# mathijs727/OpenCL-Path-Tracer

Hardware: AMD Instinct MI355X
Metric: Mrays/s at 1080p, 1M-tri SBVH scene; 1/2/4/8-GPU scaling + %HBM roofline (higher is better)
Workload: dtype f32

## Files before the change

### include/ptamd.h

```cpp
#ifndef PTAMD_H
#define PTAMD_H

#include <stddef.h>
#include <stdint.h>

#ifdef __cplusplus
extern "C" {
#endif

typedef enum {
    PT_OK = 0,
    PT_ERR_INVALID = -1,
    PT_ERR_HIP = -2,
    PT_ERR_STATE = -3,
    PT_ERR_UNSUPPORTED = -4
} pt_status;


typedef struct {
    float vertex[4];
    float normal[4];
    float texCoord[2];
    float _pad[2];
} pt_vertex;
// ... 121 lines not shown
void pt_destroy(pt_ctx* ctx);
const char* pt_last_error(const pt_ctx* ctx);
int pt_set_stream(pt_ctx* ctx, void* hip_stream);

int pt_upload_static(pt_ctx* ctx, const pt_vertex* verts, uint32_t n_verts, const pt_triangle* tris, uint32_t n_tris,
    const pt_material* mats, uint32_t n_mats, const pt_sub_bvh_node* nodes, uint32_t n_nodes);
int pt_upload_dynamic(pt_ctx* ctx, const pt_emissive_triangle* lights, uint32_t n_lights,
    const pt_top_bvh_node* top_nodes, uint32_t n_top, uint32_t top_root);
int pt_upload_static_async(pt_ctx* ctx, const pt_vertex* verts, uint32_t n_verts, const pt_triangle* tris, uint32_t n_tris,
    const pt_material* mats, uint32_t n_mats, const pt_sub_bvh_node* nodes, uint32_t n_nodes);
int pt_upload_dynamic_async(pt_ctx* ctx, const pt_emissive_triangle* lights, uint32_t n_lights,
    const pt_top_bvh_node* top_nodes, uint32_t n_top, uint32_t top_root);
int pt_frame_tick(pt_ctx* ctx);
int pt_update_geometry(pt_ctx* ctx, const pt_vertex* verts, uint32_t n_verts, const pt_sub_bvh_node* nodes, uint32_t n_nodes);
int pt_refit_vertices(pt_ctx* ctx, uint32_t first_vertex, const pt_vertex* verts, uint32_t n_verts);
typedef enum { PT_TEX_RGBA32F = 0, PT_TEX_BGRA8_UNORM = 1 } pt_texture_format;
int pt_upload_texture_array(pt_ctx* ctx, int kind, uint32_t width, uint32_t height, uint32_t layers, int format, const void* data);

int pt_set_camera(pt_ctx* ctx, const pt_camera* cam);
int pt_set_tiles(pt_ctx* ctx, const pt_rect* rects, uint32_t n);
int pt_set_accum_buffer(pt_ctx* ctx, void* device_float4);
int pt_clear(pt_ctx* ctx);

int pt_render(pt_ctx* ctx, uint32_t spp);
int pt_synchronize(pt_ctx* ctx);
int pt_resolve(pt_ctx* ctx, float* rgba_out);
int pt_resolve_device(pt_ctx* ctx, void* device_rgba);
void* pt_resolve_device_ptr(pt_ctx* ctx);
int pt_read_accum(pt_ctx* ctx, float* out_float4);
int pt_write_accum(pt_ctx* ctx, const float* in_float4, uint32_t spp);
void* pt_accum_device_ptr(pt_ctx* ctx);
uint32_t pt_samples_per_pixel(const pt_ctx* ctx);
int pt_stats_get(pt_ctx* ctx, pt_stats* out);
int pt_stats_reset(pt_ctx* ctx);
int pt_profile_kernels(pt_ctx* ctx, int enable);
int pt_reduce_accum(pt_ctx* ctx, void* nccl_comm, int root);

#define PT_GUIDE_SKY_DEPTH 1e6f
int pt_render_guides(pt_ctx* ctx, uint32_t spp);
uint32_t pt_guide_samples(const pt_ctx* ctx);
int pt_read_guides(pt_ctx* ctx, float* albedo_hits, float* normal_depth);
int pt_write_guides(pt_ctx* ctx, const float* albedo_hits, const float* normal_depth, uint32_t spp);
void* pt_guides_device_ptr(pt_ctx* ctx, int which);

#define PT_DENOISE_DEFAULT_K_NORMAL 64.0f
#define PT_DENOISE_DEFAULT_SIGMA_DEPTH 0.05f
#define PT_DENOISE_DEFAULT_SIGMA_LUM 0.7f
enum { PT_DENOISE_TONEMAPPED = 0, PT_DENOISE_HDR = 1 };
enum { PT_DENOISE_INPUT_ACCUM = 0, PT_DENOISE_INPUT_TEMPORAL = 1, PT_DENOISE_INPUT_TEMPORAL_VARIANCE = 2 };
typedef struct {
    uint32_t iterations;
    uint32_t output;
    float k_normal, sigma_depth, sigma_lum;
    uint32_t input;
    uint32_t _reserved[2];
} pt_denoise_params;
int pt_denoise(pt_ctx* ctx, const pt_denoise_params* params, float* rgba_out, float* ms_out);
int pt_denoise_device(pt_ctx* ctx, const pt_denoise_params* params, void* device_rgba);

int pt_set_sample_base(pt_ctx* ctx, uint32_t base);
uint32_t pt_sample_base(const pt_ctx* ctx);

typedef struct {
    uint32_t max_history;
    float k_normal, sigma_depth;
    uint32_t _reserved[5];
} pt_temporal_params;
int pt_temporal_accumulate(pt_ctx* ctx, const pt_temporal_params* params);
int pt_temporal_reset(pt_ctx* ctx);
uint32_t pt_temporal_frames(const pt_ctx* ctx);
int pt_read_temporal(pt_ctx* ctx, float* colour_count, float* normal_depth);
int pt_write_temporal(pt_ctx* ctx, const float* colour_count, const float* normal_depth, const pt_camera* made_under);
void* pt_temporal_device_ptr(pt_ctx* ctx, int which);

int pt_set_instance_motion(pt_ctx* ctx, const float* prev_inv_transforms, uint32_t n_top);
int pt_instance_motion(const pt_ctx* ctx, uint32_t* moving_out);
int pt_read_motion_guides(pt_ctx* ctx, float* motion, float* prev_normal);
int pt_write_motion_guides(pt_ctx* ctx, const float* motion, const float* prev_normal);
void* pt_motion_guides_device_ptr(pt_ctx* ctx, int which);
int pt_debug_motion_records(const float* prev_inv, const float* cur_inv, uint32_t n, float* out24);

int pt_set_vertex_motion(pt_ctx* ctx, int enable);
int pt_vertex_motion(const pt_ctx* ctx, uint32_t* deformed_out);
int pt_debug_vertex_motion_rows(const float* inv_transforms, uint32_t n, float* out12);

#define PT_VARIANCE_DEFAULT_SIGMA_VARIANCE 2.0f
#define PT_VARIANCE_DEFAULT_RELATIVE_FLOOR 0.1f
#define PT_VARIANCE_DEFAULT_FULL_HISTORY 16.0f
typedef struct {
    float sigma_variance;
    float relative_floor;
    float full_history;
    uint32_t _reserved[5];
} pt_variance_params;
int pt_set_temporal_variance(pt_ctx* ctx, const pt_variance_params* params);
int pt_temporal_variance(const pt_ctx* ctx);
int pt_read_temporal_variance(pt_ctx* ctx, float* out);
int pt_write_temporal_variance(pt_ctx* ctx, const float* in);
void* pt_temporal_variance_device_ptr(pt_ctx* ctx);

#define PT_RESPONSE_RADIUS 3
#define PT_RESPONSE_DEFAULT_FAST_HISTORY 4u
#define PT_RESPONSE_DEFAULT_SIGMA_RESPONSE 2.0f
#define PT_RESPONSE_DEFAULT_RELATIVE_FLOOR 0.02f
typedef struct {
    uint32_t fast_history;
    float sigma_response;
    float relative_floor;
    uint32_t _reserved[5];
} pt_response_params;
int pt_set_temporal_response(pt_ctx* ctx, const pt_response_params* params);
int pt_temporal_response(const pt_ctx* ctx);
int pt_read_temporal_fast(pt_ctx* ctx, float* colour_count);
int pt_write_temporal_fast(pt_ctx* ctx, const float* colour_count);
int pt_read_temporal_response(pt_ctx* ctx, float* s_out);
void* pt_temporal_fast_device_ptr(pt_ctx* ctx);

typedef struct {
    const float *ox, *oy, *oz, *dx, *dy, *dz;
    const float* tmax;
} pt_rays_soa;
typedef struct {
    float *t, *u, *v;
    int32_t* prim;
    int32_t* inst;
} pt_hits_soa;
int pt_intersect(pt_ctx* ctx, const pt_rays_soa* rays, uint32_t n, int any_hit, pt_hits_soa* hits, uint32_t repeat, float* ms_out);
int pt_gen_rays(pt_ctx* ctx, uint32_t sample, uint32_t n, float* ox, float* oy, float* oz, float* dx, float* dy, float* dz, uint32_t* pixel);
int pt_primary_pass(pt_ctx* ctx, uint32_t sample, uint32_t batch, uint32_t n, float* ox, float* oy, float* oz, float* dx, float* dy, float* dz,
    uint32_t* pixel, pt_hits_soa* hits);

typedef struct {
    uint32_t n;
    const float *ox, *oy, *oz, *dx, *dy, *dz;
    const float *thr_r, *thr_g, *thr_b;
    const uint32_t* pixel;
    const uint32_t* flags;
    const uint32_t* bounce;
    const float *t, *u, *v;
    const int32_t *prim, *inst;
    uint32_t sample;
    float *radiance;
    uint32_t* out_alive;
    float *nox, *noy, *noz, *ndx, *ndy, *ndz, *nthr_r, *nthr_g, *nthr_b;
    uint32_t* nflags;
    uint32_t* shadow_alive;
    float *sox, *soy, *soz, *sdx, *sdy, *sdz, *slen, *sc_r, *sc_g, *sc_b;
} pt_shade_batch_io;
int pt_shade_batch(pt_ctx* ctx, pt_shade_batch_io* io);

int pt_debug_copy_bandwidth(pt_ctx* ctx, size_t bytes, uint32_t repeat, float* gbps_out);
int pt_debug_math_probe(pt_ctx* ctx, const float* a, const float* b, uint32_t n, float* out);
int pt_debug_rng_probe(pt_ctx* ctx, const uint32_t* in, uint32_t n, uint32_t* out);
int pt_debug_live_resources(uint32_t out[4]);
int pt_debug_quantise_node(const float* lo12, const float* hi12, const uint32_t* refs4, const uint8_t* empty4, uint32_t empty_ref, void* out64);
int pt_debug_convert(const pt_config* cfg, const pt_vertex* verts, uint32_t n_verts, const pt_triangle* tris, uint32_t n_tris, const pt_material* mats,
                     uint32_t n_mats, const pt_sub_bvh_node* nodes, uint32_t n_nodes, const pt_emissive_triangle* lights, uint32_t n_lights,
                     const pt_top_bvh_node* top_nodes, uint32_t n_top, uint32_t top_root, char* line, size_t line_bytes);
const char* pt_version(void);

#ifdef __cplusplus
}
#endif
#endif
```

### opencl-path-tracer_amd/csrc/pt_context.h

```cpp
#pragma once

namespace {

thread_local std::string g_createError;

std::atomic<uint32_t> g_live[4];

template <typename T>
struct DevBuf {
    T* p = nullptr;
    size_t n = 0;
    DevBuf() = default;
    DevBuf(DevBuf&& o) noexcept : p(std::exchange(o.p, nullptr)), n(std::exchange(o.n, 0)) {}
    ~DevBuf() { release(); }
    hipError_t alloc(size_t count)
    {
        release();
        n = count;
        if (count == 0)
            return hipSuccess;
        const hipError_t e = hipMalloc((void**)&p, count * sizeof(T));
        if (e == hipSuccess)
            g_live[0]++;
        return e;
// ... 126 lines not shown
    DevBuf<float4> plane[2];
    float4* operator[](int k) const { return plane[k].p; }
    int ensure(pt_ctx* c);
    int zero(pt_ctx* c);
    int read(pt_ctx* c, float* out0, float* out1);
    int write(pt_ctx* c, const float* in0, const float* in1);
};

inline hipError_t allocPlanes(DevBuf<float4>& a, DevBuf<float4>& b, DevBuf<float4>& c, size_t count)
{
    hipError_t e = a.alloc(count);
    if (e == hipSuccess && (e = b.alloc(count)) == hipSuccess)
        e = c.alloc(count);
    return e;
}
struct RayQueueBuf {
    DevBuf<float4> o, d, thr;
    RayQueue view() const { return { o.p, d.p, thr.p }; }
    hipError_t alloc(size_t count) { return allocPlanes(o, d, thr, count); }
    void release() { o.release(), d.release(), thr.release(); }
};
struct ShadowQueueBuf {
    DevBuf<float4> o, d, c;
    ShadowQueue view() const { return { o.p, d.p, c.p }; }
    hipError_t alloc(size_t count) { return allocPlanes(o, d, c, count); }
    void release() { o.release(), d.release(), c.release(); }
};

}

struct StaticScene {
    ptconv::StaticHost host;
    DevBuf<WideNode> dWide;
    DevBuf<WideBoxes> dBoxes;
    DevBuf<uint32_t> dLeafOfs, dRefTri;
    DevBuf<TriIsect> dTris;
    DevBuf<TriFat> dFat;
    uint64_t onDeviceTopology = 0;
    DevBuf<pt_vertex> dVerts;
    DevBuf<pt_sub_bvh_node> dNodes;
    DevBuf<uint32_t> dKidBoxNode;
    DevBuf<float> dExtra;
    DevBuf<uint32_t> dParent, dNeed, dArrived;
    uint64_t refitTablesFor = 0;
    bool refitTablesOk = false;
    bool latestInStage = false;
    Staging stage;
    DevBuf<TriShade> triShade;
    DevBuf<Material> materials;
    bool have = false;
};

struct pt_ctx {
    pt_config cfg {};
    std::string error;
    int device = 0;
    int numCUs = 0;
    Stream stream;
    Stream copyStream;
    Stream sideStream;
    Stream sideStream2;
    Event evStart, evStop;
    std::vector<Event> profEvents;
    bool profile = false;

    ~pt_ctx()
    {
        (void)hipSetDevice(device);
        for (hipStream_t s : { stream.s, copyStream.s, sideStream.s, sideStream2.s })
            if (s)
                (void)hipStreamSynchronize(s);
    }

    struct DynamicSet {
        DevBuf<WideNode> wide;
        DevBuf<TriIsect> tris;
        DevBuf<TriFat> fat;
        DevBuf<Instance> instances;
        DevBuf<Light> lights;
        DevBuf<BakeJob> jobs;
        uint64_t staticVersion = 0;
        int staticIndex = 0;
        uint32_t numTris = 0, firstWorldNode = 0;
        Staging stage;
        uint32_t numLights = 0, rootRef = 0;
        uint32_t foldedInstances = 0, instRootBase = 0, numInstRoots = 0;
        DevBuf<float4> instFold;
        DevBuf<uint32_t> instRootSrc;
        uint32_t instFoldCount = 0;
        uint32_t rootRefFolded = 0;
        bool packetOk = false;
        uint32_t stackNeed = 0;
        bool hasInstances = false;
        bool generalRoute = false;
        uint32_t enteredInstances = 0;
        std::vector<uint32_t> instanceTopNode;
        std::vector<Instance> hostInstances;
        uint32_t numTopNodes = 0;
        Event uploaded;
        Event lastUse;
        bool used = false;
    } dyn[2];
    StaticScene stat[2];
    StaticScene* st = &stat[0];
    int statCur = 0;
    int statPending = -1;
    uint64_t staticVersions = 0;
    int active = 0;
    int pending = -1;
    Event evShaded[kMaxPasses], evShadowed[kMaxPasses];
    DevBuf<float4> accumShadow;
    ShadowQueueBuf shadowQ[kMaxPasses];
    bool mergePending = false;
    DevBuf<uint8_t> texMaterial, texSky;
    SceneDev scene {};
    bool haveStatic = false, haveDynamic = false, haveCamera = false;

    CameraDev camera {};
    DevBuf<uint32_t> pixelList;
    std::vector<uint32_t> hostPixelList;
    DevBuf<uint32_t> pixelOrdinal;
    DevBuf<float4> resolveTmp;
    uint32_t numOwned = 0;
    uint32_t capacity = 0;
    uint32_t capExt = 0, capShadow = 0;
    bool q0Small = false;
    bool ratiosKnown = false;
    double ratioExt = 0, ratioShadow = 0;
    double ratioShadowFirst = 0;
    Pinned<uint32_t> overflowPinned;
    uint32_t batchSamples = 0, probeBatches = 0;
    uint32_t epoch = 0, passCountsEpoch = 0;
    bool identityPixels = true;
    DevBuf<float4> accumOwn, accumPlanes;
    uint32_t packetBlocks[2] = { 0, 0 };
    uint32_t multiBlocks[4] = { 0, 0, 0, 0 };
    Pinned<uint32_t> passCountsPinned;
    Event passCountsCopied;
    uint32_t passCountsHint[2 * (kMaxPasses + 1)] = {};
    uint32_t passCountsEntries = 0;
    uint32_t passCountsPending = 0;
    uint32_t shadeHeadShift = 0;
    uint32_t packetUse = 0;
    uint64_t packetLaunches = 0, genLaunches = 0, bundleLaunches = 0;
    float4* accum = nullptr;
    uint32_t planes = 1;
    uint32_t spp = 0;

    RayQueueBuf rays[2], stagedRays;
    ShadowQueueBuf shadow, stagedShadow;
    DevBuf<float4> hitH;
    DevBuf<int32_t> hitInst;
    DevBuf<uint32_t> activeFlag;
    DevBuf<uint4> streams;
    DevBuf<Control> control;
    DevBuf<Totals> totals;
    DevBuf<uint32_t> spill;
    size_t spillHalf = 0;
    uint32_t traceBlocks[3] = { 0, 0, 0 };
    uint32_t teamBlocks = 0;
    float teamRounds = 1.5f;
    uint32_t teamUse = 7;
    uint32_t batchEntries = 0;
    uint64_t teamLaunches = 0;
    uint32_t foldPlanes = 0;
    bool queuesReady = false;

    PlanePair guides;
    uint32_t guideSpp = 0;
    DevBuf<float4> guideRayO, guideRayD, guideHit;
    DevBuf<int32_t> guideHitInst;
    DevBuf<Control> guideCtl;
    DevBuf<float4> denoiseColour[2], denoiseGuide;
    Event evDenoise[2];

    PlanePair temporal[2];
    int temporalNewest = 0;
    uint32_t temporalFrames = 0;
    CameraDev temporalCamera {};
    uint32_t sampleBase = 0;

    DevBuf<float> temporalVariance[2];
    bool varianceSet = false;
    float sigmaVariance = 0, relativeFloor = 0, fullHistory = 0;

    DevBuf<float4> temporalFast[2];
    DevBuf<float2> responseLuminance;
    DevBuf<float> responseMix;
    bool responseSet = false;
    float fastHistory = 0, sigmaResponse = 0, responseFloor = 0;

    DevBuf<MotionRecord> motionRecords;
    std::vector<MotionRecord> motionHost;
    bool motionSet = false;
    uint32_t motionMoving = 0;
    PlanePair motionGuides;

    DevBuf<TriFat> fatThen;
    DevBuf<float4> vertexRows;
    std::vector<float4> vertexRowsHost;
    bool vertexMotionSet = false;
    bool vertexDeformed = false;

    double msLastRender = 0, msIntersect = 0, msShade = 0, msShadow = 0, msGen = 0, msPacket = 0;
};

namespace {

int fail(pt_ctx* ctx, int code, const char* fmt, ...)
{
    char buf[512];
    va_list ap;
    va_start(ap, fmt);
    vsnprintf(buf, sizeof(buf), fmt, ap);
    va_end(ap);
    if (ctx)
        ctx->error = buf;
    else
        g_createError = buf;
    return code;
}

#define HIPCHK(ctx, call)                                                                              \
    do {                                                                                               \
        hipError_t _e = (call);                                                                        \
        if (_e != hipSuccess)                                                                          \
            return fail(ctx, PT_ERR_HIP, "%s failed: %s (%s:%d)", #call, hipGetErrorString(_e), __FILE__, __LINE__); \
    } while (0)

template <typename F>
int guarded(pt_ctx* c, const char* what, F&& body)
{
    try {
        return body();
    } catch (const std::bad_alloc&) {
        return fail(c, PT_ERR_UNSUPPORTED, "%s: out of host memory", what);
    } catch (const std::exception& e) {
        return fail(c, PT_ERR_INVALID, "%s: %s", what, e.what());
    } catch (...) {
        return fail(c, PT_ERR_INVALID, "%s: unknown exception", what);
    }
}

inline AccumView accumView(const pt_ctx* c) { return { c->accum, c->accumPlanes.p, c->pixelOrdinal.p, c->planes - 1u }; }
inline uint32_t maxBounces(const pt_ctx* c) { return c->cfg.max_bounces ? c->cfg.max_bounces : 4u; }
inline bool parityMode(const pt_ctx* c) { return c->cfg.rng_mode == PT_RNG_LFSR113_PARITY; }
inline bool generalShading(const pt_ctx* c) { return (c->cfg.flags & (PT_FLAG_INTEGRATOR_MIS | PT_FLAG_COMPARE_SHADING | PT_FLAG_SOLID_ANGLE_LIGHTS)) != 0u; }

void refreshSceneView(pt_ctx* c)
{
    SceneDev& s = c->scene;
    const pt_ctx::DynamicSet& d = c->dyn[c->active];
    s.wide = d.wide.p;
    s.tris = d.tris.p;
    s.triFat = d.fat.p;
    s.materials = c->st->materials.p;
    s.instances = d.instances.p;
    s.lights = d.lights.p;
    s.numLights = d.numLights;
    s.rootRef = d.rootRef;
    s.firstWorldNode = d.firstWorldNode;
    s.instRootBase = d.numInstRoots ? d.instRootBase : 0x7FFFFFFFu;
    s.numInstRoots = d.numInstRoots;
    s.materialTex.texels = c->texMaterial.p;
    s.sky.texels = c->texSky.p;
    s.numTriangles = c->haveDynamic ? d.numTris : c->st->host.numTris;
}

template <typename T>
int uploadVec(pt_ctx* c, DevBuf<T>& buf, const std::vector<T>& host)
{
    if (!buf.p || buf.n < std::max<size_t>(host.size(), 1))
        HIPCHK(c, buf.alloc(std::max<size_t>(host.size() + host.size() / 8, 1)));
    if (!host.empty())
        HIPCHK(c, hipMemcpy(buf.p, host.data(), host.size() * sizeof(T), hipMemcpyHostToDevice));
    return PT_OK;
}

int PlanePair::zero(pt_ctx* c)
{
    for (DevBuf<float4>& b : plane)
        HIPCHK(c, hipMemsetAsync(b.p, 0, b.n * sizeof(float4), c->stream));
    return PT_OK;
}

int PlanePair::ensure(pt_ctx* c)
{
    if (plane[0].p)
        return PT_OK;
    for (DevBuf<float4>& b : plane)
        HIPCHK(c, b.alloc((size_t)c->cfg.width * c->cfg.height));
    return zero(c);
}

int PlanePair::read(pt_ctx* c, float* out0, float* out1)
{
    if (const int rc = ensure(c))
        return rc;
    float* const out[2] = { out0, out1 };
    for (int k = 0; k < 2; k++)
        if (out[k])
            HIPCHK(c, hipMemcpyAsync(out[k], plane[k].p, plane[k].n * sizeof(float4), hipMemcpyDeviceToHost, c->stream));
    HIPCHK(c, hipStreamSynchronize(c->stream));
    return PT_OK;
}

// ... 13 lines not shown
```

### opencl-path-tracer_amd/csrc/pt_device.h

```cpp
#pragma once
#include <hip/hip_runtime.h>
#include <stdint.h>

namespace ptd {

struct PairNode {
    float4 bx;
    float4 by;
    float4 bz;
    uint32_t left, right;
    uint32_t _pad0, _pad1;
};

struct WideNode {
    float ox, oy, oz;
    float scaleX;
    uint32_t qlox, qhix, qloy, qhiy;
    uint32_t qloz, qhiz;
    float scaleY, scaleZ;
    uint32_t child[4];
};

constexpr uint32_t kRefIndexBits = 27;
constexpr uint32_t kRefIndexMask = (1u << kRefIndexBits) - 1u;
constexpr uint32_t kMaxLeafTris = 30;
constexpr uint32_t kRefSpecial = 31;
constexpr uint32_t kSpecialFinish = kRefIndexMask;
constexpr uint32_t kSpecialLeaveInstance = kRefIndexMask - 1u;
constexpr uint32_t kRefFinish = 0xFFFFFFFFu;
constexpr uint32_t kRefLeaveInstance = (kRefSpecial << kRefIndexBits) | kSpecialLeaveInstance;
constexpr uint32_t kRefNone = kRefFinish;
constexpr uint32_t kSpecialIdle = kRefIndexMask - 2u;
constexpr uint32_t kRefIdle = (kRefSpecial << kRefIndexBits) | kSpecialIdle;
constexpr uint32_t kRefFirstSpecial = kRefSpecial << kRefIndexBits;
__host__ __device__ inline uint32_t makeRef(uint32_t index, uint32_t count) { return (count << kRefIndexBits) | index; }
__host__ __device__ inline uint32_t refIndex(uint32_t r) { return r & kRefIndexMask; }
__host__ __device__ inline uint32_t refCount(uint32_t r) { return r >> kRefIndexBits; }

struct TriIsect {
    float4 a;
    float4 b;
    float4 c;
};

struct TriShade {
    uint32_t i0, i1, i2, material;
};
struct VertexShade {
    float4 n_u;
    float4 v_pad;
};
struct TriFat {
    float4 n0u, n1u, n2u;
    float4 vvvm;
    float4 e1e;
    float4 e2v;
    float4 v0c;
    float4 mat;
};

struct Instance {
    float4 r0, r1, r2;
    uint32_t rootRef;
    uint32_t topNode;
    uint32_t folded;
    uint32_t simple;
};

struct MotionRecord {
    float4 a0, a1, a2;
    float4 p0, p1, p2;
};

struct Material {
    float4 colour;
    float4 params;
    float4 typeAndPad;
};
enum : int { MAT_DIFFUSE = 0, MAT_PBR = 1, MAT_REFRACTIVE = 2, MAT_BASIC_REFRACTIVE = 3, MAT_EMISSIVE = 4 };

struct Light {
    float4 v0, v1, v2;
    float4 normal;
    float4 colour;
};

struct BakeJob {
    double m[12];
    uint32_t srcNode, numNodes;
    uint32_t dstNode;
    uint32_t srcRef, numRefs;
    uint32_t dstTri;
    uint32_t instance;
    uint32_t _pad;
};

struct WideBoxes {
    float lo[4][3], hi[4][3];
};

struct Texture {
    const void* texels;
    int32_t width, height, layers;
    int32_t format;
};
__device__ inline float4 fetchTexel(const Texture& tex, size_t index)
{
    if (tex.format == 0)
        return ((const float4*)tex.texels)[index];
    const uint32_t p = ((const uint32_t*)tex.texels)[index];
    return make_float4((float)((p >> 16) & 0xFFu) / 255.0f, (float)((p >> 8) & 0xFFu) / 255.0f, (float)(p & 0xFFu) / 255.0f, (float)(p >> 24) / 255.0f);
}

struct SceneDev {
    const PairNode* nodes;
    const WideNode* wide;
    const TriIsect* tris;
    const TriFat* triFat;
    const Material* materials;
    const Instance* instances;
    const Light* lights;
    Texture materialTex;
    Texture sky;
    uint32_t numLights;
    uint32_t rootRef;
    uint32_t numTriangles;
    uint32_t firstWorldNode;
    uint32_t instRootBase;
    uint32_t numInstRoots;
};

struct RayQueue {
    float4* o;
    float4* d;
    float4* thr;
};
struct HitQueue {
    float4* h;
    int32_t* inst;
};
struct ShadowQueue {
    float4* o;
    float4* d;
    float4* c;
};

enum : uint32_t { FLAG_FINISHED = 1, FLAG_LASTSPECULAR = 2 };
__host__ __device__ inline uint32_t packState(uint32_t flags, uint32_t bounce, uint32_t plane) { return (flags & 0xFFu) | ((bounce & 0xFFu) << 8) | (plane << 16); }
struct AccumView {
    float4* plane0;
    float4* extra;
    const uint32_t* ordinal;
    uint32_t perPixel;
    __device__ inline float4* at(uint32_t plane, uint32_t pixel) const
    {
        if (plane == 0u)
            return plane0 + pixel;
        const uint32_t slot = ordinal ? ordinal[pixel] : pixel;
        return extra + (size_t)slot * perPixel + (plane - 1u);
    }
    __device__ inline float4* atOrdinal(uint32_t plane, uint32_t slot) const { return extra + (size_t)slot * perPixel + (plane - 1u); }
};

struct CameraDev {
    float4 eye, screen, u, v, uN, vN;
    float focalDistance, apertureRadius, relativeAperture, shutterTime, ISO;
    uint32_t thinLens;
};

constexpr int kMaxPasses = 16;
#ifndef PT_GEN_INTERLEAVE
#define PT_GEN_INTERLEAVE 256
#endif
constexpr uint32_t kGenInterleave = PT_GEN_INTERLEAVE;
constexpr uint32_t kDepositSlots = 64;
struct Control {
    uint32_t extCount[kMaxPasses + 1];
    uint32_t shadowCount[kMaxPasses + 1];
    uint32_t extCursor[kMaxPasses + 1];
    uint32_t shadowCursor[kMaxPasses + 1];
    uint32_t shadeHits[kMaxPasses + 1];
    uint32_t depositsShade;
    uint32_t depositsShadow;
    uint32_t generated;
    uint32_t _pad;
    uint32_t depositSlots[kDepositSlots][16];
};
struct Totals {
    unsigned long long raysExtension, raysShadow, raysGenerated, shadeHits, deposits, depositsShadow;
};

}
```

### opencl-path-tracer_amd/csrc/pt_packet_multi.h

```cpp
#pragma once
#include "pt_packet.h"

#ifndef PT_MULTI_RAYS
#define PT_MULTI_RAYS 4
#endif
#ifndef PT_MULTI_MIN_WAVES
#define PT_MULTI_MIN_WAVES (PT_MULTI_RAYS >= 8 ? 3 : PT_MULTI_RAYS >= 4 ? 5 : 6)
#endif

namespace ptd {


template <int R>
__device__ inline bool bundleOctant(const V3 (&d)[R], V3& mLo, V3& mHi, bool& nx, bool& ny, bool& nz)
{
    mLo = mk(INFINITY), mHi = mk(0.f);
    unsigned long long sx = 0ull, sy = 0ull, sz = 0ull, ax = ~0ull, ay = ~0ull, az = ~0ull;
#pragma unroll
    for (int r = 0; r < R; r++) {
        const V3 id = mk(rcpSlab(d[r].x), rcpSlab(d[r].y), rcpSlab(d[r].z));
        mLo = mk(fminf(mLo.x, fabsf(id.x)), fminf(mLo.y, fabsf(id.y)), fminf(mLo.z, fabsf(id.z)));
        mHi = mk(fmaxf(mHi.x, fabsf(id.x)), fmaxf(mHi.y, fabsf(id.y)), fmaxf(mHi.z, fabsf(id.z)));
        const unsigned long long bx = __builtin_amdgcn_ballot_w64(id.x < 0.f), by = __builtin_amdgcn_ballot_w64(id.y < 0.f), bz = __builtin_amdgcn_ballot_w64(id.z < 0.f);
        sx |= bx, sy |= by, sz |= bz, ax &= bx, ay &= by, az &= bz;
    }
    nx = sx != 0ull, ny = sy != 0ull, nz = sz != 0ull;
    return (sx == 0ull || ax == ~0ull) && (sy == 0ull || ay == ~0ull) && (sz == 0ull || az == ~0ull);
}
__device__ inline void bundleBeam(const V3 co, V3 mLo, V3 mHi, bool nx, bool ny, bool nz, uint32_t axis, uint32_t isFar, float& S, float& negSO, float& mulPos,
    float& mulNeg, uint32_t& ofsQ)
{
    waveMin3Max3(mLo.x, mLo.y, mLo.z, mHi.x, mHi.y, mHi.z);
    const bool neg = axis == 0u ? nx : (axis == 1u ? ny : nz);
    const float oA = axis == 0u ? co.x : (axis == 1u ? co.y : co.z);
    const float mLoA = (axis == 0u ? mLo.x : (axis == 1u ? mLo.y : mLo.z)) * (1.f - 1.f / 262144.f);
    const float mHiA = (axis == 0u ? mHi.x : (axis == 1u ? mHi.y : mHi.z)) * (1.f + 1.f / 262144.f);
    S = neg ? -1.f : 1.f;
    negSO = -(S * oA);
    mulPos = isFar ? -mHiA : mLoA, mulNeg = isFar ? -mLoA : mHiA;
    ofsQ = 16u + 4u * (2u * axis + ((neg ? 1u : 0u) ^ isFar));
}

template <int R>
__device__ inline void bundleWaist(const V3 (&o)[R], const V3 (&d)[R], V3& pLo, V3& pHi)
{
    pLo = mk(INFINITY), pHi = mk(-INFINITY);
#pragma unroll
    for (int r = 0; r < R; r++) {
        const V3 p = mk(o[r].x + d[r].x, o[r].y + d[r].y, o[r].z + d[r].z);
        const V3 e = mk((fabsf(o[r].x) + fabsf(d[r].x)) * 0x1p-22f, (fabsf(o[r].y) + fabsf(d[r].y)) * 0x1p-22f, (fabsf(o[r].z) + fabsf(d[r].z)) * 0x1p-22f);
        pLo = mk(fminf(pLo.x, p.x - e.x), fminf(pLo.y, p.y - e.y), fminf(pLo.z, p.z - e.z));
        pHi = mk(fmaxf(pHi.x, p.x + e.x), fmaxf(pHi.y, p.y + e.y), fmaxf(pHi.z, p.z + e.z));
    }
}
__device__ inline void bundleBeamLens(V3 pLo, V3 pHi, V3 mLo, V3 mHi, bool nx, bool ny, bool nz, uint32_t axis, uint32_t isFar, float& S, float& negSO, float& mulPos,
    float& mulNeg, uint32_t& ofsQ, float& corner)
{
    waveMin3Max3(pLo.x, pLo.y, pLo.z, pHi.x, pHi.y, pHi.z);
    waveMin3Max3(mLo.x, mLo.y, mLo.z, mHi.x, mHi.y, mHi.z);
    const bool neg = axis == 0u ? nx : (axis == 1u ? ny : nz);
    const float pLoA = axis == 0u ? pLo.x : (axis == 1u ? pLo.y : pLo.z), pHiA = axis == 0u ? pHi.x : (axis == 1u ? pHi.y : pHi.z);
    const float mLoA = (axis == 0u ? mLo.x : (axis == 1u ? mLo.y : mLo.z)) * (1.f - 1.f / 262144.f);
    const float mHiA = (axis == 0u ? mHi.x : (axis == 1u ? mHi.y : mHi.z)) * (1.f + 1.f / 262144.f);
    S = neg ? -1.f : 1.f;
    corner = (neg != (isFar != 0u)) ? pLoA : pHiA;
    negSO = -(S * corner);
    mulPos = isFar ? -mHiA : mLoA, mulNeg = isFar ? -mLoA : mHiA;
    ofsQ = 16u + 4u * (2u * axis + ((neg ? 1u : 0u) ^ isFar));
}

template <int R, bool TWO_LEVEL, bool LENS = false>
#ifndef PT_MULTI_MIN_WAVES_TL
#define PT_MULTI_MIN_WAVES_TL PT_MULTI_MIN_WAVES
#endif
#ifndef PT_MULTI_MIN_WAVES_LENS
#define PT_MULTI_MIN_WAVES_LENS PT_MULTI_MIN_WAVES
#endif
#ifndef PT_MULTI_MIN_WAVES_LENS_TL
#define PT_MULTI_MIN_WAVES_LENS_TL 4
#endif
__global__ void __launch_bounds__(kPacketBlock, LENS ? (TWO_LEVEL ? PT_MULTI_MIN_WAVES_LENS_TL : PT_MULTI_MIN_WAVES_LENS) : (TWO_LEVEL ? PT_MULTI_MIN_WAVES_TL : PT_MULTI_MIN_WAVES))
    k_trace_multi(TraceArgs a)
{
    constexpr int RO = LENS ? R : 1;
    constexpr float tShift = LENS ? 1.0f : 0.0f;
    constexpr int kSaveRay = 0, kSaveBeam = 3 * RO + 3 * R, kSaveInst = kSaveBeam + 5, kSave = kSaveInst + R;
    __shared__ uint32_t ldsSave[TWO_LEVEL ? kPacketBlock / 64 : 1][TWO_LEVEL ? kSave : 1][64];
    const uint32_t pwave = threadIdx.x >> 6;
    typedef uint32_t u4v __attribute__((ext_vector_type(4)));
    typedef const u4v __attribute__((address_space(4)))* ScalarU4;
    const uint32_t lane = threadIdx.x & 63u;
    const uint32_t gwave = (blockIdx.x * kPacketBlock + threadIdx.x) >> 6;
    const uint32_t totalWaves = (gridDim.x * kPacketBlock) >> 6;
    const uint32_t count = a.ctl->extCount[a.pass];
    const SceneDev& sc = a.sc;
    constexpr uint32_t kPer = 64u * R;
    const uint32_t supers = (count + kPer - 1u) / kPer;
    const uint32_t rootRef = uni(sc.rootRef);
    const ScalarU4 wideS = (ScalarU4)(unsigned long long)sc.wide;
    const ScalarU4 trisS = (ScalarU4)(unsigned long long)sc.tris;

#ifndef PT_MULTI_SPAN
#define PT_MULTI_SPAN 8
#endif
    constexpr uint32_t kSpan = PT_MULTI_SPAN;
    uint32_t spanBase = uni(gwave) * kSpan, spanLeft = kSpan;
    for (;;) {
        if (spanLeft == 0u) {
            const uint32_t left = supers > spanBase ? supers - spanBase : 0u;
            const uint32_t claim = min(kSpan, max(1u, left / totalWaves));
            uint32_t b = 0;
            if (lane == 0)
                b = atomicAdd(&a.ctl->extCursor[a.pass], claim);
            spanBase = totalWaves * kSpan + uni(b);
            spanLeft = claim;
        }
        if (spanBase >= supers)
            break;
        const uint32_t base = spanBase * kPer;
        spanBase++;
        spanLeft--;

        V3 co[RO], cd[R];
        float tClosest[R], hu[R], hv[R];
        int hprim[R];
        bool whole = true;
#pragma unroll
        for (int r = 0; r < R; r++) {
            const uint32_t idx = base + 64u * (uint32_t)r + lane;
            const bool active = idx < count;
            V3 o = mk(0.f), d = mk(0.f, 0.f, 1.f);
            if (active) {
                uint32_t px, pl;
                primaryEntry(a.fp, a.pixelList, idx, &px, &pl);
                primaryRay(a.fp, px, pl, &o, &d);
                if (a.noOrigins) {
                    ((float4*)a.rayD)[idx] = make_float4(d.x, d.y, d.z, asF(px));
                } else {
                    ((float4*)a.rayO)[idx] = make_float4(o.x, o.y, o.z, asF(px));
                    ((float4*)a.rayD)[idx] = make_float4(d.x, d.y, d.z, asF(packState(FLAG_LASTSPECULAR, 0u, pl)));
                }
            }
            nudgeZero(o, d);
            if (LENS || r == 0)
                co[LENS ? r : 0] = o;
            cd[r] = d;
            tClosest[r] = INFINITY, hu[r] = hv[r] = 0.f, hprim[r] = -1;
            if constexpr (TWO_LEVEL)
                ldsSave[pwave][kSaveInst + r][lane] = 0xFFFFFFFFu;
            whole = whole && __builtin_amdgcn_ballot_w64(active) == ~0ull;
            if constexpr (!LENS)
                whole = whole && __builtin_amdgcn_ballot_w64(o.x != asF(uni(asU(co[0].x))) || o.y != asF(uni(asU(co[0].y))) || o.z != asF(uni(asU(co[0].z)))) == 0ull;
        }
        V3 mLo, mHi;
        bool nx, ny, nz;
        whole = bundleOctant<R>(cd, mLo, mHi, nx, ny, nz) && whole;

        if (whole) {
            const uint32_t role = lane & 7u, child = (lane >> 3) & 3u, axis = min(role >> 1, 2u), isFar = role & 1u;
            const uint32_t ofsO = 4u * axis, ofsE = axis == 0u ? 12u : 36u + 4u * axis, shift = 8u * child;
            float S, negSO, mulPos, mulNeg, corner = 0.f;
            uint32_t ofsQ;
            if constexpr (LENS) {
                V3 pLo, pHi;
                bundleWaist<R>(co, cd, pLo, pHi);
                bundleBeamLens(pLo, pHi, mLo, mHi, nx, ny, nz, axis, isFar, S, negSO, mulPos, mulNeg, ofsQ, corner);
            } else {
                bundleBeam(co[0], mLo, mHi, nx, ny, nz, axis, isFar, S, negSO, mulPos, mulNeg, ofsQ);
            }
            int curInst = -1;
            if constexpr (TWO_LEVEL) {
#pragma unroll
                for (int r = 0; r < RO; r++)
                    ldsSave[pwave][kSaveRay + 3 * r][lane] = asU(co[r].x), ldsSave[pwave][kSaveRay + 3 * r + 1][lane] = asU(co[r].y), ldsSave[pwave][kSaveRay + 3 * r + 2][lane] = asU(co[r].z);
#pragma unroll
                for (int r = 0; r < R; r++)
                    ldsSave[pwave][kSaveRay + 3 * RO + 3 * r][lane] = asU(cd[r].x), ldsSave[pwave][kSaveRay + 3 * RO + 1 + 3 * r][lane] = asU(cd[r].y),
                                  ldsSave[pwave][kSaveRay + 3 * RO + 2 + 3 * r][lane] = asU(cd[r].z);
                ldsSave[pwave][kSaveBeam + 0][lane] = asU(S), ldsSave[pwave][kSaveBeam + 1][lane] = asU(negSO), ldsSave[pwave][kSaveBeam + 2][lane] = asU(mulPos);
                ldsSave[pwave][kSaveBeam + 3][lane] = asU(mulNeg), ldsSave[pwave][kSaveBeam + 4][lane] = ofsQ;
            }
            float tcMax = INFINITY;
            uint32_t stRef = 0u;
            uint32_t sp = 0u;
            uint32_t cur = rootRef;
#ifdef PT_TRACE_STATS
            uint32_t stNodes = 0u, stLeaves = 0u, stTris = 0u;
#endif
            while (true) {
#ifdef PT_TRACE_STATS
                if (refCount(cur) == 0u)
                    stNodes++;
                else if (refCount(cur) != kRefSpecial)
                    stLeaves++, stTris += refCount(cur);
#endif
                if (TWO_LEVEL && refCount(cur) == kRefSpecial) {
                    if (cur != kRefLeaveInstance) {
                        typedef const u4v_t __attribute__((address_space(4)))* ScalarU4i;
                        const ScalarU4i mrow = (ScalarU4i)(unsigned long long)&sc.instances[refIndex(cur)];
                        const u4v_t m0 = mrow[0], m1 = mrow[1], m2 = mrow[2];
                        const float4 r0 = asF4(m0), r1 = asF4(m1), r2 = asF4(m2);
                        if (uni(mrow[3].w) != 0u) {
#pragma unroll
                            for (int r = 0; r < RO; r++)
                                co[r] = mk(fmaf(r0.x, co[r].x, r0.w), fmaf(r1.y, co[r].y, r1.w), fmaf(r2.z, co[r].z, r2.w));
#pragma unroll
                            for (int r = 0; r < R; r++)
                                cd[r] = mk(r0.x * cd[r].x, r1.y * cd[r].y, r2.z * cd[r].z);
                            const float scl = fastRcp(r0.x);
                            if constexpr (LENS) {
                                const float wA = axis == 0u ? r0.w : (axis == 1u ? r1.w : r2.w);
                                const float c = fmaf(r0.x, corner, wA);
                                const float e = (fabsf(r0.x * corner) + fabsf(wA)) * 0x1p-22f;
                                negSO = isFar ? -(S * c) + e : -(S * c) - e;
                            } else {
                                negSO = -(S * (axis == 0u ? co[0].x : (axis == 1u ? co[0].y : co[0].z)));
                            }
                            mulPos *= scl, mulNeg *= scl;
                        } else {
                            V3 to[RO], td[R];
#pragma unroll
                            for (int r = 0; r < R; r++)
                                rayIntoInstance(r0, r1, r2, co[LENS ? r : 0], cd[r], &to[LENS ? r : 0], &td[r]);
                            V3 tLo, tHi;
                            bool tnx, tny, tnz;
                            if (!bundleOctant<R>(td, tLo, tHi, tnx, tny, tnz)) {
                                whole = false;
                                break;
                            }
#pragma unroll
                            for (int r = 0; r < RO; r++)
                                co[r] = to[r];
#pragma unroll
                            for (int r = 0; r < R; r++)
                                cd[r] = td[r];
                            if constexpr (LENS) {
                                V3 pLo, pHi;
                                float cornerInst;
                                bundleWaist<R>(co, cd, pLo, pHi);
                                bundleBeamLens(pLo, pHi, tLo, tHi, tnx, tny, tnz, axis, isFar, S, negSO, mulPos, mulNeg, ofsQ, cornerInst);
                            } else {
                                bundleBeam(co[0], tLo, tHi, tnx, tny, tnz, axis, isFar, S, negSO, mulPos, mulNeg, ofsQ);
                            }
                        }
                        curInst = (int)refIndex(cur);
                        stRef = laneWrite(stRef, kRefLeaveInstance, uni(sp));
                        sp++;
                        cur = uni(mrow[3].x);
                        continue;
                    }
#pragma unroll
                    for (int r = 0; r < RO; r++)
                        co[r] = mk(asF(ldsSave[pwave][kSaveRay + 3 * r][lane]), asF(ldsSave[pwave][kSaveRay + 3 * r + 1][lane]), asF(ldsSave[pwave][kSaveRay + 3 * r + 2][lane]));
#pragma unroll
                    for (int r = 0; r < R; r++)
                        cd[r] = mk(asF(ldsSave[pwave][kSaveRay + 3 * RO + 3 * r][lane]), asF(ldsSave[pwave][kSaveRay + 3 * RO + 1 + 3 * r][lane]),
                            asF(ldsSave[pwave][kSaveRay + 3 * RO + 2 + 3 * r][lane]));
                    S = asF(ldsSave[pwave][kSaveBeam + 0][lane]), negSO = asF(ldsSave[pwave][kSaveBeam + 1][lane]), mulPos = asF(ldsSave[pwave][kSaveBeam + 2][lane]);
                    mulNeg = asF(ldsSave[pwave][kSaveBeam + 3][lane]), ofsQ = ldsSave[pwave][kSaveBeam + 4][lane];
                    curInst = -1;
                } else if (refCount(cur) == 0u) {
                    const uint32_t ni = refIndex(cur);
                    const u4v D = wideS[ni * 4u + 3u];
                    const char* nb = (const char*)&sc.wide[ni];
                    const float originA = *(const float*)(nb + ofsO);
                    const float scaleA = *(const float*)(nb + ofsE);
                    const uint32_t qd = *(const uint32_t*)(nb + ofsQ);
                    const float q = (float)((qd >> shift) & 0xFFu);
                    const float g = fmaf(q, S * scaleA, fmaf(S, originA, negSO));
                    float v = g * (g >= 0.f ? mulPos : mulNeg);
                    v = maxRowShr2(v);
                    v = maxRowShr2(v);
                    const float tn = rowShr1(v);
                    const unsigned long long m = __builtin_amdgcn_ballot_w64(tn + v <= 0.f) & __builtin_amdgcn_ballot_w64(v <= tShift) & __builtin_amdgcn_ballot_w64(tn < tcMax);
                    const uint32_t tloBits = (uint32_t)max((int32_t)asU(tn + tShift), 0);
                    uint32_t key[4];
#pragma unroll
                    for (int k = 0; k < 4; k++)
                        key[k] = ((m >> (8 * k + 5)) & 1ull) ? ((__builtin_amdgcn_readlane(tloBits, 8 * k + 5) & ~3u) | (uint32_t)k) : (kKeyNone | (uint32_t)k);
                    const bool s01 = key[0] < key[1], s23 = key[2] < key[3];
                    const uint32_t k01 = s01 ? key[0] : key[1], k23 = s23 ? key[2] : key[3];
                    const uint32_t r01 = s01 ? D.x : D.y, r23 = s23 ? D.z : D.w;
                    const bool sl = k01 < k23;
                    const uint32_t best = sl ? k01 : k23;
                    if (best < kKeyNone) {
                        const uint32_t refs[4] = { D.x, D.y, D.z, D.w };
                        const uint32_t limit = kKeyNone - best - 1u;
#pragma unroll
                        for (int k = 0; k < 4; k++)
                            if (key[k] - best - 1u < limit) {
                                stRef = laneWrite(stRef, uni(refs[k]), uni(sp));
                                sp++;
                            }
                        cur = sl ? r01 : r23;
                        continue;
// ... 14 lines not shown
                        for (int r = 0; r < R; r++) {
                            float det, u, v, t;
                            if constexpr (LENS)
                                triOriginHalf(co[r], v0, e1, e2, &T, &Q, &e2Q);
                            triRayHalf(cd[r], e1, e2, T, Q, e2Q, &det, &u, &v, &t);
                            const bool hit = PT_TRI_HIT(det, u, v, t, tClosest[r]);
                            if (hit) {
                                tClosest[r] = t;
                                hu[r] = u;
                                hv[r] = v;
                                hprim[r] = (int)(first + k);
                                if constexpr (TWO_LEVEL)
                                    ldsSave[pwave][kSaveInst + r][lane] = (uint32_t)curInst;
                                any = true;
                            }
                        }
                    }
                    if (__builtin_amdgcn_ballot_w64(any) != 0ull) {
                        float far = tClosest[0];
#pragma unroll
                        for (int r = 1; r < R; r++)
                            far = fmaxf(far, tClosest[r]);
                        if (__builtin_amdgcn_ballot_w64(far == INFINITY) == 0ull)
                            tcMax = LENS ? asF(uni(asU(waveMax(far)))) * (1.0f + 0x1p-20f) - tShift : asF(uni(asU(waveMax(far))));
                    }
                }
                if (sp == 0u)
                    break;
                sp--;
                cur = __builtin_amdgcn_readlane(stRef, sp);
            }
#ifdef PT_TRACE_STATS
            if (lane == 0) {
                atomicAdd(&g_traceStats[56], 1ull), atomicAdd(&g_traceStats[57], (unsigned long long)stNodes), atomicAdd(&g_traceStats[58], (unsigned long long)stLeaves);
                atomicAdd(&g_traceStats[59], (unsigned long long)stTris);
                if (!whole)
                    atomicAdd(&g_traceStats[60], 1ull);
            }
#endif
        }
        if (!whole) {
#pragma unroll 1
            for (int r = 0; r < R; r++) {
                const uint32_t idx = base + 64u * (uint32_t)r + lane;
                const bool active = idx < count;
                V3 o = mk(0.f), d = mk(0.f, 0.f, 1.f);
                if (active) {
                    uint32_t px, pl;
                    primaryEntry(a.fp, a.pixelList, idx, &px, &pl);
                    primaryRay(a.fp, px, pl, &o, &d);
                }
                nudgeZero(o, d);
                V3 cid = mk(rcpSlab(d.x), rcpSlab(d.y), rcpSlab(d.z));
                bool nx = cid.x < 0.f, ny = cid.y < 0.f, nz = cid.z < 0.f;
                const V3 wo = o, wd = d;
                int curInst = -1;
                if constexpr (TWO_LEVEL)
                    ldsSave[pwave][kSaveInst + r][lane] = 0xFFFFFFFFu;
                float tC = INFINITY, u_ = 0.f, v_ = 0.f;
                int hp = -1;
                uint32_t stRef = 0u, stLo = 0u, stHi = 0u;
                uint32_t sp = 0u;
                uint32_t cur = rootRef;
                unsigned long long curMask = __builtin_amdgcn_ballot_w64(active);
                if (curMask != 0ull)
                    while (true) {
                        const bool here = __builtin_amdgcn_inverse_ballot_w64(curMask);
                        if (TWO_LEVEL && refCount(cur) == kRefSpecial) {
                            if (cur != kRefLeaveInstance) {
                                V3 to, td;
                                uint32_t root;
                                packetIntoInstance(sc.instances, refIndex(cur), o, d, &to, &td, &root);
                                o = to, d = td, cid = mk(rcpSlab(td.x), rcpSlab(td.y), rcpSlab(td.z));
                                nx = cid.x < 0.f, ny = cid.y < 0.f, nz = cid.z < 0.f;
                                curInst = (int)refIndex(cur);
                                lanePush(stRef, stLo, stHi, kRefLeaveInstance, 0u, 0u, uni(sp));
                                sp++;
                                cur = uni(root);
                                continue;
                            }
                            o = wo, d = wd, cid = mk(rcpSlab(d.x), rcpSlab(d.y), rcpSlab(d.z));
                            nx = cid.x < 0.f, ny = cid.y < 0.f, nz = cid.z < 0.f;
                            curInst = -1;
                        } else if (refCount(cur) == 0u) {
                            const uint32_t ni = refIndex(cur);
                            const u4v A = wideS[ni * 4u + 0u], Cs = wideS[ni * 4u + 2u], D = wideS[ni * 4u + 3u];
                            const uint4* wp = (const uint4*)&sc.wide[ni];
                            const uint4 B = wp[1];
                            const uint2 C = *(const uint2*)&wp[2];
                            const SlabSetup slab = slabSetup(make_uint4(A.x, A.y, A.z, A.w), B, make_uint4(C.x, C.y, Cs.z, Cs.w), o, cid, nx, ny, nz);
                            const float tLimit = here ? tC : -INFINITY;
                            unsigned long long m[4];
                            uint32_t key[4];
#pragma unroll
                            for (int k = 0; k < 4; k++) {
                                const f2 tt = childSlab(slab, k);
                                const float tmin = tt.x, tmax = tt.y;
                                const float tlo = fmaxf(tmin, 0.f);
                                const bool vis = tmax >= tlo && tmin < tLimit;
                                m[k] = __builtin_amdgcn_ballot_w64(vis);
                                const uint32_t pick = (uint32_t)(__builtin_ffsll((long long)m[k]) - 1) & 63u;
                                key[k] = (__builtin_amdgcn_readlane(asU(vis ? tlo : INFINITY), pick) & ~3u) | (uint32_t)k;
                            }
                            const bool s01 = key[0] < key[1], s23 = key[2] < key[3];
                            const uint32_t k01 = s01 ? key[0] : key[1], k23 = s23 ? key[2] : key[3];
                            const uint32_t r01 = s01 ? D.x : D.y, r23 = s23 ? D.z : D.w;
                            const unsigned long long m01 = s01 ? m[0] : m[1], m23 = s23 ? m[2] : m[3];
                            const bool sl = k01 < k23;
                            const uint32_t best = sl ? k01 : k23;
                            if (best < kKeyNone) {
                                const uint32_t refs[4] = { D.x, D.y, D.z, D.w };
                                const uint32_t limit = kKeyNone - best - 1u;
#pragma unroll
                                for (int k = 0; k < 4; k++)
                                    if (key[k] - best - 1u < limit) {
                                        lanePush(stRef, stLo, stHi, uni(refs[k]), uni((uint32_t)m[k]), uni((uint32_t)(m[k] >> 32)), uni(sp));
                                        sp++;
                                    }
                                cur = sl ? r01 : r23;
                                curMask = sl ? m01 : m23;
                                continue;
                            }
                        } else {
                            const uint32_t first = refIndex(cur), n = refCount(cur);
                            for (uint32_t k = 0; k < n; k++) {
                                const u4v ta = trisS[(first + k) * 3u + 0u], tb = trisS[(first + k) * 3u + 1u];
                                const uint32_t tcx = trisS[(first + k) * 3u + 2u].x;
                                V3 v0, e1, e2;
                                triEdges(asF4(ta), asF4(tb), asF(tcx), &v0, &e1, &e2);
                                V3 T, Q;
                                float e2Q, det, u, v, t;
                                triOriginHalf(o, v0, e1, e2, &T, &Q, &e2Q);
                                triRayHalf(d, e1, e2, T, Q, e2Q, &det, &u, &v, &t);
                                const bool hit = here && PT_TRI_HIT(det, u, v, t, tC);
                                if (hit) {
                                    tC = t, u_ = u, v_ = v, hp = (int)(first + k);
                                    if constexpr (TWO_LEVEL)
                                        ldsSave[pwave][kSaveInst + r][lane] = (uint32_t)curInst;
                                }
                            }
                        }
                        if (sp == 0u)
                            break;
                        sp--;
                        cur = __builtin_amdgcn_readlane(stRef, sp);
                        curMask = (unsigned long long)__builtin_amdgcn_readlane(stLo, sp) | ((unsigned long long)__builtin_amdgcn_readlane(stHi, sp) << 32);
                    }
#pragma unroll
                for (int q = 0; q < R; q++)
                    if (q == r)
                        tClosest[q] = tC, hu[q] = u_, hv[q] = v_, hprim[q] = hp;
            }
        }
#pragma unroll
        for (int r = 0; r < R; r++) {
            const uint32_t idx = base + 64u * (uint32_t)r + lane;
            if (idx < count) {
                int hinst = -1;
                if constexpr (TWO_LEVEL)
                    hinst = (int)ldsSave[pwave][kSaveInst + r][lane];
                writeClosestHit(a, sc, idx, tClosest[r], hu[r], hv[r], hprim[r], hinst);
            }
        }
    }
}

}
```

### opencl-path-tracer_amd/csrc/pt_schedule.h

```cpp
#pragma once

namespace {

void lfsrJump(uint32_t g[4])
{
    uint32_t z, b;
    z = g[0] & (uint32_t)(-2);
    b = (z << 6) ^ z;
    z = (z) ^ (z << 2) ^ (z << 3) ^ (z << 10) ^ (z << 13) ^ (z << 16) ^ (z << 19) ^ (z << 22) ^ (z << 25) ^ (z << 27) ^ (z << 28)
        ^ ((b >> 3) & 0x1FFFFFFF) ^ ((b >> 4) & 0x0FFFFFFF) ^ ((b >> 6) & 0x03FFFFFF) ^ ((b >> 9) & 0x007FFFFF)
        ^ ((b >> 12) & 0x000FFFFF) ^ ((b >> 15) & 0x0001FFFF) ^ ((b >> 18) & 0x00003FFF) ^ ((b >> 21) & 0x000007FF);
    g[0] = z;
    z = g[1] & (uint32_t)(-8);
    b = (z << 2) ^ z;
    z = ((b >> 13) & 0x0007FFFF) ^ (z << 16);
    g[1] = z;
    z = g[2] & (uint32_t)(-16);
    b = (z << 13) ^ z;
    z = (z << 2) ^ (z << 4) ^ (z << 10) ^ (z << 12) ^ (z << 13) ^ (z << 17) ^ (z << 25)
        ^ ((b >> 3) & 0x1FFFFFFF) ^ ((b >> 11) & 0x001FFFFF) ^ ((b >> 15) & 0x0001FFFF) ^ ((b >> 16) & 0x0000FFFF) ^ ((b >> 24) & 0x000000FF);
    g[2] = z;
    z = g[3] & (uint32_t)(-128);
    b = (z << 3) ^ z;
    z = (z << 9) ^ (z << 10) ^ (z << 11) ^ (z << 14) ^ (z << 16) ^ (z << 18) ^ (z << 23) ^ (z << 24)
        ^ ((b >> 1) & 0x7FFFFFFF) ^ ((b >> 2) & 0x3FFFFFFF) ^ ((b >> 7) & 0x01FFFFFF) ^ ((b >> 9) & 0x007FFFFF)
        ^ ((b >> 11) & 0x001FFFFF) ^ ((b >> 14) & 0x0003FFFF) ^ ((b >> 15) & 0x0001FFFF) ^ ((b >> 16) & 0x0000FFFF)
        ^ ((b >> 23) & 0x000001FF) ^ ((b >> 24) & 0x000000FF);
    g[3] = z;
}

int resetStreams(pt_ctx* c)
{
    const size_t n = (size_t)c->cfg.width * c->cfg.height;
    std::vector<uint4> host(n);
    uint32_t g[4] = { 987654321u, 987654321u, 987654321u, 987654321u };
    for (size_t i = 0; i < n; i++) {
        host[i] = make_uint4(g[0], g[1], g[2], g[3]);
        lfsrJump(g);
    }
    return uploadVec(c, c->streams, host);
}

#ifndef PT_SPLIT_SHADOW_ACCUM
#define PT_SPLIT_SHADOW_ACCUM 1
#endif
inline bool splitShadowAccum(const pt_ctx* c, uint64_t cap)
{
    return PT_SPLIT_SHADOW_ACCUM && c->planes == 1u && !parityMode(c) && c->cfg.max_active_rays == 0 && cap <= (4u << 20) && !(c->packetUse & 2u) && maxBounces(c) <= (uint32_t)kMaxPasses;
}

bool derivedPrimariesCapable(const pt_ctx* c);
inline void newEpoch(pt_ctx* c)
{
    c->epoch++;
    c->ratiosKnown = false;
    c->ratioExt = c->ratioShadow = c->ratioShadowFirst = 0;
}
inline bool smallQueues(const pt_ctx* c) { return c->capExt < c->capacity || c->capShadow < c->capacity; }
inline int checkOverflow(pt_ctx* c)
{
    if (c->overflowPinned.p && *c->overflowPinned.p)
        return fail(c, PT_ERR_STATE, "a batch emitted more rays than its queues hold (pt_config.ext_queue_fraction / shadow_queue_fraction; the scene changed under a "
                                    "running batch?): the rays beyond were dropped, the image since the last pt_clear is incomplete -- pt_clear and render again");
    return PT_OK;
}
inline void adoptPassCounts(pt_ctx* c)
{
    std::memcpy(c->passCountsHint, c->passCountsPinned.p, sizeof(c->passCountsHint));
    c->passCountsEntries = c->passCountsPending;
    c->passCountsPending = 0;
    if (c->passCountsEpoch == c->epoch && c->passCountsEntries) {
        const double entries = (double)c->passCountsEntries;
        uint32_t shadowMost = 0;
        for (int b = 0; b <= kMaxPasses; b++)
            shadowMost = std::max(shadowMost, c->passCountsHint[kMaxPasses + 1 + b]);
        c->ratioExt = std::max(c->ratioExt, (double)c->passCountsHint[1] / entries);
        c->ratioShadow = std::max(c->ratioShadow, (double)shadowMost / entries);
        c->ratioShadowFirst = std::max(c->ratioShadowFirst, (double)c->passCountsHint[kMaxPasses + 1] / entries);
        c->ratiosKnown = true;
    }
}
inline uint32_t safeBatch(const pt_ctx* c)
{
    auto limit = [&](uint32_t cap, double ratio) -> double {
        if (!(ratio > 0.0))
            return (double)c->planes;
        const double room = (double)cap - std::min(65536.0, (double)cap / 64.0);
        return room / (ratio * 1.03 * (double)c->numOwned);
    };
    double b = std::min(limit(c->capExt, c->ratioExt), limit(c->capShadow, c->ratioShadow));
    if (const char* e = getenv("PTAMD_DEBUG_BATCH_SCALE"))
        b *= atof(e);
    return (uint32_t)std::max(1.0, std::min((double)c->planes, b));
}

int ensureQueues(pt_ctx* c)
{
    if (c->queuesReady)
        return PT_OK;
    if (c->numOwned == 0)
        return fail(c, PT_ERR_STATE, "no pixels owned by this context");
    c->planes = 1;
    if (!parityMode(c) && c->cfg.max_active_rays == 0) {
        uint32_t want = c->cfg.samples_in_flight;
        if (want == 0)
            want = (uint32_t)std::min<uint64_t>(4096, std::max<uint64_t>(1, (32u << 20) / std::max(c->numOwned, 1u)));
        c->planes = std::min(want, 4096u);
        if (c->planes >= kGenInterleave) {
            c->planes -= c->planes % kGenInterleave;
        } else {
            uint32_t p2 = 1;
            while (p2 * 2u <= c->planes)
                p2 *= 2u;
            c->planes = p2;
        }
    }
    uint64_t cap64 = c->cfg.max_active_rays ? c->cfg.max_active_rays : (uint64_t)c->numOwned * c->planes;
    if (cap64 > 0x7FFFFFC0ull)
        return fail(c, PT_ERR_UNSUPPORTED, "%llu queue entries (%u owned pixels x %u samples in flight) exceed the 2^31 entries a queue can index: lower samples_in_flight",
            (unsigned long long)cap64, c->numOwned, c->planes);
    uint32_t cap = ((uint32_t)cap64 + 63u) & ~63u;
    {
        HIPCHK(c, hipStreamSynchronize(c->stream));
        c->rays[0].release(), c->rays[1].release(), c->shadow.release(), c->hitH.release(), c->hitInst.release(), c->accumPlanes.release();
        for (ShadowQueueBuf& q : c->shadowQ)
            q.release();
        c->stagedRays.release(), c->stagedShadow.release(), c->activeFlag.release();
        c->foldPlanes = 0;
        const bool split = splitShadowAccum(c, cap);
        c->capExt = c->capShadow = cap;
        c->q0Small = false;
        const float fe = c->cfg.ext_queue_fraction, fs = c->cfg.shadow_queue_fraction;
        if (!parityMode(c) && c->cfg.max_active_rays == 0 && c->planes >= 16u && !split) {
            if (fe > 0.f && fe < 1.f)
                c->capExt = std::min<uint64_t>(cap, (((uint64_t)((double)cap * fe) + 63u) & ~63ull) + 64u);
            if (fs > 0.f && fs < 1.f)
                c->capShadow = std::min<uint64_t>(cap, (((uint64_t)((double)cap * fs) + 63u) & ~63ull) + 64u);
            const uint64_t floorEntries = std::min<uint64_t>(cap, ((16ull * c->numOwned + 63u) & ~63ull));
            c->capExt = (uint32_t)std::max<uint64_t>(c->capExt, floorEntries);
            c->capShadow = (uint32_t)std::max<uint64_t>(c->capShadow, floorEntries);
            c->q0Small = c->capExt < cap && derivedPrimariesCapable(c);
        }
        newEpoch(c);
        const uint64_t q0 = 16ull * cap + 32ull * (c->q0Small ? c->capExt : cap);
        const uint64_t need = q0 + 48ull * c->capExt + 48ull * c->capShadow + 20ull * cap + (uint64_t)cap * (parityMode(c) ? 2ull * 48 + 4 : 0)
            + (uint64_t)(c->planes - 1) * c->numOwned * sizeof(float4)
            + (split ? (uint64_t)cap * 48 * maxBounces(c) + (uint64_t)c->cfg.width * c->cfg.height * sizeof(float4) * maxBounces(c) : 0);
        size_t freeB = 0, totalB = 0;
        HIPCHK(c, hipMemGetInfo(&freeB, &totalB));
        if (need > (uint64_t)freeB)
            return fail(c, PT_ERR_UNSUPPORTED, "queues and accumulator planes need %.1f GB (%u owned pixels x %u samples in flight), %.1f GB of device memory are free: lower samples_in_flight or set max_active_rays",
                need / 1e9, c->numOwned, c->planes, freeB / 1e9);
    }
    if (c->planes > 1) {
        const size_t n = (size_t)(c->planes - 1) * c->numOwned;
        HIPCHK(c, c->accumPlanes.alloc(n));
        HIPCHK(c, hipMemsetAsync(c->accumPlanes.p, 0, n * sizeof(float4), c->stream));
    }
    c->capacity = cap;
    HIPCHK(c, c->rays[0].o.alloc(c->q0Small ? c->capExt : cap));
    HIPCHK(c, c->rays[0].d.alloc(cap));
    HIPCHK(c, c->rays[0].thr.alloc(c->q0Small ? c->capExt : cap));
    HIPCHK(c, c->rays[1].alloc(c->capExt));
    HIPCHK(c, c->shadow.alloc(c->capShadow));
    HIPCHK(c, c->hitH.alloc(cap));
    HIPCHK(c, c->hitInst.alloc(cap));
    if (parityMode(c)) {
        HIPCHK(c, c->stagedRays.alloc(cap));
        HIPCHK(c, c->stagedShadow.alloc(cap));
        HIPCHK(c, c->activeFlag.alloc(cap));
        int rc = resetStreams(c);
        if (rc)
            return rc;
    }
    if (splitShadowAccum(c, cap)) {
        const size_t npx = (size_t)c->cfg.width * c->cfg.height;
        if (!c->accumShadow.p || c->accumShadow.n < npx * maxBounces(c)) {
            HIPCHK(c, c->accumShadow.alloc(npx * maxBounces(c)));
            HIPCHK(c, hipMemsetAsync(c->accumShadow.p, 0, npx * maxBounces(c) * sizeof(float4), c->stream));
        }
        for (uint32_t b = 0; b < maxBounces(c); b++)
            HIPCHK(c, c->shadowQ[b].alloc(cap));
    }
    HIPCHK(c, c->control.alloc(1));
    HIPCHK(c, hipMemsetAsync(c->control.p, 0, sizeof(Control), c->stream));
    c->queuesReady = true;
    return PT_OK;
}

int ensureSpill(pt_ctx* c)
{
    if (c->spill.p)
        return PT_OK;
    const void* variants[3][2] = { { (const void*)k_trace<false, 0>, (const void*)k_trace<true, 0> }, { (const void*)k_trace<false, 1>, (const void*)k_trace<true, 1> },
        { (const void*)k_trace<false, 2>, (const void*)k_trace<true, 2> } };
    const void* packetVariants[2][2] = { { (const void*)k_trace_packet<false, false>, (const void*)k_trace_packet<true, false> },
        { (const void*)k_trace_packet<false, true>, (const void*)k_trace_packet<true, true> } };
    for (int tl = 0; tl < 3; tl++) {
        int blocksPerCU = 8;
        for (const void* fn : variants[tl]) {
            int b = 0;
            HIPCHK(c, hipOccupancyMaxActiveBlocksPerMultiprocessor(&b, fn, kTraceBlock, 0));
            blocksPerCU = std::min(blocksPerCU, b);
        }
        blocksPerCU = std::max(1, blocksPerCU);
        if (const char* e = getenv("PTAMD_TRACE_BLOCKS_PER_CU"))
            blocksPerCU = std::max(1, std::min(blocksPerCU, atoi(e)));
        c->traceBlocks[tl] = (uint32_t)(blocksPerCU * c->numCUs);
        if (tl >= 2)
            continue;
        int pb = 8;
        for (const void* fn : packetVariants[tl]) {
            int b = 0;
            HIPCHK(c, hipOccupancyMaxActiveBlocksPerMultiprocessor(&b, fn, kPacketBlock, 0));
            pb = std::min(pb, b);
        }
        pb = std::max(1, pb);
        if (const char* e = getenv("PTAMD_PACKET_BLOCKS_PER_CU"))
            pb = std::max(1, std::min(pb, atoi(e)));
        c->packetBlocks[tl] = (uint32_t)(pb * c->numCUs);
    }
    {
        int b = 0;
        HIPCHK(c, hipOccupancyMaxActiveBlocksPerMultiprocessor(&b, (const void*)k_trace_multi<PT_MULTI_RAYS, false>, kPacketBlock, 0));
        c->multiBlocks[0] = (uint32_t)(std::max(1, b) * c->numCUs);
        HIPCHK(c, hipOccupancyMaxActiveBlocksPerMultiprocessor(&b, (const void*)k_trace_multi<PT_MULTI_RAYS, true>, kPacketBlock, 0));
        c->multiBlocks[1] = (uint32_t)(std::max(1, b) * c->numCUs);
        HIPCHK(c, hipOccupancyMaxActiveBlocksPerMultiprocessor(&b, (const void*)k_trace_multi<PT_MULTI_RAYS, false, true>, kPacketBlock, 0));
        c->multiBlocks[2] = (uint32_t)(std::max(1, b) * c->numCUs);
        HIPCHK(c, hipOccupancyMaxActiveBlocksPerMultiprocessor(&b, (const void*)k_trace_multi<PT_MULTI_RAYS, true, true>, kPacketBlock, 0));
        c->multiBlocks[3] = (uint32_t)(std::max(1, b) * c->numCUs);
        if (const char* e = getenv("PTAMD_PACKET_BLOCKS_PER_CU"))
            for (uint32_t& mb : c->multiBlocks)
                mb = std::max(1u, std::min(mb, (uint32_t)std::max(1, atoi(e)) * (uint32_t)c->numCUs));
    }
    {
        int t0 = 0, t1 = 0;
        HIPCHK(c, hipOccupancyMaxActiveBlocksPerMultiprocessor(&t0, (const void*)k_trace_team<false>, kTeamBlock, 0));
        HIPCHK(c, hipOccupancyMaxActiveBlocksPerMultiprocessor(&t1, (const void*)k_trace_team<true>, kTeamBlock, 0));
        c->teamBlocks = (uint32_t)(std::max(1, std::min(t0, t1)) * c->numCUs);
        if (const char* e = getenv("PTAMD_TEAM_ROUNDS"))
            c->teamRounds = std::max(0.f, (float)atof(e));
        if (const char* e = getenv("PTAMD_TEAM_USE"))
            c->teamUse = (uint32_t)atoi(e);
    }
    const size_t threads = (size_t)std::max(std::max(c->traceBlocks[0], c->traceBlocks[1]), c->traceBlocks[2]) * kTraceBlock;
    HIPCHK(c, c->spill.alloc(3 * threads * kSpillStack));
    c->spillHalf = threads * kSpillStack;
    return PT_OK;
}

inline int sceneKind(const pt_ctx* c)
{
    static const bool forceTwoLevel = getenv("PTAMD_FORCE_TWO_LEVEL_KERNELS") != nullptr;
    return (c->dyn[c->active].hasInstances || forceTwoLevel) ? 1 : 0;
}

inline int traceKind(const pt_ctx* c) { return sceneKind(c) == 0 ? 0 : (c->dyn[c->active].generalRoute ? 2 : 1); }

bool teamLaunch(const pt_ctx* c, uint32_t pass, bool anyHit = false)
{
    if (!(c->teamRounds > 0.f) || !c->teamBlocks || parityMode(c) || c->dyn[c->active].hasInstances || c->dyn[c->active].stackNeed > kTeamStackNeedMax)
        return false;
    if (c->cfg.flags & PT_FLAG_TEAM_INTERSECT)
        return true;
    if (!c->batchEntries || pass > (uint32_t)kMaxPasses)
        return false;
    if (pass == 0u && c->planes == 1u && c->batchEntries <= (4u << 20) && (c->teamUse & (anyHit ? 4u : 1u)))
        return true;
    if (c->passCountsEntries != c->batchEntries || !(c->teamUse & 2u))
        return false;
    const uint64_t teams = (uint64_t)c->teamBlocks * (kTeamBlock / 4);
    return (double)c->passCountsHint[pass] <= (double)teams * c->teamRounds;
}

void launchTrace(pt_ctx* c, bool anyHit, const TraceArgs& args, hipStream_t stream = nullptr)
{
    if (teamLaunch(c, args.pass, anyHit)) {
        c->teamLaunches++;
        if (anyHit)
            hipLaunchKernelGGL(k_trace_team<true>, dim3(c->teamBlocks), dim3(kTeamBlock), 0, stream ? stream : c->stream, args);
        else
            hipLaunchKernelGGL(k_trace_team<false>, dim3(c->teamBlocks), dim3(kTeamBlock), 0, stream ? stream : c->stream, args);
        return;
    }
    const bool twoLevel = sceneKind(c) != 0;
    const int kind = traceKind(c);
    TraceArgs a = args;
    if (twoLevel) {
        a.sc.rootRef = c->dyn[c->active].rootRefFolded;
        a.instFold = c->dyn[c->active].instFold.p, a.instFoldCount = c->dyn[c->active].instFoldCount;
    }
    const dim3 grid(c->traceBlocks[kind]), block(kTraceBlock);
    if (!stream)
        stream = c->stream;
    if (anyHit) {
        if (kind == 2)
            hipLaunchKernelGGL((k_trace<true, 2>), grid, block, 0, stream, a);
        else if (kind == 1)
            hipLaunchKernelGGL((k_trace<true, 1>), grid, block, 0, stream, a);
        else
            hipLaunchKernelGGL((k_trace<true, 0>), grid, block, 0, stream, a);
    } else {
        if (kind == 2)
            hipLaunchKernelGGL((k_trace<false, 2>), grid, block, 0, stream, a);
        else if (kind == 1)
            hipLaunchKernelGGL((k_trace<false, 1>), grid, block, 0, stream, a);
        else
            hipLaunchKernelGGL((k_trace<false, 0>), grid, block, 0, stream, a);
    }
}

TraceArgs traceArgsBase(pt_ctx* c)
{
    TraceArgs a {};
    a.sc = c->scene;
    a.spill = c->spill.p;
    a.totalThreads = c->traceBlocks[traceKind(c)] * kTraceBlock;
    a.parityShadow = parityMode(c) ? 1u : 0u;
    return a;
}

FrameParams frameParams(const pt_ctx* c, uint32_t sample)
{
    FrameParams fp {};
    fp.cam = c->camera;
    fp.width = c->cfg.width;
    fp.height = c->cfg.height;
    fp.sample = sample;
    fp.seed = c->cfg.seed;
    fp.maxBounces = maxBounces(c);
    fp.parity = parityMode(c) ? 1u : 0u;
    fp.numOwned = c->numOwned;
    fp.planes = 1;
    fp.interleave = 1;
    fp.interleaveShift = 0;
    fp.invWidth = 1.0f / (float)c->cfg.width;
    fp.integrator = (c->cfg.flags & PT_FLAG_COMPARE_SHADING) ? INTEGRATOR_COMPARE : ((c->cfg.flags & PT_FLAG_INTEGRATOR_MIS) ? INTEGRATOR_MIS : INTEGRATOR_IS);
    fp.weightedLights = (c->cfg.flags & PT_FLAG_SOLID_ANGLE_LIGHTS) ? 1u : 0u;
    fp.invSpan = 0.f;
    return fp;
}

struct Prof {
    pt_ctx* c;
    size_t next = 0;
    std::vector<std::pair<int, size_t>> marks;
    void begin(int family)
    {
        if (!c->profile)
            return;
        if (c->profEvents.size() < next + 2) {
            c->profEvents.resize(next + 2);
            for (Event& e : c->profEvents)
                (void)e.create(true);
        }
        (void)hipEventRecord(c->profEvents[next], c->stream);
        marks.push_back({ family, next });
    }
    void end()
    {
        if (!c->profile)
            return;
        (void)hipEventRecord(c->profEvents[next + 1], c->stream);
        next += 2;
    }
};

void launchGen(pt_ctx* c, const FrameParams& fp, int q, uint32_t first, uint32_t n, uint32_t slotBase, uint32_t pass)
{
    Control* ctl = c->control.p;
    const uint32_t span = fp.planes > 1u ? fp.numOwned * fp.interleave : std::max(n, 1u);
    const uint32_t blocks = (span + 255u) / 256u, rows = fp.planes > 1u ? fp.planes / fp.interleave : 1u;
    c->genLaunches++;
    hipLaunchKernelGGL(k_gen, dim3(blocks, rows), dim3(256), 0, c->stream, fp, c->rays[q].view(), c->identityPixels ? nullptr : c->pixelList.p,
        first, n, slotBase, c->streams.p, &ctl->extCount[pass], &ctl->generated);
}

#ifndef PT_FRAME_BUNDLES
#define PT_FRAME_BUNDLES 0
#endif
#ifndef PT_FUSED_PRIMARY
#define PT_FUSED_PRIMARY 1
#endif
#ifndef PT_SHADE_SPLIT
#define PT_SHADE_SPLIT 1
#endif
#ifndef PT_LAST_SHADOW_ON_MAIN
#define PT_LAST_SHADOW_ON_MAIN 1
#endif
#ifndef PT_DERIVED_PRIMARIES
#define PT_DERIVED_PRIMARIES 1
#endif
#ifndef PT_OVERLAP_SMALL
#define PT_OVERLAP_SMALL 1
#endif
#ifndef PT_PACKET_USE
#define PT_PACKET_USE 1
#endif
constexpr uint32_t kPacketUseDefault = PT_PACKET_USE;

void launchPacket(pt_ctx* c, bool anyHit, const TraceArgs& a)
{
    const bool twoLevel = sceneKind(c) != 0;
    const dim3 grid(c->packetBlocks[twoLevel ? 1 : 0]), block(kPacketBlock);
    c->packetLaunches++;
    if (anyHit) {
        if (twoLevel)
            hipLaunchKernelGGL((k_trace_packet<true, true>), grid, block, 0, c->stream, a);
        else
            hipLaunchKernelGGL((k_trace_packet<true, false>), grid, block, 0, c->stream, a);
    } else {
        if (twoLevel)
            hipLaunchKernelGGL((k_trace_packet<false, true>), grid, block, 0, c->stream, a);
        else
            hipLaunchKernelGGL((k_trace_packet<false, false>), grid, block, 0, c->stream, a);
    }
}

inline bool lensBundles()
{
    static const bool on = !(getenv("PTAMD_LENS_BUNDLES") && atoi(getenv("PTAMD_LENS_BUNDLES")) == 0);
    return on;
}
inline bool primaryBundles(const pt_ctx* c)
{
    return PT_MULTI_RAYS > 1 && (!c->camera.thinLens || lensBundles()) && !(c->packetUse & 8u) && c->dyn[c->active].packetOk && (c->packetUse & 1u);
}
bool derivedPrimariesCapable(const pt_ctx* c)
{
    return c->haveCamera && c->haveDynamic && !c->camera.thinLens && primaryBundles(c) && PT_FUSED_PRIMARY && PT_DERIVED_PRIMARIES && !(c->cfg.flags & PT_FLAG_QUEUE_PRIMARY_RAYS);
}

inline bool firstPassCoherent(const pt_ctx* c, const FrameParams& fp, uint32_t batch) { return fp.interleave >= 16u || (PT_FRAME_BUNDLES && batch == 1u && primaryBundles(c)); }

void launchIntersect(pt_ctx* c, int q, uint32_t pass, bool coherent = false, const FrameParams* fused = nullptr, bool noOrigins = false)
{
    Control* ctl = c->control.p;
    TraceArgs a = traceArgsBase(c);
    if (fused) {
        a.fused = 1u;
        a.fp = *fused;
        a.pixelList = c->identityPixels ? nullptr : c->pixelList.p;
    }
    a.rayO = c->rays[q].o.p;
    a.rayD = c->rays[q].d.p;
    a.hit = c->hitH.p;
    a.inst = c->hitInst.p;
    a.ctl = ctl;
    a.pass = pass;
    if (coherent && c->dyn[c->active].packetOk && (c->packetUse & 1u)) {
        if (fused && primaryBundles(c)) {
            a.noOrigins = noOrigins ? 1u : 0u;
            c->packetLaunches++;
            c->bundleLaunches++;
            if (c->camera.thinLens) {
                a.noOrigins = 0u;
                if (sceneKind(c) != 0)
                    hipLaunchKernelGGL((k_trace_multi<PT_MULTI_RAYS, true, true>), dim3(c->multiBlocks[3]), dim3(kPacketBlock), 0, c->stream, a);
                else
                    hipLaunchKernelGGL((k_trace_multi<PT_MULTI_RAYS, false, true>), dim3(c->multiBlocks[2]), dim3(kPacketBlock), 0, c->stream, a);
            } else if (sceneKind(c) != 0)
                hipLaunchKernelGGL((k_trace_multi<PT_MULTI_RAYS, true>), dim3(c->multiBlocks[1]), dim3(kPacketBlock), 0, c->stream, a);
            else
                hipLaunchKernelGGL((k_trace_multi<PT_MULTI_RAYS, false>), dim3(c->multiBlocks[0]), dim3(kPacketBlock), 0, c->stream, a);
        } else {
            launchPacket(c, false, a);
        }
    } else {
        launchTrace(c, false, a);
    }
}

void launchShadow(pt_ctx* c, uint32_t pass, bool coherent = false, hipStream_t side = nullptr, const ShadowQueueBuf* own = nullptr)
{
    Control* ctl = c->control.p;
    TraceArgs a = traceArgsBase(c);
    if (side)
        a.spill = c->spill.p + c->spillHalf * (side == c->sideStream2 ? 2u : 1u);
    const ShadowQueueBuf& q = own ? *own : c->shadow;
    a.rayO = q.o.p;
    a.rayD = q.d.p;
    a.rayC = q.c.p;
    a.accum = own ? AccumView { c->accumShadow.p + (size_t)pass * c->cfg.width * c->cfg.height, nullptr, nullptr, 0u } : accumView(c);
    a.ctl = ctl;
    a.pass = pass;
    if (coherent && c->dyn[c->active].packetOk && (c->packetUse & 2u))
        launchPacket(c, true, a);
    else
        launchTrace(c, true, a, side);
}

void launchShade(pt_ctx* c, const FrameParams& fp, int in, int out, uint32_t pass, uint32_t launchEntries, const ShadowQueueBuf* ownShadow = nullptr, bool derivedPrimaries = false)
{
    Control* ctl = c->control.p;
    ShadeArgs a {};
    a.sc = c->scene;
    a.fp = fp;
    a.in = c->rays[in].view();
    a.hits = { c->hitH.p, c->hitInst.p };
    a.accum = accumView(c);
    a.inCount = &ctl->extCount[pass];
    a.outCount = &ctl->extCount[pass + 1];
    a.shadowCount = &ctl->shadowCount[pass];
    a.shadeHits = &ctl->shadeHits[pass];
    a.deposits = parityMode(c) ? &ctl->depositsShade : &ctl->depositSlots[0][0];
    a.streams = c->streams.p;
    a.derivedPrimaries = derivedPrimaries ? 1u : 0u;
    a.outCap = out == 1 ? c->capExt : (c->q0Small ? c->capExt : c->capacity);
    a.shadowCap = ownShadow ? c->capacity : c->capShadow;
    const uint32_t blocks = (std::max(launchEntries, 1u) + kShadeBlock - 1u) / kShadeBlock;
    if (parityMode(c)) {
        a.out = c->stagedRays.view();
        a.shadow = c->stagedShadow.view();
        a.activeFlag = c->activeFlag.p;
        if (generalShading(c))
            hipLaunchKernelGGL((k_shade<true, true>), dim3(blocks), dim3(kShadeBlock), 0, c->stream, a);
        else
            hipLaunchKernelGGL((k_shade<true, false>), dim3(blocks), dim3(kShadeBlock), 0, c->stream, a);
        CompactArgs ca {};
        ca.staged = c->stagedRays.view();
        ca.out = c->rays[out].view();
        ca.stagedShadow = c->stagedShadow.view();
        ca.outShadow = c->shadow.view();
        ca.activeFlag = c->activeFlag.p;
        ca.inCount = &ctl->extCount[pass];
        ca.outCount = &ctl->extCount[pass + 1];
        ca.shadowCount = &ctl->shadowCount[pass];
        ca.shadeHits = &ctl->shadeHits[pass];
        hipLaunchKernelGGL(k_compact_stable, dim3(1), dim3(1024), 0, c->stream, ca);
    } else {
        a.out = c->rays[out].view();
        a.shadow = ownShadow ? ownShadow->view() : c->shadow.view();
        uint32_t head = blocks;
        if (PT_SHADE_SPLIT && pass > 0) {
            if (c->passCountsEntries && !c->shadeHeadShift) {
                const double scale = (double)launchEntries / (double)c->passCountsEntries;
                const double guess = (double)c->passCountsHint[pass] * scale * 1.03;
                head = std::min(blocks, (uint32_t)(guess / kShadeBlock) + 8u);
            } else {
                head = std::max(1u, blocks >> std::min(pass + c->shadeHeadShift, 24u));
            }
        }
        if (generalShading(c))
            hipLaunchKernelGGL((k_shade<false, true>), dim3(head), dim3(kShadeBlock), 0, c->stream, a);
        else if (c->st->host.materialBins)
            hipLaunchKernelGGL((k_shade<false, false, false, true>), dim3(head), dim3(kShadeBlock), 0, c->stream, a);
        else
            hipLaunchKernelGGL((k_shade<false, false>), dim3(head), dim3(kShadeBlock), 0, c->stream, a);
        if (head < blocks) {
            a.firstTile = head;
            const uint32_t rest = std::min(blocks - head, launchEntries <= (4u << 20) ? 64u : 512u);
            if (generalShading(c))
                hipLaunchKernelGGL((k_shade<false, true, true>), dim3(rest), dim3(kShadeBlock), 0, c->stream, a);
            else
                hipLaunchKernelGGL((k_shade<false, false, true>), dim3(rest), dim3(kShadeBlock), 0, c->stream, a);
        }
    }
}

FrameParams batchFrameParams(pt_ctx* c, uint32_t sample, uint32_t batch)
{
    FrameParams fp = frameParams(c, sample);
    fp.planes = batch;
    fp.interleave = 1;
    while (fp.interleave < kGenInterleave && batch % (fp.interleave * 2u) == 0u)
        fp.interleave *= 2u, fp.interleaveShift++;
    fp.invSpan = 1.0f / (float)((uint64_t)c->numOwned << fp.interleaveShift);
    return fp;
}

int renderSampleFixed(pt_ctx* c, uint32_t sample, uint32_t batch, Prof& prof)
{
    FrameParams fp = batchFrameParams(c, sample, batch);
    if (c->passCountsPending) {
        if (hipEventQuery(c->passCountsCopied) == hipSuccess) {
            adoptPassCounts(c);
        } else {
            (void)hipGetLastError();
        }
    }
    const uint32_t bounces = maxBounces(c);
    const uint32_t entries = c->numOwned * batch;
    c->batchEntries = entries;
    const bool coherentFirst = firstPassCoherent(c, fp, batch);
    const bool packetsFirst = coherentFirst && c->dyn[c->active].packetOk && (c->packetUse & 1u);
    const bool fused = packetsFirst && PT_FUSED_PRIMARY && !(c->cfg.flags & PT_FLAG_QUEUE_PRIMARY_RAYS);
    const bool derived = fused && primaryBundles(c) && !c->camera.thinLens && PT_DERIVED_PRIMARIES;
    if (c->q0Small && !derived && entries > c->capExt)
        return fail(c, PT_ERR_STATE, "the first queue was sized for camera rays queued as directions only, and this batch queues their origins");
    prof.begin(0);
    if (fused)
        hipLaunchKernelGGL(k_begin_batch, dim3(1), dim3(64), 0, c->stream, &c->control.p->extCount[0], &c->control.p->generated, entries);
    else
        launchGen(c, fp, 0, 0, entries, 0, 0);
    prof.end();
    const bool overlap = PT_OVERLAP_SMALL && entries <= (4u << 20) && !c->profile && !(c->packetUse & 2u);
    const bool split = splitShadowAccum(c, c->capacity);
    if (split) {
        if (!c->accumShadow.p || !c->shadowQ[bounces - 1].o.p)
            return fail(c, PT_ERR_STATE, "the buffers of the one-sample-in-flight schedule are missing");
        c->mergePending = true;
    }
    int in = 0, out = 1;
    for (uint32_t b = 0; b < bounces; b++) {
        prof.begin(1);
        const bool coherent = b == 0 && coherentFirst;
        if (c->profile && coherent && c->dyn[c->active].packetOk && (c->packetUse & 1u))
            prof.marks.back().first = 4;
        launchIntersect(c, in, b, coherent, fused && b == 0 ? &fp : nullptr, derived && b == 0);
        prof.end();
        if (overlap && !split && b > 0)
            HIPCHK(c, hipStreamWaitEvent(c->stream, c->evShadowed[b - 1], 0));
        prof.begin(2);
        launchShade(c, fp, in, out, b, entries, split ? &c->shadowQ[b] : nullptr, derived && b == 0);
        if (b == 0 ? smallQueues(c) : c->capShadow < c->capExt) {
            const uint32_t outCap = out == 1 ? c->capExt : (c->q0Small ? c->capExt : c->capacity);
            hipLaunchKernelGGL(k_clamp_counts, dim3(1), dim3(64), 0, c->stream, c->control.p, b, outCap, c->capShadow, c->overflowPinned.p);
        }
        prof.end();
        prof.begin(3);
        if (overlap && b + 1u == bounces && PT_LAST_SHADOW_ON_MAIN) {
            launchShadow(c, b, coherent, nullptr, split ? &c->shadowQ[b] : nullptr);
        } else if (overlap) {
            hipStream_t side = split && (b & 1u) ? c->sideStream2 : c->sideStream;
            HIPCHK(c, hipEventRecord(c->evShaded[b], c->stream));
            HIPCHK(c, hipStreamWaitEvent(side, c->evShaded[b], 0));
            launchShadow(c, b, coherent, side, split ? &c->shadowQ[b] : nullptr);
            HIPCHK(c, hipEventRecord(c->evShadowed[b], side));
        } else {
            launchShadow(c, b, coherent, nullptr, split ? &c->shadowQ[b] : nullptr);
        }
        prof.end();
        std::swap(in, out);
    }
    if (overlap && PT_LAST_SHADOW_ON_MAIN) {
        if (split && bounces > 1)
            HIPCHK(c, hipStreamWaitEvent(c->stream, c->evShadowed[bounces - 2], 0));
        if (split && bounces > 2)
            HIPCHK(c, hipStreamWaitEvent(c->stream, c->evShadowed[bounces - 3], 0));
    } else if (overlap) {
        HIPCHK(c, hipStreamWaitEvent(c->stream, c->evShadowed[bounces - 1], 0));
        if (split && bounces > 1)
            HIPCHK(c, hipStreamWaitEvent(c->stream, c->evShadowed[bounces - 2], 0));
    }
    const bool report = c->passCountsPinned.p && !c->passCountsPending;
    hipLaunchKernelGGL(k_end_sample, dim3(1), dim3(64), 0, c->stream, c->control.p, c->totals.p, bounces, report ? c->passCountsPinned.p : nullptr);
    if (report) {
        HIPCHK(c, hipEventRecord(c->passCountsCopied, c->stream));
        c->passCountsPending = entries;
        c->passCountsEpoch = c->epoch;
    }
    c->batchSamples = batch;
    c->batchEntries = 0;
    c->foldPlanes = std::max(c->foldPlanes, batch);
    HIPCHK(c, hipGetLastError());
    return PT_OK;
}

void foldPlanesNow(pt_ctx* c)
{
    if (c->mergePending) {
        const uint32_t n = c->cfg.width * c->cfg.height;
        hipLaunchKernelGGL(k_merge_accum, dim3((n + 255u) / 256u), dim3(256), 0, c->stream, c->accum, c->accumShadow.p, n, maxBounces(c));
        c->mergePending = false;
    }
    if (c->foldPlanes > 1) {
        const uint32_t n = c->numOwned;
        hipLaunchKernelGGL(k_fold_planes, dim3((uint32_t)(((uint64_t)n * kFoldLanes + 255) / 256)), dim3(256), 0, c->stream, accumView(c), c->foldPlanes,
            c->identityPixels ? nullptr : c->pixelList.p, n);
    }
    c->foldPlanes = 0;
}

int renderSampleRefill(pt_ctx* c, uint32_t sample)
{
    const FrameParams fp = frameParams(c, sample);
    Control* ctl = c->control.p;
    const uint32_t cap = c->capacity;
    uint32_t issued = 0, surviving = 0, pass = 0;
    int in = 0, out = 1;
    Control zero {};
    while (true) {
        hipLaunchKernelGGL(k_set_word, dim3(1), dim3(64), 0, c->stream, &ctl->extCount[0], surviving);
        HIPCHK(c, hipMemsetAsync(&ctl->extCount[1], 0, sizeof(uint32_t), c->stream));
        HIPCHK(c, hipMemsetAsync(&ctl->shadowCount[0], 0, sizeof(uint32_t), c->stream));
        HIPCHK(c, hipMemsetAsync(&ctl->extCursor[0], 0, sizeof(uint32_t), c->stream));
        HIPCHK(c, hipMemsetAsync(&ctl->shadowCursor[0], 0, sizeof(uint32_t), c->stream));
        uint32_t newRays = 0;
        if (surviving != cap) {
            newRays = std::min(cap - surviving, c->numOwned - issued);
            if (newRays)
                launchGen(c, fp, in, issued, newRays, surviving, 0);
        }
        const uint32_t entries = surviving + newRays;
        launchIntersect(c, in, 0);
        launchShade(c, fp, in, out, 0, entries);
        uint32_t counts[2] = { 0, 0 };
        HIPCHK(c, hipMemcpyAsync(&counts[0], &ctl->extCount[1], sizeof(uint32_t), hipMemcpyDeviceToHost, c->stream));
        HIPCHK(c, hipMemcpyAsync(&counts[1], &ctl->shadowCount[0], sizeof(uint32_t), hipMemcpyDeviceToHost, c->stream));
        HIPCHK(c, hipStreamSynchronize(c->stream));
        issued += newRays;
        surviving = counts[0];
        pass++;
        if (counts[1] != 0)
            launchShadow(c, 0);
        hipLaunchKernelGGL(k_end_sample, dim3(1), dim3(64), 0, c->stream, c->control.p, c->totals.p, 0u, (uint32_t*)nullptr);
        if (surviving == 0 && issued >= c->numOwned)
            break;
        std::swap(in, out);
        if (pass > 100000)
            return fail(c, PT_ERR_STATE, "refill loop did not terminate");
    }
    (void)zero;
    HIPCHK(c, hipGetLastError());
    return PT_OK;
}

}
```

### opencl-path-tracer_amd/csrc/pt_shade.h

```cpp
#pragma once
#include "pt_math.h"

namespace ptd {

constexpr float kPI = 3.14159265359f;
constexpr float kINVPI = 0.31830988618f;
constexpr float kEPS = 0.0001f;
constexpr float kMaxSmoothness = 0.94f;
constexpr float kAirIor = 1.000277f;

__device__ inline float4 sampleLinearRepeat(const Texture& tex, float s, float t, float layerCoord)
{
    const int w = tex.width, h = tex.height;
    const float u = (s - floorf(s)) * (float)w;
    const float v = (t - floorf(t)) * (float)h;
    int i0 = (int)floorf(u - 0.5f), j0 = (int)floorf(v - 0.5f);
    int i1 = i0 + 1, j1 = j0 + 1;
    if (i0 < 0) i0 += w;
    if (i1 > w - 1) i1 -= w;
    if (j0 < 0) j0 += h;
    if (j1 > h - 1) j1 -= h;
    const float a = (u - 0.5f) - floorf(u - 0.5f);
    const float b = (v - 0.5f) - floorf(v - 0.5f);
    int layer = (int)rintf(layerCoord);
// ... 478 lines not shown
        const V3 I = -D;
        bool refract = false;
        float n1n2 = 0.f, cos1 = 0.f, K = 0.f;
        if (!(rand01 < F.x)) {
            n1n2 = fastDiv(n_i, n_t);
            cos1 = dot(halfway, I);
            K = 1 - (n1n2 * n1n2) * (1 - cos1 * cos1);
            refract = K >= 0;
        }
        if (refract)
            reflection = fastNormalize(-n1n2 * I + halfway * (n1n2 * cos1 - fastSqrt(K)));
        else
            reflection = fastNormalize(I - 2 * dot(I, halfway) * halfway);
        const float w = calcWeight(I, raySideNormal, halfway, mat.p0, reflection);
        BRDF = mk(w) * absorptionFactor;
    } else if (mat.type == MAT_DIFFUSE) {
        if (albedo.x == -1.0f) {
            reflection = D;
            BRDF = mk(1.0f);
        } else {
            reflection = cosineWeightedDiffuseReflection(realNormal, edge1, in, rng);
            if (MIS)
                out.pdf = dot(shadingNormal, reflection) * kINVPI;
            BRDF = albedo;
        }
    }

    out.flags = (mat.type == MAT_REFRACTIVE || mat.type == MAT_BASIC_REFRACTIVE || dospecular) ? FLAG_LASTSPECULAR : 0u;
    const V3 integral = fastDiv(BRDF * cosineTerm, PDF);
    const float survive = saturate(fmaxf(fmaxf(integral.x, integral.y), integral.z));
    const float choice = rng.u01();
    if (survive < kEPS || choice > survive) {
        out.flags = FLAG_FINISHED;
        return;
    }
    out.origin = X + reflection * kEPS;
    out.direction = reflection;
    out.throughput = fastDiv(throughput * integral, survive);
}

struct FrameParams {
    CameraDev cam;
    uint32_t width, height;
    uint32_t sample, seed;
    uint32_t maxBounces;
    uint32_t parity;
    uint32_t numOwned;
    uint32_t planes;
    uint32_t interleave;
    uint32_t interleaveShift;
    float invWidth;
    uint32_t integrator;
    uint32_t weightedLights;
    float invSpan;
};
enum : uint32_t { INTEGRATOR_IS = 0, INTEGRATOR_MIS = 1, INTEGRATOR_COMPARE = 2 };

__device__ inline void primaryEntry(const FrameParams& fp, const uint32_t* __restrict__ pixelList, uint32_t i, uint32_t* pixel, uint32_t* plane)
{
    const uint32_t span = fp.numOwned << fp.interleaveShift;
    uint32_t group = (uint32_t)((float)i * fp.invSpan);
    if (group * span > i)
        group--;
    if ((group + 1u) * span <= i)
        group++;
    const uint32_t r = i - group * span;
    *plane = (group << fp.interleaveShift) + (r & ((1u << fp.interleaveShift) - 1u));
    const uint32_t k = r >> fp.interleaveShift;
    *pixel = pixelList ? pixelList[k] : k;
}
__device__ inline void primaryRay(const FrameParams& fp, uint32_t pixel, uint32_t plane, V3* o, V3* d)
{
    uint32_t py = (uint32_t)((float)pixel * fp.invWidth);
    if (py * fp.width > pixel)
        py--;
    if ((py + 1u) * fp.width <= pixel)
        py++;
    uint32_t px = pixel - py * fp.width;
    if (fp.integrator == INTEGRATOR_COMPARE && px >= fp.width / 2u)
        px -= fp.width / 2u;
    Rng rng = rngCounter(pixel, fp.sample + plane, fp.seed, 0u);
    cameraRay(fp.cam, (int)px, (int)py, (float)fp.width, (float)fp.height, rng, o, d);
}

__global__ void k_begin_batch(uint32_t* queueCount, uint32_t* generated, uint32_t n)
{
    if (threadIdx.x == 0 && blockIdx.x == 0) {
        *queueCount = n;
        *generated += n;
    }
}

__global__ void __launch_bounds__(256) k_gen(FrameParams fp, RayQueue q, const uint32_t* __restrict__ pixelList, uint32_t first,
    uint32_t n, uint32_t slotBase, uint4* __restrict__ streams, uint32_t* __restrict__ queueCount, uint32_t* __restrict__ generated)
{
    const uint32_t r = blockIdx.x * blockDim.x + threadIdx.x;
    uint32_t i = r, plane = 0, k = first + r;
    if (fp.planes > 1u) {
        const uint32_t span = fp.numOwned << fp.interleaveShift;
        if (r >= span)
            return;
        i = blockIdx.y * span + r;
        plane = (blockIdx.y << fp.interleaveShift) + (r & ((1u << fp.interleaveShift) - 1u));
        k = first + (r >> fp.interleaveShift);
    }
    if (i == 0) {
        *queueCount = slotBase + n;
        *generated += n;
    }
    if (i >= n)
        return;
    const uint32_t pixel = pixelList ? pixelList[k] : k;
    uint32_t py = (uint32_t)((float)pixel * fp.invWidth);
    if (py * fp.width > pixel)
        py--;
    if ((py + 1u) * fp.width <= pixel)
        py++;
    uint32_t px = pixel - py * fp.width;
    if (fp.integrator == INTEGRATOR_COMPARE && px >= fp.width / 2u)
        px -= fp.width / 2u;
    Rng rng = fp.parity ? rngLfsrLoad(streams, i) : rngCounter(pixel, fp.sample + plane, fp.seed, 0u);
    V3 o, d;
    if (fp.parity)
        cameraRayPrecise(fp.cam, (int)px, (int)py, (float)fp.width, (float)fp.height, rng, &o, &d);
    else
        cameraRay(fp.cam, (int)px, (int)py, (float)fp.width, (float)fp.height, rng, &o, &d);
    if (fp.parity)
        rngLfsrStore(streams, i, rng);
    const uint32_t slot = slotBase + i;
    q.o[slot] = make_float4(o.x, o.y, o.z, asF(pixel));
    q.d[slot] = make_float4(d.x, d.y, d.z, asF(packState(FLAG_LASTSPECULAR, 0u, plane)));
    if (fp.parity)
        q.thr[slot] = make_float4(1.f, 1.f, 1.f, 0.f);
}

struct ShadeArgs {
    SceneDev sc;
    FrameParams fp;
    RayQueue in;
    HitQueue hits;
    RayQueue out;
    ShadowQueue shadow;
    AccumView accum;
    const uint32_t* inCount;
    uint32_t* outCount;
    uint32_t* shadowCount;
    uint32_t* shadeHits;
    uint32_t* deposits;
    uint4* streams;
    uint32_t* activeFlag;
    uint32_t firstTile;
    uint32_t derivedPrimaries;
    uint32_t outCap, shadowCap;
};

#ifndef PT_SHADE_BLOCK
#define PT_SHADE_BLOCK 512
#endif
#ifndef PT_SHADE_MIN_WAVES
#define PT_SHADE_MIN_WAVES 6
#endif
constexpr int kShadeBlock = PT_SHADE_BLOCK;
#ifndef PT_SHADE_PARK
#define PT_SHADE_PARK 1
#endif
#ifndef PT_SHADE_NT
#define PT_SHADE_NT 1
#endif
typedef float f4v __attribute__((ext_vector_type(4)));
__device__ inline float4 ldQ(const float4* p)
{
#if PT_SHADE_NT
    const f4v v = __builtin_nontemporal_load((const f4v*)p);
    return make_float4(v.x, v.y, v.z, v.w);
#else
    return *p;
#endif
}
__device__ inline void stQ(float4* p, float4 v)
{
#if PT_SHADE_NT
    const f4v w = { v.x, v.y, v.z, v.w };
    __builtin_nontemporal_store(w, (f4v*)p);
#else
    *p = v;
#endif
}

template <bool PARITY, bool GENERAL = false, bool LOOP = false, bool BINNED = false>
__global__ void __launch_bounds__(kShadeBlock, (PARITY || GENERAL || LOOP) ? 4 : PT_SHADE_MIN_WAVES) k_shade(ShadeArgs a)
{
    static_assert(!(PARITY && LOOP), "the parity kernel stages at the input slot: one tile per workgroup");
    static_assert(!BINNED || (!PARITY && !LOOP), "material order: production queue semantics, one tile per workgroup");
    const uint32_t count = *a.inCount;
    uint32_t tile = a.firstTile + blockIdx.x;
    if (tile * kShadeBlock >= count)
        return;
    __shared__ uint32_t sCount[kShadeBlock / 64][4];
    __shared__ uint32_t sBase[4];
  do {
    uint32_t i = tile * kShadeBlock + threadIdx.x;
    const uint32_t lane = threadIdx.x & 63u;
    if (BINNED) {
        constexpr uint32_t kWaves = kShadeBlock / 64u, kKeys = 64u / kWaves;
        static_assert(kKeys * kWaves == 64u, "one lane per (key, wave) counter");
        __shared__ uint32_t sBin[kKeys * kWaves];
        __shared__ uint16_t sPerm[kShadeBlock];
        const uint32_t w = threadIdx.x >> 6;
        uint32_t key = kKeys - 1u;
        if (i < count) {
            const int prim = (int)((const uint32_t*)&a.hits.h[i])[3];
            key = prim < 0 ? 5u : min(asU(a.sc.triFat[prim].mat.w), 4u);
        }
        uint32_t rank = 0u;
#pragma unroll
        for (uint32_t k = 0; k < kKeys; k++) {
            const unsigned long long m = __ballot(key == k);
            if (key == k)
                rank = (uint32_t)__popcll(m & ((1ull << lane) - 1ull));
            if (lane == 0)
                sBin[k * kWaves + w] = (uint32_t)__popcll(m);
        }
        __syncthreads();
        if (threadIdx.x < 64u) {
            const uint32_t v = sBin[threadIdx.x];
            uint32_t incl = v;
#pragma unroll
            for (int o = 1; o < 64; o <<= 1) {
                const uint32_t up = __shfl_up(incl, o);
                if ((int)lane >= o)
                    incl += up;
            }
            sBin[threadIdx.x] = incl - v;
        }
        __syncthreads();
        sPerm[sBin[key * kWaves + w] + rank] = (uint16_t)threadIdx.x;
        __syncthreads();
        i = tile * kShadeBlock + sPerm[threadIdx.x];
    }
#if PT_SHADE_PARK
    __shared__ float sPark[PARITY ? 1 : 10][PARITY ? 1 : kShadeBlock];
#endif
    bool emitRay = false, emitShadow = false, shaded = false, deposited = false;
    ShadeResult r;
    uint32_t pixel = 0, bounce = 0, plane = 0;
    if (i < count) {
        const float4 rd = ldQ(&a.in.d[i]);
        float4 ro;
        uint32_t fb;
        if (!PARITY && a.derivedPrimaries) {
            ro = a.fp.cam.eye;
            pixel = asU(rd.w);
            const uint32_t span = a.fp.numOwned << a.fp.interleaveShift;
            uint32_t group = (uint32_t)((float)i * a.fp.invSpan);
            if (group * span > i)
                group--;
            if ((group + 1u) * span <= i)
                group++;
            fb = packState(FLAG_LASTSPECULAR, 0u, (group << a.fp.interleaveShift) + (i & ((1u << a.fp.interleaveShift) - 1u)));
        } else {
            ro = ldQ(&a.in.o[i]);
            fb = asU(rd.w);
            pixel = asU(ro.w);
        }
        bounce = (fb >> 8) & 0xFFu;
        plane = fb >> 16;
        if (!(fb & FLAG_FINISHED)) {
            const float4 h = ldQ(&a.hits.h[i]);
            float4 thr = make_float4(1.f, 1.f, 1.f, 0.f);
            if (PARITY || bounce != 0u)
                thr = ldQ(&a.in.thr[i]);
            const V3 o = xyz(ro), d = xyz(rd), throughput = xyz(thr);
            const int prim = (int)asU(h.w);
            if (prim >= 0) {
                shaded = true;
                const V3 X = o + h.x * d;
                Rng rng = PARITY ? rngLfsrLoad(a.streams, i) : rngCounter(pixel, a.fp.sample + plane, a.fp.seed, 1u + bounce);
                ShadeOpts opt;
                opt.mis = opt.weightedLights = false;
                if (GENERAL) {
                    opt.mis = a.fp.integrator == INTEGRATOR_MIS
                        || (a.fp.integrator == INTEGRATOR_COMPARE && (pixel % a.fp.width) < a.fp.width / 2u);
                    opt.weightedLights = a.fp.weightedLights != 0u;
                    opt.rayOrigin = o;
                    opt.inPdf = thr.w;
                }
#if PT_SHADE_PARK
                shadeHit<GENERAL>(a.sc, X, fastNormalize(d), h.x, h.y, h.z, (uint32_t)prim, (uint32_t)a.hits.inst[i], throughput, fb & 0xFFu, rng, r, opt,
                    PARITY ? nullptr : &sPark[0][threadIdx.x], PARITY ? 0u : (uint32_t)kShadeBlock);
#else
                shadeHit<GENERAL>(a.sc, X, fastNormalize(d), h.x, h.y, h.z, (uint32_t)prim, (uint32_t)a.hits.inst[i], throughput, fb & 0xFFu, rng, r, opt);
#endif
                if (PARITY)
                    rngLfsrStore(a.streams, i, rng);
                if (r.radiance.x != 0.f || r.radiance.y != 0.f || r.radiance.z != 0.f) {
                    float4* ap = a.accum.at(plane, pixel);
                    float4 px = *ap;
                    px.x += r.radiance.x, px.y += r.radiance.y, px.z += r.radiance.z;
                    *ap = px;
                    deposited = true;
                }
                bounce += 1;
                if (bounce >= a.fp.maxBounces)
                    r.flags = FLAG_FINISHED;
                emitRay = PARITY ? true : !(r.flags & FLAG_FINISHED);
                emitShadow = PARITY ? true : !(r.shadowFlags & FLAG_FINISHED);
            } else {
                float4* ap = a.accum.at(plane, pixel);
                float4 px = *ap;
                asm volatile("" : "+v"(px.x), "+v"(px.y), "+v"(px.z), "+v"(px.w));
                const V3 c = throughput * readSkydome(a.sc, fastNormalize(d));
                px.x += c.x, px.y += c.y, px.z += c.z;
                *ap = px;
                deposited = true;
            }
        }
    }
    if (PARITY) {
        const uint32_t nDep = (uint32_t)__popcll(__ballot(deposited));
        if (lane == 0 && nDep)
            atomicAdd(a.deposits, nDep);
        if (i < count)
            a.activeFlag[i] = shaded ? 1u : 0u;
        if (shaded) {
            a.out.o[i] = make_float4(r.origin.x, r.origin.y, r.origin.z, asF(pixel));
            a.out.d[i] = make_float4(r.direction.x, r.direction.y, r.direction.z, asF(packState(r.flags, bounce, plane)));
            a.out.thr[i] = make_float4(r.throughput.x, r.throughput.y, r.throughput.z, GENERAL ? r.pdf : 0.f);
            a.shadow.o[i] = make_float4(r.shadowOrigin.x, r.shadowOrigin.y, r.shadowOrigin.z, r.shadowLength);
            a.shadow.d[i] = make_float4(r.shadowDirection.x, r.shadowDirection.y, r.shadowDirection.z, asF(pixel));
            a.shadow.c[i] = make_float4(r.shadowContribution.x, r.shadowContribution.y, r.shadowContribution.z, asF(packState(r.shadowFlags, 0u, plane)));
        }
        return;
    }
    const unsigned long long mRay = __ballot(emitRay);
    const unsigned long long mSh = __ballot(emitShadow);
    const unsigned long long mHit = __ballot(shaded);
    const unsigned long long mDep = __ballot(deposited);
    const uint32_t wave = threadIdx.x >> 6, nWaves = blockDim.x >> 6;
    if (lane == 0) {
        sCount[wave][0] = (uint32_t)__popcll(mRay);
        sCount[wave][1] = (uint32_t)__popcll(mSh);
        sCount[wave][2] = (uint32_t)__popcll(mHit);
        sCount[wave][3] = (uint32_t)__popcll(mDep);
    }
    __syncthreads();
    if (threadIdx.x < 4) {
        uint32_t sum = 0;
        for (uint32_t w = 0; w < nWaves; w++) {
            const uint32_t n = sCount[w][threadIdx.x];
            sCount[w][threadIdx.x] = sum;
            sum += n;
        }
        uint32_t* counter = threadIdx.x == 0 ? a.outCount : (threadIdx.x == 1 ? a.shadowCount : (threadIdx.x == 2 ? a.shadeHits : a.deposits + (blockIdx.x % kDepositSlots) * 16u));
        sBase[threadIdx.x] = sum ? atomicAdd(counter, sum) : 0u;
    }
    __syncthreads();
    const uint32_t baseRay = sBase[0] + sCount[wave][0], baseSh = sBase[1] + sCount[wave][1];
    const unsigned long long below = (1ull << lane) - 1ull;
    if (emitRay && baseRay + (uint32_t)__popcll(mRay & below) < a.outCap) {
        const uint32_t idx = baseRay + (uint32_t)__popcll(mRay & below);
        stQ(&a.out.o[idx], make_float4(r.origin.x, r.origin.y, r.origin.z, asF(pixel)));
        stQ(&a.out.d[idx], make_float4(r.direction.x, r.direction.y, r.direction.z, asF(packState(r.flags, bounce, plane))));
        stQ(&a.out.thr[idx], make_float4(r.throughput.x, r.throughput.y, r.throughput.z, GENERAL ? r.pdf : 0.f));
    }
    if (emitShadow && baseSh + (uint32_t)__popcll(mSh & below) < a.shadowCap) {
        const uint32_t idx = baseSh + (uint32_t)__popcll(mSh & below);
#if PT_SHADE_PARK
        const float* pk = &sPark[0][PARITY ? 0 : threadIdx.x];
        constexpr uint32_t S = PARITY ? 0 : kShadeBlock;
        stQ(&a.shadow.o[idx], make_float4(pk[0 * S], pk[1 * S], pk[2 * S], pk[3 * S]));
        stQ(&a.shadow.d[idx], make_float4(pk[4 * S], pk[5 * S], pk[6 * S], asF(pixel)));
        stQ(&a.shadow.c[idx], make_float4(pk[7 * S], pk[8 * S], pk[9 * S], asF(packState(0u, 0u, plane))));
#else
        stQ(&a.shadow.o[idx], make_float4(r.shadowOrigin.x, r.shadowOrigin.y, r.shadowOrigin.z, r.shadowLength));
        stQ(&a.shadow.d[idx], make_float4(r.shadowDirection.x, r.shadowDirection.y, r.shadowDirection.z, asF(pixel)));
        stQ(&a.shadow.c[idx], make_float4(r.shadowContribution.x, r.shadowContribution.y, r.shadowContribution.z, asF(packState(0u, 0u, plane))));
#endif
    }
    if (!LOOP)
        break;
    __syncthreads();
    tile += gridDim.x;
  } while (tile * kShadeBlock < count);
}

struct CompactArgs {
    RayQueue staged, out;
    ShadowQueue stagedShadow, outShadow;
    const uint32_t* activeFlag;
    const uint32_t* inCount;
    uint32_t* outCount;
    uint32_t* shadowCount;
    uint32_t* shadeHits;
};
__global__ void __launch_bounds__(1024) k_compact_stable(CompactArgs a)
{
    __shared__ uint32_t scan[1024];
    __shared__ uint32_t carry;
    const uint32_t tid = threadIdx.x;
    const uint32_t count = *a.inCount;
    if (tid == 0)
        carry = 0;
    __syncthreads();
    for (uint32_t tile = 0; tile < count; tile += 1024) {
        const uint32_t i = tile + tid;
        const uint32_t f = (i < count) ? a.activeFlag[i] : 0u;
        scan[tid] = f;
        __syncthreads();
        for (uint32_t off = 1; off < 1024; off <<= 1) {
            uint32_t v = (tid >= off) ? scan[tid - off] : 0u;
            __syncthreads();
            scan[tid] += v;
            __syncthreads();
        }
        const uint32_t base = carry;
        if (f) {
            const uint32_t idx = base + scan[tid] - 1u;
            a.out.o[idx] = a.staged.o[i];
            a.out.d[idx] = a.staged.d[i];
            a.out.thr[idx] = a.staged.thr[i];
            a.outShadow.o[idx] = a.stagedShadow.o[i];
            a.outShadow.d[idx] = a.stagedShadow.d[i];
            a.outShadow.c[idx] = a.stagedShadow.c[i];
        }
        __syncthreads();
        if (tid == 1023)
            carry = base + scan[1023];
        __syncthreads();
    }
    if (tid == 0) {
        *a.outCount = carry;
        *a.shadowCount = carry;
        *a.shadeHits = carry;
    }
}

__device__ inline float resolveExposure(float relativeAperture, float shutterTime, float ISO)
{
    const float EV100 = log2f(relativeAperture * relativeAperture / shutterTime * 100 / ISO);
    return 1.0f / (1.2f * powf(2.0f, EV100));
}
__device__ inline float resolveChannel(float exposed)
{
    const float col = exposed / (1.0f + exposed);
    return (col <= 0.0031308f) ? col * 12.92f : (powf(fabsf(col), 1.0f / 2.4f) * 1.055f) - 0.055f;
}
__global__ void __launch_bounds__(256) k_resolve(const float4* __restrict__ accum, float4* __restrict__ out, uint32_t n, float spp,
    float relativeAperture, float shutterTime, float ISO)
{
    const uint32_t i = blockIdx.x * blockDim.x + threadIdx.x;
    if (i >= n)
        return;
    const float exposure = resolveExposure(relativeAperture, shutterTime, ISO);
    const float4 s = accum[i];
    float c[3] = { s.x / spp * exposure, s.y / spp * exposure, s.z / spp * exposure };
    for (int k = 0; k < 3; k++)
        c[k] = resolveChannel(c[k]);
    out[i] = make_float4(c[0], c[1], c[2], 1.0f);
}

constexpr uint32_t kFoldLanes = 16;
__global__ void __launch_bounds__(256) k_merge_accum(float4* __restrict__ acc, float4* __restrict__ shadowAcc, uint32_t n, uint32_t planes)
{
    const uint32_t i = blockIdx.x * blockDim.x + threadIdx.x;
    if (i >= n)
        return;
    float4 a = acc[i];
    bool any = false;
    for (uint32_t p = 0; p < planes; p++) {
        const float4 b = shadowAcc[(size_t)p * n + i];
        if (b.x != 0.f || b.y != 0.f || b.z != 0.f) {
            a.x += b.x, a.y += b.y, a.z += b.z;
            shadowAcc[(size_t)p * n + i] = make_float4(0.f, 0.f, 0.f, 0.f);
            any = true;
        }
    }
    if (any)
        acc[i] = a;
}

__global__ void __launch_bounds__(256) k_fold_planes(AccumView acc, uint32_t planes, const uint32_t* pixels, uint32_t numOwned)
{
    const uint32_t t = blockIdx.x * blockDim.x + threadIdx.x;
    const uint32_t k = t / kFoldLanes, part = t % kFoldLanes;
    const bool live = k < numOwned;
    const uint32_t i = live ? (pixels ? pixels[k] : k) : 0u;
    float sx = 0.f, sy = 0.f, sz = 0.f;
    const uint32_t slot = acc.ordinal ? k : i;
    if (live)
        for (uint32_t p = 1u + part; p < planes; p += kFoldLanes) {
            float4* e = acc.atOrdinal(p, slot);
            const float4 v = *e;
            sx += v.x, sy += v.y, sz += v.z;
            *e = make_float4(0.f, 0.f, 0.f, 0.f);
        }
    for (int o = kFoldLanes / 2; o > 0; o >>= 1) {
        sx += __shfl_xor(sx, o, kFoldLanes);
        sy += __shfl_xor(sy, o, kFoldLanes);
        sz += __shfl_xor(sz, o, kFoldLanes);
    }
    if (live && part == 0u) {
        float4 s = acc.plane0[i];
        s.x += sx, s.y += sy, s.z += sz;
        acc.plane0[i] = s;
    }
}

__global__ void k_set_word(uint32_t* p, uint32_t v)
{
    if (threadIdx.x == 0 && blockIdx.x == 0)
        *p = v;
}

__global__ void __launch_bounds__(256) k_math_probe(const float* __restrict__ a, const float* __restrict__ b, uint32_t n, float* __restrict__ out)
{
    const uint32_t i = blockIdx.x * blockDim.x + threadIdx.x;
    if (i >= n)
        return;
    const float x = a[i], y = b[i];
    const V3 v = mk(x, y, x + y);
    const V3 np = normalize(v), nf = fastNormalize(v);
    const size_t s = n;
    out[i] = x / y;
    out[s + i] = fastDiv(x, y);
    out[2 * s + i] = sqrtf(fabsf(x));
    out[3 * s + i] = fastSqrt(fabsf(x));
    out[4 * s + i] = np.x, out[5 * s + i] = np.y, out[6 * s + i] = np.z;
    out[7 * s + i] = nf.x, out[8 * s + i] = nf.y, out[9 * s + i] = nf.z;
}

__global__ void __launch_bounds__(256) k_rng_probe(const uint32_t* __restrict__ in, uint32_t n, uint32_t* __restrict__ out)
{
    const uint32_t e = blockIdx.x * blockDim.x + threadIdx.x;
    if (e >= n)
        return;
    const uint32_t* q = in + (size_t)e * 8u;
    uint32_t* o = out + (size_t)e * 20u;
    if (q[0] == 0u) {
        Rng r = rngCounter(q[1], q[2], q[3], q[4]);
        for (int k = 0; k < 20; k++)
            o[k] = __float_as_uint(r.u01());
        return;
    }
    Rng r;
    r.g0 = r.g1 = r.g2 = r.g3 = 0;
    r.weyl = q[1], r.gamma = q[2], r.k1 = q[3];
    r.lfsr = false;
    Rng r2 = r;
    o[0] = __float_as_uint(r.u01());
    o[1] = (uint32_t)r2.randomInteger((int)q[4], (int)q[5]);
    o[2] = __float_as_uint(r2.u01());
    for (int k = 3; k < 20; k++)
        o[k] = 0u;
}

__global__ void k_clamp_counts(Control* ctl, uint32_t pass, uint32_t outCap, uint32_t shadowCap, uint32_t* overflowPinned)
{
    if (blockIdx.x != 0 || threadIdx.x != 0)
        return;
    bool cut = false;
    if (ctl->extCount[pass + 1] > outCap)
        ctl->extCount[pass + 1] = outCap, cut = true;
    if (ctl->shadowCount[pass] > shadowCap)
        ctl->shadowCount[pass] = shadowCap, cut = true;
    if (cut)
        *overflowPinned = 1u;
}

__global__ void k_end_sample(Control* ctl, Totals* tot, uint32_t passes, uint32_t* countsOut)
{
    static_assert(kMaxPasses < 64 && kDepositSlots <= 64u, "one lane per pass / per deposit slot");
    if (blockIdx.x != 0 || threadIdx.x >= 64u)
        return;
    const uint32_t lane = threadIdx.x;
    unsigned long long ext = 0, sh = 0, hits = 0, slots = 0;
    if (countsOut && lane <= (uint32_t)kMaxPasses) {
        countsOut[lane] = lane <= passes ? ctl->extCount[lane] : 0u;
        countsOut[kMaxPasses + 1 + lane] = lane <= passes ? ctl->shadowCount[lane] : 0u;
    }
    if (lane <= passes && lane <= (uint32_t)kMaxPasses) {
        ext = ctl->extCount[lane];
        sh = ctl->shadowCount[lane];
        hits = ctl->shadeHits[lane];
        ctl->extCount[lane] = ctl->shadowCount[lane] = ctl->extCursor[lane] = ctl->shadowCursor[lane] = ctl->shadeHits[lane] = 0;
    }
    if (lane < kDepositSlots) {
        slots = ctl->depositSlots[lane][0];
        ctl->depositSlots[lane][0] = 0;
    }
#pragma unroll
    for (int m = 32; m >= 1; m >>= 1) {
        ext += __shfl_xor(ext, m);
        sh += __shfl_xor(sh, m);
        hits += __shfl_xor(hits, m);
        slots += __shfl_xor(slots, m);
    }
    if (lane == 0) {
        tot->raysExtension += ext;
        tot->raysShadow += sh;
        tot->shadeHits += hits;
        tot->raysGenerated += ctl->generated;
        tot->deposits += slots + ctl->depositsShade + ctl->depositsShadow;
        tot->depositsShadow += ctl->depositsShadow;
        ctl->generated = 0;
        ctl->depositsShade = ctl->depositsShadow = 0;
    }
}

}
```

### opencl-path-tracer_amd/csrc/pt_walk.h

```cpp
#pragma once
#include "pt_shade.h"
#include <type_traits>

namespace ptd {

typedef float f2 __attribute__((ext_vector_type(2)));

constexpr uint32_t kGuidedSpans = 1;

struct TraceArgs {
    SceneDev sc;
    const float4* rayO;
    const float4* rayD;
    const float4* rayC;
    float4* hit;
    int32_t* inst;
    AccumView accum;
    uint32_t* occluded;
    Control* ctl;
    uint32_t pass;
    uint32_t fused;
    uint32_t noOrigins;
    const uint32_t* pixelList;
    FrameParams fp;
    uint32_t* spill;
    uint32_t totalThreads;
    uint32_t parityShadow;
    const float4* instFold;
    uint32_t instFoldCount;
};

#ifdef PT_TRACE_STATS
__device__ unsigned long long g_traceStats[64];
constexpr int kTraceStats = 18;
#define PT_STAT_BEGIN unsigned long long statAcc[kTraceStats] = {}
#define PT_STAT(i, v) statAcc[i] += (unsigned long long)(v)
#define PT_TIC(t) const unsigned long long t = __builtin_readcyclecounter()
#define PT_TOC(i, t) statAcc[i] += __builtin_readcyclecounter() - t
#define PT_STAT_END(base)                                   \
    if (lane == 0)                                          \
        for (int i = 0; i < kTraceStats; i++)               \
            atomicAdd(&g_traceStats[i + (base)], statAcc[i])
#else
#define PT_STAT_BEGIN
#define PT_STAT(i, v)
#define PT_TIC(t)
#define PT_TOC(i, t)
#define PT_STAT_END(base)
#endif

__device__ inline float fmaPlain(float a, float b, float c)
{
    float r;
    asm("v_fma_f32 %0, %1, %2, %3" : "=v"(r) : "v"(a), "v"(b), "v"(c));
    return r;
}
__device__ inline uint32_t times3(uint32_t x)
{
    uint32_t r;
    asm("v_lshl_add_u32 %0, %1, 1, %1" : "=v"(r) : "v"(x));
    return r;
}
__device__ inline f2 planePair(const f2 q, const float a, const float b) { return { fmaPlain(q.x, a, b), fmaPlain(q.y, a, b) }; }
__device__ inline float rcpSlab(float x) { return fminf(fmaxf(fastRcp(x), -1e18f), 1e18f); }

template <typename Vec>
__device__ inline void nudgeZero(Vec& o, Vec& d)
{
    if (d.x == 0.0f) d.x = FLT_MIN;
    if (d.y == 0.0f) d.y = FLT_MIN;
    if (d.z == 0.0f) d.z = FLT_MIN;
    if (o.x == 0.0f) o.x = -FLT_MIN;
    if (o.y == 0.0f) o.y = -FLT_MIN;
    if (o.z == 0.0f) o.z = -FLT_MIN;
}

struct SlabSetup {
    float ax, ay, az, bx, by, bz;
    uint32_t qnx, qfx, qny, qfy, qnz, qfz;
};
__device__ inline void slabCoefficients(SlabSetup& s, const uint4 A, const uint4 C, const V3 o, const V3 invDir)
{
    s.ax = asF(A.w) * invDir.x, s.ay = asF(C.z) * invDir.y, s.az = asF(C.w) * invDir.z;
    s.bx = (asF(A.x) - o.x) * invDir.x, s.by = (asF(A.y) - o.y) * invDir.y, s.bz = (asF(A.z) - o.z) * invDir.z;
}
__device__ inline void slabPlanes(SlabSetup& s, const uint4 B, const uint4 C, const bool nx, const bool ny, const bool nz)
{
    s.qnx = nx ? B.y : B.x, s.qfx = nx ? B.x : B.y;
    s.qny = ny ? B.w : B.z, s.qfy = ny ? B.z : B.w;
    s.qnz = nz ? C.y : C.x, s.qfz = nz ? C.x : C.y;
}
__device__ inline SlabSetup slabSetup(const uint4 A, const uint4 B, const uint4 C, const V3 o, const V3 invDir, const bool nx, const bool ny, const bool nz)
{
    SlabSetup s;
    slabCoefficients(s, A, C, o, invDir);
    slabPlanes(s, B, C, nx, ny, nz);
    return s;
}
__device__ inline SlabSetup slabSetup(const uint4 A, const uint4 B, const uint4 C, const V3 o, const V3 invDir)
{
    SlabSetup s;
    slabCoefficients(s, A, C, o, invDir);
    slabPlanes(s, B, C, invDir.x < 0.f, invDir.y < 0.f, invDir.z < 0.f);
    return s;
}
__device__ inline f2 childSlab(const SlabSetup& s, const int k)
{
    const f2 qx = { (float)((s.qnx >> (8 * k)) & 0xFFu), (float)((s.qfx >> (8 * k)) & 0xFFu) };
    const f2 qy = { (float)((s.qny >> (8 * k)) & 0xFFu), (float)((s.qfy >> (8 * k)) & 0xFFu) };
    const f2 qz = { (float)((s.qnz >> (8 * k)) & 0xFFu), (float)((s.qfz >> (8 * k)) & 0xFFu) };
    const f2 tx = planePair(qx, s.ax, s.bx), ty = planePair(qy, s.ay, s.by), tz = planePair(qz, s.az, s.bz);
    return { fmaxf(fmaxf(tx.x, ty.x), tz.x), fminf(fminf(tx.y, ty.y), tz.y) };
}

__device__ inline void sortSwap(float& ki, float& kj, uint32_t& ri, uint32_t& rj)
{
    const bool sw = kj < ki;
    const float tk = sw ? kj : ki;
    kj = sw ? ki : kj;
    ki = tk;
    const uint32_t tr = sw ? rj : ri;
    rj = sw ? ri : rj;
    ri = tr;
}
__device__ inline void sort4NearestToFront(float (&key)[4], uint32_t (&ref)[4])
{
    sortSwap(key[0], key[1], ref[0], ref[1]), sortSwap(key[2], key[3], ref[2], ref[3]), sortSwap(key[0], key[2], ref[0], ref[2]);
}
__device__ inline void sort4Nearest(float (&key)[4], uint32_t (&ref)[4])
{
    sort4NearestToFront(key, ref);
    sortSwap(key[1], key[3], ref[1], ref[3]), sortSwap(key[1], key[2], ref[1], ref[2]);
}

__device__ inline void triEdges(const float4 ta, const float4 tb, const float tcx, V3* v0, V3* e1, V3* e2)
{
    *v0 = mk(ta.x, ta.y, ta.z), *e1 = mk(ta.w, tb.x, tb.y), *e2 = mk(tb.z, tb.w, tcx);
}
__device__ inline void fetchTri(const SceneDev& sc, const uint32_t index, V3* v0, V3* e1, V3* e2)
{
    static_assert(sizeof(TriIsect) == 48, "48 = 3 << 4: a shift-add and a shift instead of a quarter-rate 32-bit multiply");
    const TriIsect* tp = (const TriIsect*)((const char*)sc.tris + (size_t)(uint32_t)(times3(index) << 4));
    const float4 ta = tp->a, tb = tp->b;
    const float tcx = tp->c.x;
    triEdges(ta, tb, tcx, v0, e1, e2);
}

__device__ inline V3 crossExact(const V3 a, const V3 b)
{
#pragma clang fp contract(off)
    return mk(__builtin_fmaf(a.y, b.z, -(a.z * b.y)), __builtin_fmaf(a.z, b.x, -(a.x * b.z)), __builtin_fmaf(a.x, b.y, -(a.y * b.x)));
}
__device__ inline float dotExact(const V3 a, const V3 b)
{
#pragma clang fp contract(off)
    return __builtin_fmaf(a.z, b.z, __builtin_fmaf(a.x, b.x, a.y * b.y));
}
__device__ inline void triOriginHalf(const V3 o, const V3 v0, const V3 e1, const V3 e2, V3* T, V3* Q, float* e2Q)
{
#pragma clang fp contract(off)
    *T = mk(o.x - v0.x, o.y - v0.y, o.z - v0.z);
    *Q = crossExact(*T, e1);
    *e2Q = dotExact(e2, *Q);
}
__device__ inline void triRayHalf(const V3 d, const V3 e1, const V3 e2, const V3 T, const V3 Q, const float e2Q, float* det, float* u, float* v, float* t)
{
#pragma clang fp contract(off)
    const V3 P = crossExact(d, e2);
    const float pz = e1.z * P.z;
    *det = pz + __builtin_fmaf(e1.x, P.x, e1.y * P.y);
    const float inv = fastRcp(*det);
    *u = dotExact(T, P) * inv;
    *v = dotExact(d, Q) * inv;
    *t = e2Q * inv;
}
__device__ inline void triangleTest(const V3 o, const V3 d, const V3 v0, const V3 e1, const V3 e2, float* det, float* u, float* v, float* t)
{
    V3 T, Q;
    float e2Q;
    triOriginHalf(o, v0, e1, e2, &T, &Q, &e2Q);
// ... 32 lines not shown
```

### opencl-path-tracer_amd/csrc/ptamd.hip

```cpp
#include "../../include/ptamd.h"
#include "pt_shade.h"
#include "pt_trace.h"
#include "pt_packet.h"
#include "pt_packet_multi.h"
#include "pt_bake.h"
#include "pt_team.h"
#include "pt_denoise.h"
#include "pt_temporal.h"
#ifndef PT_PACK_WIDE
#define PT_PACK_WIDE 1
#endif
#include <algorithm>
#include <atomic>
#include <dlfcn.h>
#if __has_include(<rccl/rccl.h>)
#include <rccl/rccl.h>
#define PT_HAVE_RCCL_HEADER 1
#endif
#include <chrono>
#include <cmath>
#include <cstdarg>
#include <cstdio>
#include <cstring>
#include <functional>
// ... 229 lines not shown
    float best = 0.f;
    for (uint32_t r = 0; r <= std::max(repeat, 1u); r++) {
        (void)hipEventRecord(e0, c->stream);
        hipLaunchKernelGGL(k_copy_probe, dim3(blocks), dim3(256), 0, c->stream, src.p, dst.p, n);
        (void)hipEventRecord(e1, c->stream);
        HIPCHK(c, hipStreamSynchronize(c->stream));
        float ms = 0;
        (void)hipEventElapsedTime(&ms, e0, e1);
        if (r > 0 && ms > 0.f)
            best = std::max(best, (float)(2.0 * (double)n * sizeof(float4) / (ms * 1e-3) / 1e9));
    }
    *gbps_out = best;
    return PT_OK;
    });
}

int pt_debug_math_probe(pt_ctx* c, const float* a, const float* b, uint32_t n, float* out)
{
    return guarded(c, "pt_debug_math_probe", [&]() -> int {
    if (!c || !a || !b || !out || n == 0)
        return PT_ERR_INVALID;
    HIPCHK(c, hipSetDevice(c->device));
    DevBuf<float> dA, dB, dOut;
    HIPCHK(c, dA.alloc(n));
    HIPCHK(c, dB.alloc(n));
    HIPCHK(c, dOut.alloc((size_t)n * 10));
    HIPCHK(c, hipMemcpy(dA.p, a, (size_t)n * sizeof(float), hipMemcpyHostToDevice));
    HIPCHK(c, hipMemcpy(dB.p, b, (size_t)n * sizeof(float), hipMemcpyHostToDevice));
    hipLaunchKernelGGL(k_math_probe, dim3((n + 255u) / 256u), dim3(256), 0, c->stream, dA.p, dB.p, n, dOut.p);
    HIPCHK(c, hipGetLastError());
    HIPCHK(c, hipStreamSynchronize(c->stream));
    HIPCHK(c, hipMemcpy(out, dOut.p, (size_t)n * 10 * sizeof(float), hipMemcpyDeviceToHost));
    return PT_OK;
    });
}

int pt_debug_rng_probe(pt_ctx* c, const uint32_t* in, uint32_t n, uint32_t* out)
{
    return guarded(c, "pt_debug_rng_probe", [&]() -> int {
    if (!c || !in || !out || n == 0 || n > (1u << 24))
        return PT_ERR_INVALID;
    HIPCHK(c, hipSetDevice(c->device));
    DevBuf<uint32_t> dIn, dOut;
    HIPCHK(c, dIn.alloc((size_t)n * 8));
    HIPCHK(c, dOut.alloc((size_t)n * 20));
    HIPCHK(c, hipMemcpy(dIn.p, in, (size_t)n * 8 * sizeof(uint32_t), hipMemcpyHostToDevice));
    hipLaunchKernelGGL(k_rng_probe, dim3((n + 255u) / 256u), dim3(256), 0, c->stream, dIn.p, n, dOut.p);
    HIPCHK(c, hipGetLastError());
    HIPCHK(c, hipStreamSynchronize(c->stream));
    HIPCHK(c, hipMemcpy(out, dOut.p, (size_t)n * 20 * sizeof(uint32_t), hipMemcpyDeviceToHost));
    return PT_OK;
    });
}

int pt_debug_live_resources(uint32_t out[4])
{
    if (!out)
        return PT_ERR_INVALID;
    for (int k = 0; k < 4; k++)
        out[k] = g_live[k].load();
    return PT_OK;
}

const char* pt_last_error(const pt_ctx* ctx) { return ctx ? ctx->error.c_str() : g_createError.c_str(); }

int pt_debug_quantise_node(const float* lo12, const float* hi12, const uint32_t* refs4, const uint8_t* empty4, uint32_t emptyRef, void* out64)
{
    if (!lo12 || !hi12 || !refs4 || !empty4 || !out64)
        return PT_ERR_INVALID;
    float lo[4][3], hi[4][3];
    bool empty[4];
    for (int k = 0; k < 4; k++) {
        empty[k] = empty4[k] != 0;
        for (int a = 0; a < 3; a++)
            lo[k][a] = lo12[k * 3 + a], hi[k][a] = hi12[k * 3 + a];
    }
    WideNode w;
    quantiseWideNode(lo, hi, refs4, empty, emptyRef, &w);
    std::memcpy(out64, &w, sizeof(w));
    return PT_OK;
}

int pt_debug_convert(const pt_config* cfg, const pt_vertex* verts, uint32_t nV, const pt_triangle* tris, uint32_t nT, const pt_material* mats, uint32_t nM,
    const pt_sub_bvh_node* nodes, uint32_t nN, const pt_emissive_triangle* lights, uint32_t nL, const pt_top_bvh_node* topNodes, uint32_t nTop, uint32_t topRoot,
    char* line, size_t lineBytes)
{
    return guarded(nullptr, "pt_debug_convert", [&]() -> int {
        if (!cfg || !line)
            return fail(nullptr, PT_ERR_INVALID, "pt_debug_convert: null argument");
        const ptconv::ConvertOptions o = convertOptions(*cfg);
        ptconv::StaticHost s;
        ptconv::DynamicHost d;
        uint64_t versions = 0;
        std::string why;
        ptconv::StageTimer tm("convert", o.timing);
        int rc = ptconv::convertStatic(s, o, versions, verts, nV, tris, nT, mats, nM, nodes, nN, tm, why);
        if (rc == PT_OK && nTop)
            rc = ptconv::convertDynamic(s, o, versions, {}, lights, nL, topNodes, nTop, topRoot, d, why);
        if (rc)
            return fail(nullptr, rc, "%s", why.c_str());
        auto fnv = [](const void* p, size_t n) {
            uint64_t h = 1469598103934665603ull;
            for (size_t i = 0; i < n; i++)
                h = (h ^ ((const uint8_t*)p)[i]) * 1099511628211ull;
            return (unsigned long long)h;
        };
        char buf[1024];
        int n = snprintf(buf, sizeof buf, "wide %zu %016llx boxes %016llx leafOfs %016llx refTri %zu %016llx kidSrc %016llx kidBoxNode %016llx stackNeed %016llx fat %016llx pairs %zu %016llx",
            s.wide.size(), fnv(s.wide.data(), s.wide.size() * sizeof(WideNode)), fnv(s.boxes.data(), s.boxes.size() * sizeof(s.boxes[0])),
            fnv(s.leafOfs.data(), s.leafOfs.size() * 4), s.refTri.size(), fnv(s.refTri.data(), s.refTri.size() * 4), fnv(s.kidSrc.data(), s.kidSrc.size() * 4),
            fnv(s.kidBoxNode.data(), s.kidBoxNode.size() * 4), fnv(s.stackNeed.data(), s.stackNeed.size() * 4), fnv(s.fat.data(), s.fat.size() * sizeof(s.fat[0])),
            s.hostBottomNodes.size(), fnv(s.hostBottomNodes.data(), s.hostBottomNodes.size() * sizeof(PairNode)));
        if (nTop)
            n += snprintf(buf + n, sizeof buf - n, " | topWide %zu %016llx instances %zu %016llx lights %zu %016llx jobs %zu %016llx instanceTopNode %016llx instRoots %zu %016llx "
                "instRootSrc %016llx instFold %zu %016llx hasInstances %d enteredInstances %u enteredGeneral %u foldedInstances %u generalRoute %d bakedNodes %u bakedTris %u "
                "stackNeed %u rootRef %08x rootRefFolded %08x",
                d.topWide.size(), fnv(d.topWide.data(), d.topWide.size() * sizeof(WideNode)), d.instances.size(), fnv(d.instances.data(), d.instances.size() * sizeof(Instance)),
                d.lights.size(), fnv(d.lights.data(), d.lights.size() * sizeof(Light)), d.jobs.size(), fnv(d.jobs.data(), d.jobs.size() * sizeof(BakeJob)),
                fnv(d.instanceTopNode.data(), d.instanceTopNode.size() * 4), d.instRoots.size(), fnv(d.instRoots.data(), d.instRoots.size() * sizeof(WideNode)),
                fnv(d.instRootSrc.data(), d.instRootSrc.size() * 4), d.instFold.size(), fnv(d.instFold.data(), d.instFold.size() * sizeof(float4)), (int)d.hasInstances,
                d.enteredInstances, d.enteredGeneral, d.foldedInstances, (int)d.generalRoute, d.bakedNodes, d.bakedTris, d.stackNeed, d.rootRef, d.rootRefFolded);
        if ((size_t)n >= lineBytes)
            return fail(nullptr, PT_ERR_INVALID, "pt_debug_convert: the line takes %d bytes", n + 1);
        std::memcpy(line, buf, (size_t)n + 1);
        return PT_OK;
    });
}

int pt_create(const pt_config* cfg, pt_ctx** out)
{
    return guarded(nullptr, "pt_create", [&]() -> int {
    if (!cfg || !out)
        return fail(nullptr, PT_ERR_INVALID, "pt_create: null argument");
    if (cfg->width == 0 || cfg->height == 0 || (uint64_t)cfg->width * cfg->height > 0x7FFFFFFFull)
        return fail(nullptr, PT_ERR_INVALID, "pt_create: bad image size %ux%u", cfg->width, cfg->height);
    if (cfg->max_bounces > (uint32_t)kMaxPasses - 1)
        return fail(nullptr, PT_ERR_INVALID, "pt_create: max_bounces > %d", kMaxPasses - 1);
    int count = 0;
    hipError_t e = hipGetDeviceCount(&count);
    if (e != hipSuccess || count == 0)
        return fail(nullptr, PT_ERR_HIP, "pt_create: no HIP device (%s) -- this library has no CPU fallback", hipGetErrorString(e));
    if (cfg->device < 0 || cfg->device >= count)
        return fail(nullptr, PT_ERR_INVALID, "pt_create: device %d out of range (%d devices)", cfg->device, count);
    pt_ctx* c = new pt_ctx();
    c->cfg = *cfg;
    c->packetUse = (cfg->flags & PT_FLAG_NO_PACKETS) ? 0u : kPacketUseDefault;
    if (cfg->flags & PT_FLAG_PACKET_INTERSECT)
        c->packetUse |= 4u;
    if (const char* hs = getenv("PTAMD_SHADE_HEAD_SHIFT"))
        c->shadeHeadShift = (uint32_t)std::max(0, atoi(hs));
    if (const char* pk = getenv("PTAMD_PACKET"))
        if (!(cfg->flags & PT_FLAG_NO_PACKETS))
            c->packetUse = (uint32_t)atoi(pk) | (c->packetUse & 4u);
    c->device = cfg->device;
    auto bail = [&](hipError_t err, const char* what) {
        int rc = fail(nullptr, PT_ERR_HIP, "pt_create: %s: %s", what, hipGetErrorString(err));
        delete c;
        return rc;
    };
    if ((e = hipSetDevice(c->device)) != hipSuccess)
        return bail(e, "hipSetDevice");
    hipDeviceProp_t prop;
    if ((e = hipGetDeviceProperties(&prop, c->device)) != hipSuccess)
        return bail(e, "hipGetDeviceProperties");
    c->numCUs = prop.multiProcessorCount;
    if ((e = c->stream.create()) != hipSuccess)
        return bail(e, "hipStreamCreate");
    if ((e = c->copyStream.create()) != hipSuccess)
        return bail(e, "hipStreamCreate (copy stream)");
    if ((e = c->evStart.create(true)) != hipSuccess || (e = c->evStop.create(true)) != hipSuccess || (e = c->evDenoise[0].create(true)) != hipSuccess
        || (e = c->evDenoise[1].create(true)) != hipSuccess)
        return bail(e, "hipEventCreate");
    if ((e = c->sideStream.create()) != hipSuccess || (e = c->sideStream2.create()) != hipSuccess)
        return bail(e, "hipStreamCreate (side stream)");
    for (int k = 0; k < kMaxPasses; k++)
        if ((e = c->evShaded[k].create()) != hipSuccess || (e = c->evShadowed[k].create()) != hipSuccess)
            return bail(e, "hipEventCreate");
    for (auto& d : c->dyn)
        if ((e = d.uploaded.create()) != hipSuccess || (e = d.lastUse.create()) != hipSuccess || (e = d.stage.read.create()) != hipSuccess)
            return bail(e, "hipEventCreate");
    for (StaticScene& s : c->stat)
        if ((e = s.stage.read.create()) != hipSuccess)
            return bail(e, "hipEventCreate");
    if ((e = c->passCountsPinned.alloc(sizeof(c->passCountsHint) / sizeof(uint32_t))) != hipSuccess || (e = c->passCountsCopied.create()) != hipSuccess)
        return bail(e, "pinned counters");
    std::memset(c->passCountsPinned.p, 0, sizeof(c->passCountsHint));
    if ((e = c->overflowPinned.alloc(1)) != hipSuccess)
        return bail(e, "pinned overflow word");
    *c->overflowPinned.p = 0u;
    if ((e = c->totals.alloc(1)) != hipSuccess || (e = hipMemsetAsync(c->totals.p, 0, sizeof(Totals), c->stream)) != hipSuccess)
        return bail(e, "alloc totals");
    if ((e = c->accumOwn.alloc((size_t)cfg->width * cfg->height)) != hipSuccess
        || (e = hipMemsetAsync(c->accumOwn.p, 0, (size_t)cfg->width * cfg->height * sizeof(float4), c->stream)) != hipSuccess)
        return bail(e, "alloc accumulator");
    c->accum = c->accumOwn.p;
    c->numOwned = cfg->width * cfg->height;
    c->identityPixels = true;
    *out = c;
    int rc = pt_set_tiles(c, nullptr, 0);
    if (rc) {
        g_createError = c->error;
        pt_destroy(c);
        *out = nullptr;
        return rc;
    }
    return PT_OK;
    });
}

void pt_destroy(pt_ctx* c) { delete c; }

int pt_set_stream(pt_ctx* c, void* hip_stream)
{
    if (!c)
        return PT_ERR_INVALID;
    HIPCHK(c, hipSetDevice(c->device));
    HIPCHK(c, hipStreamSynchronize(c->stream));
    if (hip_stream)
        c->stream.adopt((hipStream_t)hip_stream);
    else
        HIPCHK(c, c->stream.create());
    return PT_OK;
}

int pt_upload_static_async(pt_ctx* c, const pt_vertex* verts, uint32_t nV, const pt_triangle* tris, uint32_t nT, const pt_material* mats,
    uint32_t nM, const pt_sub_bvh_node* nodes, uint32_t nN)
{
    return guarded(c, "pt_upload_static_async", [&]() -> int {
        if (!c)
            return PT_ERR_INVALID;
        if (!c->haveStatic || !c->haveDynamic)
            return uploadStaticImpl(c, verts, nV, tris, nT, mats, nM, nodes, nN);
        HIPCHK(c, hipSetDevice(c->device));
        HIPCHK(c, hipStreamSynchronize(c->copyStream));
        const int target = 1 - c->statCur;
        if (c->pending >= 0 && c->dyn[c->pending].staticIndex == target)
            c->pending = -1;
        c->statPending = -1;
        StaticScene* const cur = c->st;
        c->st = &c->stat[target];
        int rc = uploadStaticImpl(c, verts, nV, tris, nT, mats, nM, nodes, nN, true);
        if (rc == PT_OK)
            rc = uploadStaticGeom(c, convertOptions(c->cfg));
        if (rc != PT_OK)
            c->st->have = false;
        c->st = cur;
        if (rc == PT_OK)
            c->statPending = target;
        return rc;
    });
}

int pt_upload_static(pt_ctx* c, const pt_vertex* verts, uint32_t nV, const pt_triangle* tris, uint32_t nT, const pt_material* mats,
    uint32_t nM, const pt_sub_bvh_node* nodes, uint32_t nN)
{
    return guarded(c, "pt_upload_static", [&]() -> int { return uploadStaticImpl(c, verts, nV, tris, nT, mats, nM, nodes, nN); });
}

int pt_update_geometry(pt_ctx* c, const pt_vertex* verts, uint32_t nV, const pt_sub_bvh_node* nodes, uint32_t nN)
{
    return guarded(c, "pt_update_geometry", [&]() -> int {
        if (!c)
            return PT_ERR_INVALID;
        if (!c->haveStatic)
            return fail(c, PT_ERR_STATE, "pt_update_geometry: call pt_upload_static first");
        if (c->statPending >= 0)
            return fail(c, PT_ERR_STATE, "pt_update_geometry: a rebuilt scene (pt_upload_static_async) is waiting for pt_frame_tick: refit after the tick");
        if (!verts || !nodes || nV != c->st->host.numVerts || nN != c->st->host.numRefNodes)
            return fail(c, PT_ERR_INVALID, "pt_update_geometry: the vertex and node counts must be the uploaded ones (%u, %u)", c->st->host.numVerts, c->st->host.numRefNodes);
        for (uint32_t i = 0; i < nN; i++)
            if (nodes[i].leftChildOrFirstTriangle != c->st->host.hostSubNodes[i].leftChildOrFirstTriangle || nodes[i].triangleCount != c->st->host.hostSubNodes[i].triangleCount)
                return fail(c, PT_ERR_INVALID, "pt_update_geometry: node %u changed its links: a refit keeps the topology (use pt_upload_static for a rebuilt tree)", i);
        HIPCHK(c, hipSetDevice(c->device));
        StaticScene& g = *c->st;
        if (g.onDeviceTopology != g.host.topology) {
            refreshHost(g);
            ptconv::refitPairBoxes(g.host, verts, nodes, false);
            ptconv::refitWideOnHost(g.host);
            c->st->host.rawVerts.assign(verts, verts + nV);
            c->st->host.hostSubNodes.assign(nodes, nodes + nN);
            g.latestInStage = false;
            c->st->host.hostGeomStale = true;
            g.host.version = ++c->staticVersions;
            return PT_OK;
        }
        ptconv::refitPairBoxes(g.host, verts, nodes, true);
        const std::vector<float> extra = ptconv::extraBoxes(g.host);
        const size_t bytesV = (size_t)nV * sizeof(pt_vertex), bytesN = (size_t)nN * sizeof(pt_sub_bvh_node), bytesE = extra.size() * sizeof(float);
        const size_t total = bytesV + bytesN + bytesE;
        HIPCHK(c, g.stage.wait());
        if (g.stage.bytes < total && g.latestInStage)
            refreshHost(g);
        HIPCHK(c, g.stage.reserve(total, total + total / 8));
        unsigned char* st = g.stage.mem.p;
        std::memcpy(st, verts, bytesV);
        std::memcpy(st + bytesV, nodes, bytesN);
        g.latestInStage = true;
        c->st->host.hostGeomStale = true;
        g.host.version = ++c->staticVersions;
        HIPCHK(c, hipMemcpyAsync(g.dVerts.p, st, bytesV, hipMemcpyHostToDevice, c->copyStream));
        HIPCHK(c, hipMemcpyAsync(g.dNodes.p, st + bytesV, bytesN, hipMemcpyHostToDevice, c->copyStream));
        if (bytesE) {
            std::memcpy(st + bytesV + bytesN, extra.data(), bytesE);
            if (g.dExtra.n < extra.size())
                HIPCHK(c, g.dExtra.alloc(extra.size()));
            HIPCHK(c, hipMemcpyAsync(g.dExtra.p, st + bytesV + bytesN, bytesE, hipMemcpyHostToDevice, c->copyStream));
        }
        HIPCHK(c, g.stage.recordRead(c->copyStream));
// ... 1190 lines not shown
        return PT_ERR_INVALID;
    if (const int rc = fixedScheduleOnly(c, "pt_set_vertex_motion"))
        return rc;
    if (!c->haveDynamic)
        return fail(c, PT_ERR_STATE, "pt_set_vertex_motion: no dynamic state is active yet (pt_upload_dynamic)");
    if (c->guideSpp != 0)
        return fail(c, PT_ERR_STATE, "pt_set_vertex_motion: %u guide samples are in the sums already -- set or forget the motion right after pt_clear", c->guideSpp);
    if (!enable) {
        c->vertexMotionSet = c->vertexDeformed = false;
        return PT_OK;
    }
    if (c->pending >= 0)
        return fail(c, PT_ERR_STATE, "pt_set_vertex_motion: an upload is pending (pt_upload_dynamic_async without its pt_frame_tick): it is overwriting the set that held the previous state");
    pt_ctx::DynamicSet &cur = c->dyn[c->active], &old = c->dyn[1 - c->active];
    if (!old.used)
        return fail(c, PT_ERR_STATE, "pt_set_vertex_motion: there is no previous state (one pt_frame_tick adopted the only state so far)");
    if (old.staticIndex != cur.staticIndex)
        return fail(c, PT_ERR_UNSUPPORTED, "pt_set_vertex_motion: the previous state was built on another static scene (pt_upload_static_async): rebuilt trees have no vertex motion");
    if (old.numTris != cur.numTris)
        return fail(c, PT_ERR_UNSUPPORTED, "pt_set_vertex_motion: the previous state has %u triangles, the active one %u", old.numTris, cur.numTris);
    HIPCHK(c, hipSetDevice(c->device));
    const bool deformed = old.staticVersion != cur.staticVersion && cur.numTris != 0;
    if (deformed && (old.fat.n < cur.numTris || cur.fat.n < cur.numTris))
        return fail(c, PT_ERR_STATE, "pt_set_vertex_motion: the states hold no shading records for %u triangles", cur.numTris);
    std::vector<MotionRecord> records;
    std::vector<float4> rows;
    if (c->motionSet)
        records = c->motionHost;
    int rc = makeVertexTables(c, c->motionSet, records, rows, "pt_set_vertex_motion");
    if (rc || (rc = c->motionGuides.ensure(c)))
        return rc;
    if (deformed) {
        if (c->fatThen.n < cur.numTris) {
            HIPCHK(c, hipStreamSynchronize(c->stream));
            HIPCHK(c, c->fatThen.alloc(cur.numTris));
        }
        HIPCHK(c, hipMemcpyAsync(c->fatThen.p, old.fat.p, (size_t)cur.numTris * sizeof(TriFat), hipMemcpyDeviceToDevice, c->stream));
        HIPCHK(c, hipEventRecord(old.lastUse, c->stream));
    }
    if ((rc = commitVertexTables(c, c->motionSet, records, rows)))
        return rc;
    c->vertexMotionSet = true;
    c->vertexDeformed = deformed;
    return PT_OK;
    });
}

int pt_vertex_motion(const pt_ctx* c, uint32_t* deformedOut)
{
    if (deformedOut)
        *deformedOut = c && c->vertexMotionSet && c->vertexDeformed ? 1u : 0u;
    return c && c->vertexMotionSet ? 1 : 0;
}

int pt_debug_vertex_motion_rows(const float* invTransforms, uint32_t n, float* out12)
{
    return guarded(nullptr, "pt_debug_vertex_motion_rows", [&]() -> int {
    if (!invTransforms || !out12)
        return fail(nullptr, PT_ERR_INVALID, "pt_debug_vertex_motion_rows: null argument");
    std::vector<float4> rows(std::max<size_t>((size_t)n * 3, 1));
    std::string why;
    const int rc = ptconv::vertexMotionRows(invTransforms, n, rows.data(), why);
    if (rc)
        return fail(nullptr, rc, "pt_debug_vertex_motion_rows: %s", why.c_str());
    std::memcpy(out12, rows.data(), (size_t)n * 3 * sizeof(float4));
    return PT_OK;
    });
}

int pt_read_motion_guides(pt_ctx* c, float* motion, float* prevNormal)
{
    if (!c)
        return PT_ERR_INVALID;
    HIPCHK(c, hipSetDevice(c->device));
    return c->motionGuides.read(c, motion, prevNormal);
}

int pt_write_motion_guides(pt_ctx* c, const float* motion, const float* prevNormal)
{
    if (!c || !motion || !prevNormal)
        return PT_ERR_INVALID;
    HIPCHK(c, hipSetDevice(c->device));
    return c->motionGuides.write(c, motion, prevNormal);
}

void* pt_motion_guides_device_ptr(pt_ctx* c, int which) { return c && (which == 0 || which == 1) ? (void*)c->motionGuides[which] : nullptr; }

int pt_debug_motion_records(const float* prevInv, const float* curInv, uint32_t n, float* out24)
{
    return guarded(nullptr, "pt_debug_motion_records", [&]() -> int {
    if (!prevInv || !curInv || !out24)
        return fail(nullptr, PT_ERR_INVALID, "pt_debug_motion_records: null argument");
    std::vector<MotionRecord> records(std::max<uint32_t>(n, 1u));
    std::string why;
    const int rc = ptconv::motionRecords(prevInv, curInv, n, nullptr, records.data(), nullptr, why);
    if (rc)
        return fail(nullptr, rc, "pt_debug_motion_records: %s", why.c_str());
    std::memcpy(out24, records.data(), (size_t)n * sizeof(MotionRecord));
    return PT_OK;
    });
}

int pt_stats_get(pt_ctx* c, pt_stats* out)
{
    if (!c || !out)
        return PT_ERR_INVALID;
    HIPCHK(c, hipSetDevice(c->device));
    HIPCHK(c, hipStreamSynchronize(c->stream));
    Totals t {};
    HIPCHK(c, hipMemcpy(&t, c->totals.p, sizeof(Totals), hipMemcpyDeviceToHost));
    std::memset(out, 0, sizeof(*out));
    out->rays_extension = t.raysExtension;
    out->rays_shadow = t.raysShadow;
    out->rays_generated = t.raysGenerated;
    out->shade_hits = t.shadeHits;
    out->deposits = t.deposits;
    out->deposits_shadow = t.depositsShadow;
    out->samples = c->spp;
    float ms = 0;
    if (hipEventElapsedTime(&ms, c->evStart, c->evStop) == hipSuccess)
        c->msLastRender = ms;
    else
        (void)hipGetLastError();
    out->ms_last_render = c->msLastRender;
    out->ms_intersect = c->msIntersect;
    out->ms_shade = c->msShade;
    out->ms_shadow = c->msShadow;
    out->ms_gen = c->msGen;
    out->packet_launches = c->packetLaunches;
    out->gen_launches = c->genLaunches;
    out->bundle_launches = c->bundleLaunches;
    out->ms_packet = c->msPacket;
    out->stack_need = c->dyn[c->active].stackNeed;
    out->folded_instances = c->dyn[c->active].foldedInstances;
    out->entered_instances = c->dyn[c->active].enteredInstances;
    out->batch_samples = c->batchSamples;
    out->probe_batches = c->probeBatches;
    out->first_pass_ext_ratio = (float)c->ratioExt, out->first_pass_shadow_ratio = (float)c->ratioShadowFirst;
    out->general_route = c->dyn[c->active].generalRoute ? 1u : 0u;
    out->team_launches = c->teamLaunches;
    return PT_OK;
}

int pt_stats_reset(pt_ctx* c)
{
    if (!c)
        return PT_ERR_INVALID;
    HIPCHK(c, hipSetDevice(c->device));
    HIPCHK(c, hipMemsetAsync(c->totals.p, 0, sizeof(Totals), c->stream));
    c->packetLaunches = c->genLaunches = c->bundleLaunches = c->teamLaunches = 0;
    return PT_OK;
}

int pt_profile_kernels(pt_ctx* c, int enable)
{
    if (!c)
        return PT_ERR_INVALID;
    c->profile = enable != 0;
    return PT_OK;
}

int pt_reduce_accum(pt_ctx* c, void* nccl_comm, int root)
{
    if (!c || !nccl_comm)
        return PT_ERR_INVALID;
    typedef int (*reduce_fn)(const void*, void*, size_t, int, int, int, void*, hipStream_t);
    static reduce_fn reduce = nullptr;
    if (!reduce) {
        void* lib = nullptr;
        if (const char* path = getenv("PTAMD_RCCL_LIB"))
            lib = dlopen(path, RTLD_NOW | RTLD_GLOBAL);
        const char* names[] = { "librccl.so.1", "librccl.so" };
        for (int pass = 0; pass < 2 && !lib; pass++)
            for (const char* n : names)
                if (!lib)
                    lib = dlopen(n, RTLD_NOW | (pass == 0 ? RTLD_NOLOAD : RTLD_GLOBAL));
        if (lib)
            reduce = (reduce_fn)dlsym(lib, "ncclReduce");
        if (!reduce)
            return fail(c, PT_ERR_UNSUPPORTED, "pt_reduce_accum: librccl not found (%s)", dlerror() ? dlerror() : "no ncclReduce symbol");
    }
    HIPCHK(c, hipSetDevice(c->device));
    float* buf = (float*)c->accum;
    const size_t count = (size_t)c->cfg.width * c->cfg.height * 4;
#ifdef PT_HAVE_RCCL_HEADER
    constexpr int kFloat = (int)ncclFloat, kSum = (int)ncclSum;
    static_assert(kFloat == 7 && kSum == 0, "the values this file falls back to where rccl.h is absent at build time");
#else
    constexpr int kFloat = 7, kSum = 0;
#endif
    const int rc = reduce(buf, buf, count, kFloat, kSum, root, nccl_comm, c->stream);
    if (rc != 0)
        return fail(c, PT_ERR_HIP, "pt_reduce_accum: ncclReduce returned %d", rc);
    return PT_OK;
}


namespace {

void unpackRays(const std::vector<float4>& o, const std::vector<float4>& d, float* ox, float* oy, float* oz, float* dx, float* dy, float* dz, uint32_t* pixel)
{
    for (size_t i = 0; i < o.size(); i++) {
        if (ox) ox[i] = o[i].x;
        if (oy) oy[i] = o[i].y;
        if (oz) oz[i] = o[i].z;
        if (dx) dx[i] = d[i].x;
        if (dy) dy[i] = d[i].y;
        if (dz) dz[i] = d[i].z;
        if (pixel)
            std::memcpy(&pixel[i], &o[i].w, 4);
    }
}

void unpackHits(const pt_ctx* c, const std::vector<float4>& h, const std::vector<int32_t>& in, pt_hits_soa* hits)
{
    const std::vector<uint32_t>& top = c->dyn[c->active].instanceTopNode;
    for (size_t i = 0; i < h.size(); i++) {
        hits->t[i] = h[i].x, hits->u[i] = h[i].y, hits->v[i] = h[i].z;
        int32_t prim;
        std::memcpy(&prim, &h[i].w, 4);
        hits->prim[i] = prim;
        hits->inst[i] = (in[i] >= 0 && (size_t)in[i] < top.size()) ? (int32_t)top[in[i]] : -1;
    }
}

}

int pt_intersect(pt_ctx* c, const pt_rays_soa* rays, uint32_t n, int any_hit, pt_hits_soa* hits, uint32_t repeat, float* ms_out)
{
    return guarded(c, "pt_intersect", [&]() -> int {
    if (!c || !rays || !hits || n == 0)
        return PT_ERR_INVALID;
    if (!c->haveStatic || !c->haveDynamic)
        return fail(c, PT_ERR_STATE, "pt_intersect: upload the scene first");
    HIPCHK(c, hipSetDevice(c->device));
    int rc = ensureSpill(c);
    if (rc)
        return rc;
    std::vector<float4> hO(n), hD(n), hC(n);
    for (uint32_t i = 0; i < n; i++) {
        hO[i] = make_float4(rays->ox[i], rays->oy[i], rays->oz[i], any_hit ? rays->tmax[i] : 0.f);
        hD[i] = make_float4(rays->dx[i], rays->dy[i], rays->dz[i], 0.f);
        hC[i] = make_float4(0.f, 0.f, 0.f, 0.f);
    }
    DevBuf<float4> dO, dD, dC, dH, dAcc;
    DevBuf<int32_t> dI;
    DevBuf<uint32_t> dOcc;
    DevBuf<Control> dCtl;
    HIPCHK(c, allocPlanes(dO, dD, dC, n));
    HIPCHK(c, dH.alloc(n));
    HIPCHK(c, dI.alloc(n));
    HIPCHK(c, dOcc.alloc(n));
    HIPCHK(c, dAcc.alloc(1));
    HIPCHK(c, dCtl.alloc(1));
    HIPCHK(c, hipMemcpy(dO.p, hO.data(), n * sizeof(float4), hipMemcpyHostToDevice));
    HIPCHK(c, hipMemcpy(dD.p, hD.data(), n * sizeof(float4), hipMemcpyHostToDevice));
    HIPCHK(c, hipMemcpy(dC.p, hC.data(), n * sizeof(float4), hipMemcpyHostToDevice));
    HIPCHK(c, hipMemsetAsync(dAcc.p, 0, sizeof(float4), c->stream));
    HIPCHK(c, hipMemsetAsync(dH.p, 0xFF, n * sizeof(float4), c->stream));
    HIPCHK(c, hipMemsetAsync(dI.p, 0xFF, n * sizeof(int32_t), c->stream));
    HIPCHK(c, hipMemsetAsync(dOcc.p, 0xFF, n * sizeof(uint32_t), c->stream));
    float msTotal = 0;
    repeat = std::max(repeat, 1u);
    Event e0, e1;
    HIPCHK(c, e0.create(true));
    HIPCHK(c, e1.create(true));
    for (uint32_t r = 0; r < repeat; r++) {
        Control ctl {};
        ctl.extCount[0] = ctl.shadowCount[0] = n;
        HIPCHK(c, hipMemcpyAsync(dCtl.p, &ctl, sizeof(ctl), hipMemcpyHostToDevice, c->stream));
        HIPCHK(c, hipStreamSynchronize(c->stream));
        TraceArgs a = traceArgsBase(c);
        a.parityShadow = 0;
        a.rayO = dO.p, a.rayD = dD.p, a.rayC = dC.p;
        a.hit = dH.p, a.inst = dI.p, a.accum = AccumView { dAcc.p, nullptr, nullptr, 0u }, a.occluded = dOcc.p;
        a.ctl = dCtl.p, a.pass = 0;
        HIPCHK(c, hipEventRecord(e0, c->stream));
        if (c->dyn[c->active].packetOk && (c->packetUse & 4u))
            launchPacket(c, any_hit != 0, a);
        else
            launchTrace(c, any_hit != 0, a);
        HIPCHK(c, hipEventRecord(e1, c->stream));
        HIPCHK(c, hipStreamSynchronize(c->stream));
        HIPCHK(c, hipGetLastError());
        float ms = 0;
        HIPCHK(c, hipEventElapsedTime(&ms, e0, e1));
        msTotal += ms;
    }
    if (any_hit) {
        std::vector<uint32_t> occ(n);
        HIPCHK(c, hipMemcpy(occ.data(), dOcc.p, n * sizeof(uint32_t), hipMemcpyDeviceToHost));
        for (uint32_t i = 0; i < n; i++)
            hits->prim[i] = (int32_t)occ[i];
    } else {
        std::vector<float4> h(n);
        std::vector<int32_t> in(n);
        HIPCHK(c, hipMemcpy(h.data(), dH.p, n * sizeof(float4), hipMemcpyDeviceToHost));
        HIPCHK(c, hipMemcpy(in.data(), dI.p, n * sizeof(int32_t), hipMemcpyDeviceToHost));
        unpackHits(c, h, in, hits);
    }
    if (ms_out)
        *ms_out = msTotal / (float)repeat;
    return PT_OK;
    });
}

// ... 178 lines not shown
```

### opencl-path-tracer_amd/ptamd/device.py

```python
import ctypes as C
import os
import numpy as np
from . import layout as L

_HERE = os.path.dirname(os.path.abspath(__file__))
DEVICE_LIB_PATH = os.environ.get("PTAMD_LIB") or os.path.join(_HERE, "..", "csrc", "libptamd.so")

RNG_COUNTER, RNG_LFSR113_PARITY = 0, 1
TEX_RGBA32F, TEX_BGRA8_UNORM = 0, 1
FLAG_ROWMAJOR_PIXELS = 1
FLAG_NO_BAKED_INSTANCES = 2
FLAG_TWO_LEVEL_ONLY = 4
FLAG_NO_PACKETS = 8
FLAG_PACKET_INTERSECT = 16
FLAG_INTEGRATOR_MIS = 32
FLAG_COMPARE_SHADING = 64
FLAG_SOLID_ANGLE_LIGHTS = 128
FLAG_MATERIAL_BINS = 512
FLAG_PARKED_INSTANCES = 4096
FLAG_TEAM_INTERSECT = 8192
FLAG_QUEUE_PRIMARY_RAYS = 256


class Config(C.Structure):
    _fields_ = [("width", C.c_uint32), ("height", C.c_uint32), ("max_active_rays", C.c_uint32),
                ("max_bounces", C.c_uint32), ("rng_mode", C.c_uint32), ("seed", C.c_uint32), ("device", C.c_int32),
                ("flags", C.c_uint32), ("samples_in_flight", C.c_uint32), ("ext_queue_fraction", C.c_float), ("shadow_queue_fraction", C.c_float)]


class Rect(C.Structure):
    _fields_ = [("x0", C.c_uint32), ("y0", C.c_uint32), ("x1", C.c_uint32), ("y1", C.c_uint32)]


class Stats(C.Structure):
    _fields_ = [("rays_extension", C.c_uint64), ("rays_shadow", C.c_uint64), ("rays_generated", C.c_uint64),
                ("shade_hits", C.c_uint64), ("deposits", C.c_uint64), ("samples", C.c_uint64),
                ("ms_last_render", C.c_double), ("ms_intersect", C.c_double), ("ms_shade", C.c_double),
                ("ms_shadow", C.c_double), ("ms_gen", C.c_double), ("packet_launches", C.c_uint64), ("ms_packet", C.c_double),
                ("deposits_shadow", C.c_uint64), ("gen_launches", C.c_uint64), ("bundle_launches", C.c_uint64),
                ("stack_need", C.c_uint32), ("folded_instances", C.c_uint32), ("team_launches", C.c_uint64),
                ("entered_instances", C.c_uint32), ("batch_samples", C.c_uint32), ("first_pass_ext_ratio", C.c_float), ("first_pass_shadow_ratio", C.c_float), ("probe_batches", C.c_uint32), ("general_route", C.c_uint32)]


class RaysSoA(C.Structure):
    _fields_ = [(n, C.c_void_p) for n in ("ox", "oy", "oz", "dx", "dy", "dz", "tmax")]


class HitsSoA(C.Structure):
    _fields_ = [(n, C.c_void_p) for n in ("t", "u", "v", "prim", "inst")]


class ShadeBatchIO(C.Structure):
    _fields_ = ([("n", C.c_uint32)]
                + [(n, C.c_void_p) for n in ("ox", "oy", "oz", "dx", "dy", "dz", "thr_r", "thr_g", "thr_b", "pixel",
                                             "flags", "bounce", "t", "u", "v", "prim", "inst")]
                + [("sample", C.c_uint32)]
                + [(n, C.c_void_p) for n in ("radiance", "out_alive", "nox", "noy", "noz", "ndx", "ndy", "ndz",
                                             "nthr_r", "nthr_g", "nthr_b", "nflags", "shadow_alive", "sox", "soy",
                                             "soz", "sdx", "sdy", "sdz", "slen", "sc_r", "sc_g", "sc_b")])


DENOISE_TONEMAPPED, DENOISE_HDR = 0, 1
GUIDE_SKY_DEPTH = 1e6


class DenoiseParams(C.Structure):
    _fields_ = [("iterations", C.c_uint32), ("output", C.c_uint32), ("k_normal", C.c_float), ("sigma_depth", C.c_float),
                ("sigma_lum", C.c_float), ("input", C.c_uint32), ("_reserved", C.c_uint32 * 2)]


DENOISE_INPUT_ACCUM, DENOISE_INPUT_TEMPORAL = 0, 1


class TemporalParams(C.Structure):
    _fields_ = [("max_history", C.c_uint32), ("k_normal", C.c_float), ("sigma_depth", C.c_float), ("_reserved", C.c_uint32 * 5)]


DENOISE_INPUT_TEMPORAL_VARIANCE = 2


class VarianceParams(C.Structure):
    _fields_ = [("sigma_variance", C.c_float), ("relative_floor", C.c_float), ("full_history", C.c_float), ("_reserved", C.c_uint32 * 5)]


class ResponseParams(C.Structure):
    _fields_ = [("fast_history", C.c_uint32), ("sigma_response", C.c_float), ("relative_floor", C.c_float), ("_reserved", C.c_uint32 * 5)]


EXPORTS = ["pt_create", "pt_destroy", "pt_last_error", "pt_set_stream", "pt_upload_static", "pt_upload_static_async", "pt_upload_dynamic",
           "pt_upload_dynamic_async", "pt_frame_tick", "pt_update_geometry", "pt_refit_vertices",
           "pt_upload_texture_array", "pt_set_camera", "pt_set_tiles", "pt_set_accum_buffer", "pt_clear", "pt_render",
           "pt_synchronize", "pt_resolve", "pt_resolve_device", "pt_resolve_device_ptr", "pt_read_accum", "pt_write_accum", "pt_accum_device_ptr",
           "pt_samples_per_pixel", "pt_render_guides", "pt_guide_samples", "pt_read_guides", "pt_write_guides", "pt_guides_device_ptr",
           "pt_denoise", "pt_denoise_device", "pt_set_sample_base", "pt_sample_base", "pt_temporal_accumulate", "pt_temporal_reset",
           "pt_temporal_frames", "pt_read_temporal", "pt_write_temporal", "pt_temporal_device_ptr", "pt_set_instance_motion", "pt_instance_motion",
           "pt_read_motion_guides", "pt_write_motion_guides", "pt_motion_guides_device_ptr", "pt_debug_motion_records",
           "pt_set_vertex_motion", "pt_vertex_motion", "pt_debug_vertex_motion_rows", "pt_set_temporal_variance", "pt_temporal_variance",
           "pt_read_temporal_variance", "pt_write_temporal_variance", "pt_temporal_variance_device_ptr",
           "pt_set_temporal_response", "pt_temporal_response", "pt_read_temporal_fast", "pt_write_temporal_fast", "pt_read_temporal_response",
           "pt_temporal_fast_device_ptr", "pt_stats_get", "pt_stats_reset", "pt_profile_kernels", "pt_reduce_accum",
           "pt_intersect", "pt_gen_rays", "pt_primary_pass", "pt_shade_batch", "pt_debug_quantise_node", "pt_debug_convert", "pt_debug_copy_bandwidth", "pt_debug_math_probe", "pt_debug_rng_probe", "pt_debug_live_resources",
           "pt_version"]

_lib = None


def lib():
    global _lib
    if _lib is None:
        if not os.path.exists(DEVICE_LIB_PATH):
            raise RuntimeError(f"{DEVICE_LIB_PATH} missing: the HIP extension was not built "
                               "(run __graft_entry__.build()); there is no CPU fallback")
        try:
            import torch
        except ImportError:
            pass
        l = C.CDLL(DEVICE_LIB_PATH)
        l.pt_last_error.restype = C.c_char_p
        l.pt_last_error.argtypes = [C.c_void_p]
        l.pt_version.restype = C.c_char_p
        l.pt_create.argtypes = [C.POINTER(Config), C.POINTER(C.c_void_p)]
        l.pt_destroy.argtypes = [C.c_void_p]
        l.pt_set_stream.argtypes = [C.c_void_p, C.c_void_p]
        l.pt_upload_static.argtypes = [C.c_void_p, C.c_void_p, C.c_uint32, C.c_void_p, C.c_uint32, C.c_void_p,
                                       C.c_uint32, C.c_void_p, C.c_uint32]
        l.pt_upload_static_async.argtypes = l.pt_upload_static.argtypes
        l.pt_upload_dynamic.argtypes = [C.c_void_p, C.c_void_p, C.c_uint32, C.c_void_p, C.c_uint32, C.c_uint32]
        l.pt_upload_dynamic_async.argtypes = [C.c_void_p, C.c_void_p, C.c_uint32, C.c_void_p, C.c_uint32, C.c_uint32]
        l.pt_frame_tick.argtypes = [C.c_void_p]
        l.pt_update_geometry.argtypes = [C.c_void_p, C.c_void_p, C.c_uint32, C.c_void_p, C.c_uint32]
        l.pt_refit_vertices.argtypes = [C.c_void_p, C.c_uint32, C.c_void_p, C.c_uint32]
        l.pt_upload_texture_array.argtypes = [C.c_void_p, C.c_int, C.c_uint32, C.c_uint32, C.c_uint32, C.c_int, C.c_void_p]
        l.pt_set_camera.argtypes = [C.c_void_p, C.c_void_p]
        l.pt_set_tiles.argtypes = [C.c_void_p, C.c_void_p, C.c_uint32]
        l.pt_set_accum_buffer.argtypes = [C.c_void_p, C.c_void_p]
        l.pt_clear.argtypes = [C.c_void_p]
        l.pt_render.argtypes = [C.c_void_p, C.c_uint32]
        l.pt_synchronize.argtypes = [C.c_void_p]
        l.pt_resolve.argtypes = [C.c_void_p, C.c_void_p]
        l.pt_resolve_device.argtypes = [C.c_void_p, C.c_void_p]
        l.pt_resolve_device_ptr.restype = C.c_void_p
        l.pt_resolve_device_ptr.argtypes = [C.c_void_p]
        l.pt_read_accum.argtypes = [C.c_void_p, C.c_void_p]
        l.pt_write_accum.argtypes = [C.c_void_p, C.c_void_p, C.c_uint32]
        l.pt_accum_device_ptr.restype = C.c_void_p
        l.pt_accum_device_ptr.argtypes = [C.c_void_p]
        l.pt_samples_per_pixel.restype = C.c_uint32
        l.pt_samples_per_pixel.argtypes = [C.c_void_p]
        l.pt_render_guides.argtypes = [C.c_void_p, C.c_uint32]
        l.pt_guide_samples.restype = C.c_uint32
        l.pt_guide_samples.argtypes = [C.c_void_p]
        l.pt_read_guides.argtypes = [C.c_void_p, C.c_void_p, C.c_void_p]
        l.pt_write_guides.argtypes = [C.c_void_p, C.c_void_p, C.c_void_p, C.c_uint32]
        l.pt_guides_device_ptr.restype = C.c_void_p
        l.pt_guides_device_ptr.argtypes = [C.c_void_p, C.c_int]
        l.pt_denoise.argtypes = [C.c_void_p, C.POINTER(DenoiseParams), C.c_void_p, C.POINTER(C.c_float)]
        l.pt_denoise_device.argtypes = [C.c_void_p, C.POINTER(DenoiseParams), C.c_void_p]
        l.pt_set_sample_base.argtypes = [C.c_void_p, C.c_uint32]
        l.pt_sample_base.restype = C.c_uint32
        l.pt_sample_base.argtypes = [C.c_void_p]
        l.pt_temporal_accumulate.argtypes = [C.c_void_p, C.POINTER(TemporalParams)]
        l.pt_temporal_reset.argtypes = [C.c_void_p]
        l.pt_temporal_frames.restype = C.c_uint32
        l.pt_temporal_frames.argtypes = [C.c_void_p]
        l.pt_read_temporal.argtypes = [C.c_void_p, C.c_void_p, C.c_void_p]
        l.pt_write_temporal.argtypes = [C.c_void_p, C.c_void_p, C.c_void_p, C.c_void_p]
        l.pt_temporal_device_ptr.restype = C.c_void_p
        l.pt_temporal_device_ptr.argtypes = [C.c_void_p, C.c_int]
        l.pt_set_instance_motion.argtypes = [C.c_void_p, C.c_void_p, C.c_uint32]
        l.pt_instance_motion.argtypes = [C.c_void_p, C.POINTER(C.c_uint32)]
        l.pt_read_motion_guides.argtypes = [C.c_void_p, C.c_void_p, C.c_void_p]
        l.pt_write_motion_guides.argtypes = [C.c_void_p, C.c_void_p, C.c_void_p]
        l.pt_motion_guides_device_ptr.restype = C.c_void_p
        l.pt_motion_guides_device_ptr.argtypes = [C.c_void_p, C.c_int]
        l.pt_debug_motion_records.argtypes = [C.c_void_p, C.c_void_p, C.c_uint32, C.c_void_p]
        l.pt_set_vertex_motion.argtypes = [C.c_void_p, C.c_int]
        l.pt_vertex_motion.argtypes = [C.c_void_p, C.POINTER(C.c_uint32)]
        l.pt_debug_vertex_motion_rows.argtypes = [C.c_void_p, C.c_uint32, C.c_void_p]
        l.pt_set_temporal_variance.argtypes = [C.c_void_p, C.POINTER(VarianceParams)]
        l.pt_temporal_variance.argtypes = [C.c_void_p]
        l.pt_read_temporal_variance.argtypes = [C.c_void_p, C.c_void_p]
        l.pt_write_temporal_variance.argtypes = [C.c_void_p, C.c_void_p]
        l.pt_temporal_variance_device_ptr.restype = C.c_void_p
        l.pt_temporal_variance_device_ptr.argtypes = [C.c_void_p]
        l.pt_set_temporal_response.argtypes = [C.c_void_p, C.POINTER(ResponseParams)]
        l.pt_temporal_response.argtypes = [C.c_void_p]
        l.pt_read_temporal_fast.argtypes = [C.c_void_p, C.c_void_p]
        l.pt_write_temporal_fast.argtypes = [C.c_void_p, C.c_void_p]
        l.pt_read_temporal_response.argtypes = [C.c_void_p, C.c_void_p]
        l.pt_temporal_fast_device_ptr.restype = C.c_void_p
        l.pt_temporal_fast_device_ptr.argtypes = [C.c_void_p]
        l.pt_stats_get.argtypes = [C.c_void_p, C.POINTER(Stats)]
        l.pt_stats_reset.argtypes = [C.c_void_p]
        l.pt_profile_kernels.argtypes = [C.c_void_p, C.c_int]
        l.pt_reduce_accum.argtypes = [C.c_void_p, C.c_void_p, C.c_int]
        l.pt_intersect.argtypes = [C.c_void_p, C.POINTER(RaysSoA), C.c_uint32, C.c_int, C.POINTER(HitsSoA), C.c_uint32,
                                   C.POINTER(C.c_float)]
        l.pt_gen_rays.argtypes = [C.c_void_p, C.c_uint32, C.c_uint32] + [C.c_void_p] * 7
        l.pt_primary_pass.argtypes = [C.c_void_p, C.c_uint32, C.c_uint32, C.c_uint32] + [C.c_void_p] * 8
        l.pt_shade_batch.argtypes = [C.c_void_p, C.POINTER(ShadeBatchIO)]
        l.pt_debug_convert.argtypes = [C.POINTER(Config)] + [C.c_void_p, C.c_uint32] * 6 + [C.c_uint32, C.c_void_p, C.c_size_t]
        _lib = l
    return _lib


class PtError(RuntimeError):
    pass


def _p(a):
    return None if a is None else a.ctypes.data_as(C.c_void_p)


def live_resources():
    out = (C.c_uint32 * 4)()
    lib().pt_debug_live_resources.argtypes = [C.POINTER(C.c_uint32)]
    rc = lib().pt_debug_live_resources(out)
    if rc != 0:
        raise PtError(f"pt_debug_live_resources failed ({rc})")
    return tuple(out)


def debug_convert(flat, flags=0, rng_mode=RNG_COUNTER):
    cfg = Config(64, 64, 0, 0, rng_mode, 1, 0, flags, 0, 0.0, 0.0)
    line = C.create_string_buffer(2048)
    rc = lib().pt_debug_convert(C.byref(cfg), _p(flat.vertices), len(flat.vertices), _p(flat.triangles), len(flat.triangles), _p(flat.materials),
                                len(flat.materials), _p(flat.sub_nodes), len(flat.sub_nodes), _p(flat.lights), len(flat.lights), _p(flat.top_nodes),
                                len(flat.top_nodes), flat.top_root, line, len(line))
    if rc != 0:
        raise PtError(f"pt_debug_convert failed ({rc}): {lib().pt_last_error(None).decode()}")
    return line.value.decode()


MOTION_RECORD_BYTES = 96


def _inv_transforms(prev):
    prev = np.asarray(prev)
    if prev.dtype.names and "invTransform" in prev.dtype.names:
        prev = prev["invTransform"]
    return np.ascontiguousarray(prev, np.float32).reshape(-1, 16)


def debug_motion_records(prev_inv, cur_inv):
    p, c = _inv_transforms(prev_inv), _inv_transforms(cur_inv)
    assert p.shape == c.shape
    out = np.zeros((len(p), 6, 4), np.float32)
    rc = lib().pt_debug_motion_records(_p(p), _p(c), len(p), _p(out))
    if rc != 0:
        raise PtError(f"pt_debug_motion_records failed ({rc}): {lib().pt_last_error(None).decode()}")
    return out


def debug_vertex_motion_rows(inv):
# ... 177 lines not shown
        self._chk(lib().pt_denoise_device(self._h, C.byref(prm), C.c_void_p(device_ptr) if device_ptr else None), "pt_denoise_device")

    def set_sample_base(self, base):
        self._chk(lib().pt_set_sample_base(self._h, base), "pt_set_sample_base")

    @property
    def sample_base(self):
        return int(lib().pt_sample_base(self._h))

    def temporal_accumulate(self, max_history=0, k_normal=0.0, sigma_depth=0.0, sync=True):
        prm = TemporalParams(max_history, k_normal, sigma_depth)
        self._chk(lib().pt_temporal_accumulate(self._h, C.byref(prm)), "pt_temporal_accumulate")
        if sync:
            self.synchronize()

    def temporal_reset(self):
        self._chk(lib().pt_temporal_reset(self._h), "pt_temporal_reset")

    @property
    def temporal_frames(self):
        return int(lib().pt_temporal_frames(self._h))

    def read_temporal(self):
        cn = np.zeros((self.height * self.width, 4), np.float32)
        nd = np.zeros((self.height * self.width, 4), np.float32)
        self._chk(lib().pt_read_temporal(self._h, _p(cn), _p(nd)), "pt_read_temporal")
        return cn, nd

    def write_temporal(self, colour_count, normal_depth, camera):
        cn = np.ascontiguousarray(colour_count, np.float32)
        nd = np.ascontiguousarray(normal_depth, np.float32)
        assert cn.size == nd.size == self.width * self.height * 4
        cam = np.ascontiguousarray(np.asarray(camera, L.CAMERA).reshape(1))
        self._chk(lib().pt_write_temporal(self._h, _p(cn), _p(nd), _p(cam)), "pt_write_temporal")

    def temporal_device_ptr(self, which):
        return lib().pt_temporal_device_ptr(self._h, which) or 0

    def set_temporal_variance(self, on=True, sigma_variance=0.0, relative_floor=0.0, full_history=0.0):
        prm = VarianceParams(sigma_variance, relative_floor, full_history)
        self._chk(lib().pt_set_temporal_variance(self._h, C.byref(prm) if on else None), "pt_set_temporal_variance")

    @property
    def temporal_variance(self):
        return bool(lib().pt_temporal_variance(self._h))

    def read_temporal_variance(self):
        out = np.zeros(self.height * self.width, np.float32)
        self._chk(lib().pt_read_temporal_variance(self._h, _p(out)), "pt_read_temporal_variance")
        return out

    def write_temporal_variance(self, variance):
        v = np.ascontiguousarray(variance, np.float32)
        assert v.size == self.width * self.height
        self._chk(lib().pt_write_temporal_variance(self._h, _p(v)), "pt_write_temporal_variance")

    @property
    def temporal_variance_device_ptr(self):
        return lib().pt_temporal_variance_device_ptr(self._h) or 0

    def set_temporal_response(self, on=True, fast_history=0, sigma_response=0.0, relative_floor=0.0):
        prm = ResponseParams(fast_history, sigma_response, relative_floor)
        self._chk(lib().pt_set_temporal_response(self._h, C.byref(prm) if on else None), "pt_set_temporal_response")

    @property
    def temporal_response(self):
        return bool(lib().pt_temporal_response(self._h))

    def read_temporal_fast(self):
        out = np.zeros((self.height * self.width, 4), np.float32)
        self._chk(lib().pt_read_temporal_fast(self._h, _p(out)), "pt_read_temporal_fast")
        return out

    def write_temporal_fast(self, colour_count):
        f = np.ascontiguousarray(colour_count, np.float32)
        assert f.size == self.width * self.height * 4
        self._chk(lib().pt_write_temporal_fast(self._h, _p(f)), "pt_write_temporal_fast")

    def read_temporal_response(self):
        out = np.zeros(self.height * self.width, np.float32)
        self._chk(lib().pt_read_temporal_response(self._h, _p(out)), "pt_read_temporal_response")
        return out

    @property
    def temporal_fast_device_ptr(self):
        return lib().pt_temporal_fast_device_ptr(self._h) or 0

    def set_instance_motion(self, prev):
        if prev is None:
            self._chk(lib().pt_set_instance_motion(self._h, None, 0), "pt_set_instance_motion")
            return
        m = _inv_transforms(prev)
        self._chk(lib().pt_set_instance_motion(self._h, _p(m), len(m)), "pt_set_instance_motion")

    @property
    def instance_motion(self):
        moving = C.c_uint32(0)
        return bool(lib().pt_instance_motion(self._h, C.byref(moving))), int(moving.value)

    def read_motion_guides(self):
        m = np.zeros((self.height * self.width, 4), np.float32)
        pn = np.zeros((self.height * self.width, 4), np.float32)
        self._chk(lib().pt_read_motion_guides(self._h, _p(m), _p(pn)), "pt_read_motion_guides")
        return m, pn

    def write_motion_guides(self, motion, prev_normal):
        m = np.ascontiguousarray(motion, np.float32)
        pn = np.ascontiguousarray(prev_normal, np.float32)
        assert m.size == pn.size == self.width * self.height * 4
        self._chk(lib().pt_write_motion_guides(self._h, _p(m), _p(pn)), "pt_write_motion_guides")

    def motion_guides_device_ptr(self, which):
        return lib().pt_motion_guides_device_ptr(self._h, which) or 0

    def set_vertex_motion(self, on=True):
        self._chk(lib().pt_set_vertex_motion(self._h, 1 if on else 0), "pt_set_vertex_motion")

    @property
    def vertex_motion(self):
        deformed = C.c_uint32(0)
        return bool(lib().pt_vertex_motion(self._h, C.byref(deformed))), int(deformed.value)

    def stats(self):
        s = Stats()
        self._chk(lib().pt_stats_get(self._h, C.byref(s)), "pt_stats_get")
        return {n: getattr(s, n) for n, _ in s._fields_}

    def copy_bandwidth(self, nbytes=1 << 30, repeat=5):
        lib().pt_debug_copy_bandwidth.argtypes = [C.c_void_p, C.c_size_t, C.c_uint32, C.POINTER(C.c_float)]
        g = C.c_float(0)
        self._chk(lib().pt_debug_copy_bandwidth(self._h, nbytes, repeat, C.byref(g)), "pt_debug_copy_bandwidth")
        return float(g.value)

    def debug_math_probe(self, a, b):
        a = np.ascontiguousarray(a, np.float32)
        b = np.ascontiguousarray(b, np.float32)
        if a.shape != b.shape or a.ndim != 1:
            raise ValueError("debug_math_probe: a and b must be one-dimensional and of one length")
        out = np.zeros((10, len(a)), np.float32)
        lib().pt_debug_math_probe.argtypes = [C.c_void_p, C.c_void_p, C.c_void_p, C.c_uint32, C.c_void_p]
        self._chk(lib().pt_debug_math_probe(self._h, _p(a), _p(b), len(a), _p(out)), "pt_debug_math_probe")
        return {"div": out[0], "fast_div": out[1], "sqrt": out[2], "fast_sqrt": out[3],
                "normalize": np.ascontiguousarray(out[4:7].T), "fast_normalize": np.ascontiguousarray(out[7:10].T)}

    def debug_rng_probe(self, entries):
        entries = np.ascontiguousarray(entries, np.uint32)
        if entries.ndim != 2 or entries.shape[1] != 8 or len(entries) == 0:
            raise ValueError("debug_rng_probe: entries must be a non-empty (n, 8) uint32 array")
        out = np.zeros((len(entries), 20), np.uint32)
        lib().pt_debug_rng_probe.argtypes = [C.c_void_p, C.c_void_p, C.c_uint32, C.c_void_p]
        self._chk(lib().pt_debug_rng_probe(self._h, _p(entries), len(entries), _p(out)), "pt_debug_rng_probe")
        return out

    def reset_stats(self):
        self._chk(lib().pt_stats_reset(self._h), "pt_stats_reset")

    def profile_kernels(self, enable=True):
        self._chk(lib().pt_profile_kernels(self._h, int(enable)), "pt_profile_kernels")

    def intersect(self, o, d, tmax=None, any_hit=False, repeat=1):
        o = np.ascontiguousarray(o, np.float32)
        d = np.ascontiguousarray(d, np.float32)
        n = len(o)
        cols = [np.ascontiguousarray(o[:, k]) for k in range(3)] + [np.ascontiguousarray(d[:, k]) for k in range(3)]
        tm = np.ascontiguousarray(tmax, np.float32) if tmax is not None else np.full(n, np.inf, np.float32)
        rays = RaysSoA(*[_p(c).value for c in cols], _p(tm).value)
        t, u, v = (np.zeros(n, np.float32) for _ in range(3))
        prim, inst = np.zeros(n, np.int32), np.zeros(n, np.int32)
        hits = HitsSoA(_p(t).value, _p(u).value, _p(v).value, _p(prim).value, _p(inst).value)
        ms = C.c_float(0)
        self._chk(lib().pt_intersect(self._h, C.byref(rays), n, int(any_hit), C.byref(hits), repeat, C.byref(ms)),
                  "pt_intersect")
        return dict(t=t, u=u, v=v, prim=prim, inst=inst, ms=ms.value)

    def gen_rays(self, sample, n):
        arrs = [np.zeros(n, np.float32) for _ in range(6)]
        pixel = np.zeros(n, np.uint32)
        self._chk(lib().pt_gen_rays(self._h, sample, n, *[_p(a) for a in arrs], _p(pixel)), "pt_gen_rays")
        return np.stack(arrs[:3], 1), np.stack(arrs[3:], 1), pixel

    def primary_pass(self, sample, batch, n):
        arrs = [np.zeros(n, np.float32) for _ in range(6)]
        pixel = np.zeros(n, np.uint32)
        t, u, v = (np.zeros(n, np.float32) for _ in range(3))
        prim, inst = np.zeros(n, np.int32), np.zeros(n, np.int32)
        hits = HitsSoA(_p(t).value, _p(u).value, _p(v).value, _p(prim).value, _p(inst).value)
        self._chk(lib().pt_primary_pass(self._h, sample, batch, n, *[_p(a) for a in arrs], _p(pixel), C.byref(hits)), "pt_primary_pass")
        return np.stack(arrs[:3], 1), np.stack(arrs[3:], 1), pixel, dict(t=t, u=u, v=v, prim=prim, inst=inst)

    def shade_batch(self, o, d, thr, pixel, flags, bounce, t, u, v, prim, inst, sample=0):
        n = len(o)
        f32 = lambda a: np.ascontiguousarray(a, np.float32)
        u32 = lambda a: np.ascontiguousarray(a, np.uint32)
        o, d, thr = f32(o), f32(d), f32(thr)
        ins = [f32(o[:, 0]), f32(o[:, 1]), f32(o[:, 2]), f32(d[:, 0]), f32(d[:, 1]), f32(d[:, 2]), f32(thr[:, 0]),
               f32(thr[:, 1]), f32(thr[:, 2]), u32(pixel), u32(flags), u32(bounce), f32(t), f32(u), f32(v),
               np.ascontiguousarray(prim, np.int32), np.ascontiguousarray(inst, np.int32)]
        out = dict(radiance=np.zeros((n, 3), np.float32), out_alive=np.zeros(n, np.uint32))
        for k in ("nox", "noy", "noz", "ndx", "ndy", "ndz", "nthr_r", "nthr_g", "nthr_b"):
            out[k] = np.zeros(n, np.float32)
        out["nflags"] = np.zeros(n, np.uint32)
        out["shadow_alive"] = np.zeros(n, np.uint32)
        for k in ("sox", "soy", "soz", "sdx", "sdy", "sdz", "slen", "sc_r", "sc_g", "sc_b"):
            out[k] = np.zeros(n, np.float32)
        order = ["radiance", "out_alive", "nox", "noy", "noz", "ndx", "ndy", "ndz", "nthr_r", "nthr_g", "nthr_b",
                 "nflags", "shadow_alive", "sox", "soy", "soz", "sdx", "sdy", "sdz", "slen", "sc_r", "sc_g", "sc_b"]
        io = ShadeBatchIO(n, *[_p(a).value for a in ins], sample, *[_p(out[k]).value for k in order])
        self._chk(lib().pt_shade_batch(self._h, C.byref(io)), "pt_shade_batch")
        return out
```

Before: 13160.

## Deposit sky directly for all-miss primary bundles and skip their shading

In the fused primary packet trace, a wave whose whole bundle of camera rays misses the scene now deposits the sky colour into the accumulator directly and sets a per-bundle flag. The first shade pass reads these flags and skips whole tiles or waves that are flagged, so it avoids queue writes, hit writes and shade work for sky-only regions. Camera-ray queue writes are also moved after traversal and use the cached directions, which adds some register pressure and branching in the packet kernel. It adds a flag buffer, per-bundle counters and a debug query for the flag statistics.

After: 13110. No clear change (-0.4%).

```diff
diff --git a/include/ptamd.h b/include/ptamd.h
--- a/include/ptamd.h
+++ b/include/ptamd.h
@@ -297,6 +297,7 @@
 int pt_debug_copy_bandwidth(pt_ctx* ctx, size_t bytes, uint32_t repeat, float* gbps_out);
 int pt_debug_math_probe(pt_ctx* ctx, const float* a, const float* b, uint32_t n, float* out);
 int pt_debug_rng_probe(pt_ctx* ctx, const uint32_t* in, uint32_t n, uint32_t* out);
+int pt_debug_sky_bundles(pt_ctx* ctx, uint64_t* flagged, uint64_t* total);
 int pt_debug_live_resources(uint32_t out[4]);
 int pt_debug_quantise_node(const float* lo12, const float* hi12, const uint32_t* refs4, const uint8_t* empty4, uint32_t empty_ref, void* out64);
 int pt_debug_convert(const pt_config* cfg, const pt_vertex* verts, uint32_t n_verts, const pt_triangle* tris, uint32_t n_tris, const pt_material* mats,
diff --git a/opencl-path-tracer_amd/csrc/pt_context.h b/opencl-path-tracer_amd/csrc/pt_context.h
--- a/opencl-path-tracer_amd/csrc/pt_context.h
+++ b/opencl-path-tracer_amd/csrc/pt_context.h
@@ -302,6 +302,8 @@
     DevBuf<float4> hitH;
     DevBuf<int32_t> hitInst;
     DevBuf<uint32_t> activeFlag;
+    DevBuf<uint32_t> skyFlags;
+    bool skyBundles = true;
     DevBuf<uint4> streams;
     DevBuf<Control> control;
     DevBuf<Totals> totals;
diff --git a/opencl-path-tracer_amd/csrc/pt_device.h b/opencl-path-tracer_amd/csrc/pt_device.h
--- a/opencl-path-tracer_amd/csrc/pt_device.h
+++ b/opencl-path-tracer_amd/csrc/pt_device.h
@@ -173,6 +173,10 @@
 #define PT_GEN_INTERLEAVE 256
 #endif
 constexpr uint32_t kGenInterleave = PT_GEN_INTERLEAVE;
+#ifndef PT_MULTI_RAYS
+#define PT_MULTI_RAYS 4
+#endif
+constexpr uint32_t kBundleEntries = 64u * PT_MULTI_RAYS;
 constexpr uint32_t kDepositSlots = 64;
 struct Control {
     uint32_t extCount[kMaxPasses + 1];
@@ -185,9 +189,11 @@
     uint32_t generated;
     uint32_t _pad;
     uint32_t depositSlots[kDepositSlots][16];
+    uint32_t bundleSlots[kDepositSlots][16];
 };
 struct Totals {
     unsigned long long raysExtension, raysShadow, raysGenerated, shadeHits, deposits, depositsShadow;
+    unsigned long long bundles, skyBundles;
 };
 
 }
diff --git a/opencl-path-tracer_amd/csrc/pt_packet_multi.h b/opencl-path-tracer_amd/csrc/pt_packet_multi.h
--- a/opencl-path-tracer_amd/csrc/pt_packet_multi.h
+++ b/opencl-path-tracer_amd/csrc/pt_packet_multi.h
@@ -1,9 +1,6 @@
 #pragma once
 #include "pt_packet.h"
 
-#ifndef PT_MULTI_RAYS
-#define PT_MULTI_RAYS 4
-#endif
 #ifndef PT_MULTI_MIN_WAVES
 #define PT_MULTI_MIN_WAVES (PT_MULTI_RAYS >= 8 ? 3 : PT_MULTI_RAYS >= 4 ? 5 : 6)
 #endif
@@ -67,6 +64,16 @@
     negSO = -(S * corner);
     mulPos = isFar ? -mHiA : mLoA, mulNeg = isFar ? -mLoA : mHiA;
     ofsQ = 16u + 4u * (2u * axis + ((neg ? 1u : 0u) ^ isFar));
+}
+
+__device__ inline void queueCameraRay(const TraceArgs& a, const uint32_t idx, const V3 o, const V3 d, const uint32_t px, const uint32_t pl)
+{
+    if (a.noOrigins) {
+        ((float4*)a.rayD)[idx] = make_float4(d.x, d.y, d.z, asF(px));
+    } else {
+        ((float4*)a.rayO)[idx] = make_float4(o.x, o.y, o.z, asF(px));
+        ((float4*)a.rayD)[idx] = make_float4(d.x, d.y, d.z, asF(packState(FLAG_LASTSPECULAR, 0u, pl)));
+    }
 }
 
 template <int R, bool TWO_LEVEL, bool LENS = false>
@@ -105,6 +112,7 @@
 #endif
     constexpr uint32_t kSpan = PT_MULTI_SPAN;
     uint32_t spanBase = uni(gwave) * kSpan, spanLeft = kSpan;
+    uint32_t nBundles = 0u, nSky = 0u;
     for (;;) {
         if (spanLeft == 0u) {
             const uint32_t left = supers > spanBase ? supers - spanBase : 0u;
@@ -125,6 +133,7 @@
         float tClosest[R], hu[R], hv[R];
         int hprim[R];
         bool whole = true;
+        bool nudged = false;
 #pragma unroll
         for (int r = 0; r < R; r++) {
             const uint32_t idx = base + 64u * (uint32_t)r + lane;
@@ -134,13 +143,8 @@
                 uint32_t px, pl;
                 primaryEntry(a.fp, a.pixelList, idx, &px, &pl);
                 primaryRay(a.fp, px, pl, &o, &d);
-                if (a.noOrigins) {
-                    ((float4*)a.rayD)[idx] = make_float4(d.x, d.y, d.z, asF(px));
-                } else {
-                    ((float4*)a.rayO)[idx] = make_float4(o.x, o.y, o.z, asF(px));
-                    ((float4*)a.rayD)[idx] = make_float4(d.x, d.y, d.z, asF(packState(FLAG_LASTSPECULAR, 0u, pl)));
-                }
-            }
+            }
+            nudged = nudged || __builtin_amdgcn_ballot_w64(active && (d.x == 0.0f || d.y == 0.0f || d.z == 0.0f || (LENS && (o.x == 0.0f || o.y == 0.0f || o.z == 0.0f)))) != 0ull;
             nudgeZero(o, d);
             if (LENS || r == 0)
                 co[LENS ? r : 0] = o;
@@ -461,17 +465,77 @@
                         tClosest[q] = tC, hu[q] = u_, hv[q] = v_, hprim[q] = hp;
             }
         }
-#pragma unroll
-        for (int r = 0; r < R; r++) {
-            const uint32_t idx = base + 64u * (uint32_t)r + lane;
-            if (idx < count) {
-                int hinst = -1;
-                if constexpr (TWO_LEVEL)
-                    hinst = (int)ldsSave[pwave][kSaveInst + r][lane];
-                writeClosestHit(a, sc, idx, tClosest[r], hu[r], hv[r], hprim[r], hinst);
+        const uint32_t laneR = __builtin_amdgcn_mbcnt_hi(~0u, __builtin_amdgcn_mbcnt_lo(~0u, 0u));
+        bool sky = false;
+        if (a.skyFlags) {
+            bool anyHit = false;
+#pragma unroll
+            for (int r = 0; r < R; r++)
+                anyHit = anyHit || hprim[r] >= 0;
+            sky = a.skyBundles != 0u && base + kPer <= count && __builtin_amdgcn_ballot_w64(anyHit) == 0ull;
+            if (laneR == 0u)
+                a.skyFlags[base / kPer] = sky ? 1u : 0u;
+            nBundles = uni(nBundles + 1u);
+            nSky = uni(nSky + (sky ? 1u : 0u));
+        }
+        if (sky || nudged) {
+#pragma unroll 1
+            for (int r = 0; r < R; r++) {
+                const uint32_t idx = base + 64u * (uint32_t)r + laneR;
+                if (idx < count) {
+                    uint32_t px, pl;
+                    primaryEntry(a.fp, a.pixelList, idx, &px, &pl);
+                    V3 o, d;
+                    if (nudged) {
+                        primaryRay(a.fp, px, pl, &o, &d);
+                    } else {
+                        o = LENS ? co[0] : xyz(a.fp.cam.eye), d = cd[0];
+#pragma unroll
+                        for (int q = 1; q < R; q++)
+                            if (q == r) {
+                                d = cd[q];
+                                if constexpr (LENS)
+                                    o = co[q];
+                            }
+                    }
+                    if (sky)
+                        depositSky(sc, a.accum.at(pl, px), mk(1.0f), d);
+                    else
+                        queueCameraRay(a, idx, o, d, px, pl);
+                }
+            }
+        } else {
+#pragma unroll
+            for (int r = 0; r < R; r++) {
+                const uint32_t idx = base + 64u * (uint32_t)r + laneR;
+                if (idx < count) {
+                    uint32_t px, pl;
+                    primaryEntry(a.fp, a.pixelList, idx, &px, &pl);
+                    queueCameraRay(a, idx, LENS ? co[LENS ? r : 0] : xyz(a.fp.cam.eye), cd[r], px, pl);
+                }
+            }
+        }
+        if (!sky) {
+#pragma unroll
+            for (int r = 0; r < R; r++) {
+                const uint32_t idx = base + 64u * (uint32_t)r + laneR;
+                if (idx < count) {
+                    int hinst = -1;
+                    if constexpr (TWO_LEVEL)
+                        hinst = (int)ldsSave[pwave][kSaveInst + r][lane];
+                    writeClosestHit(a, sc, idx, tClosest[r], hu[r], hv[r], hprim[r], hinst);
+                }
             }
         }
     }
-}
-
-}
+    if (a.skyFlags && __builtin_amdgcn_mbcnt_hi(~0u, __builtin_amdgcn_mbcnt_lo(~0u, 0u)) == 0u) {
+        const uint32_t slot = blockIdx.x % kDepositSlots;
+        atomicAdd(&a.ctl->bundleSlots[slot][0], nBundles);
+        if (nSky) {
+            atomicAdd(&a.ctl->bundleSlots[slot][1], nSky);
+            atomicAdd(&a.ctl->depositSlots[slot][0], nSky * kPer);
+        }
+    }
+}
+
+}
diff --git a/opencl-path-tracer_amd/csrc/pt_schedule.h b/opencl-path-tracer_amd/csrc/pt_schedule.h
--- a/opencl-path-tracer_amd/csrc/pt_schedule.h
+++ b/opencl-path-tracer_amd/csrc/pt_schedule.h
@@ -94,6 +94,8 @@
     return (uint32_t)std::max(1.0, std::min((double)c->planes, b));
 }
 
+inline size_t skyFlagWords(uint32_t cap) { return ((size_t)cap + kBundleEntries - 1u) / kBundleEntries; }
+
 int ensureQueues(pt_ctx* c)
 {
     if (c->queuesReady)
@@ -125,7 +127,7 @@
         c->rays[0].release(), c->rays[1].release(), c->shadow.release(), c->hitH.release(), c->hitInst.release(), c->accumPlanes.release();
         for (ShadowQueueBuf& q : c->shadowQ)
             q.release();
-        c->stagedRays.release(), c->stagedShadow.release(), c->activeFlag.release();
+        c->stagedRays.release(), c->stagedShadow.release(), c->activeFlag.release(), c->skyFlags.release();
         c->foldPlanes = 0;
         const bool split = splitShadowAccum(c, cap);
         c->capExt = c->capShadow = cap;
@@ -144,7 +146,7 @@
         newEpoch(c);
         const uint64_t q0 = 16ull * cap + 32ull * (c->q0Small ? c->capExt : cap);
         const uint64_t need = q0 + 48ull * c->capExt + 48ull * c->capShadow + 20ull * cap + (uint64_t)cap * (parityMode(c) ? 2ull * 48 + 4 : 0)
-            + (uint64_t)(c->planes - 1) * c->numOwned * sizeof(float4)
+            + (uint64_t)(c->planes - 1) * c->numOwned * sizeof(float4) + skyFlagWords(cap) * sizeof(uint32_t)
             + (split ? (uint64_t)cap * 48 * maxBounces(c) + (uint64_t)c->cfg.width * c->cfg.height * sizeof(float4) * maxBounces(c) : 0);
         size_t freeB = 0, totalB = 0;
         HIPCHK(c, hipMemGetInfo(&freeB, &totalB));
@@ -165,6 +167,7 @@
     HIPCHK(c, c->shadow.alloc(c->capShadow));
     HIPCHK(c, c->hitH.alloc(cap));
     HIPCHK(c, c->hitInst.alloc(cap));
+    HIPCHK(c, c->skyFlags.alloc(skyFlagWords(cap)));
     if (parityMode(c)) {
         HIPCHK(c, c->stagedRays.alloc(cap));
         HIPCHK(c, c->stagedShadow.alloc(cap));
@@ -434,7 +437,9 @@
 
 inline bool firstPassCoherent(const pt_ctx* c, const FrameParams& fp, uint32_t batch) { return fp.interleave >= 16u || (PT_FRAME_BUNDLES && batch == 1u && primaryBundles(c)); }
 
-void launchIntersect(pt_ctx* c, int q, uint32_t pass, bool coherent = false, const FrameParams* fused = nullptr, bool noOrigins = false)
+inline bool skyBundlePass(const pt_ctx* c) { return !parityMode(c) && !generalShading(c) && !c->st->host.materialBins; }
+
+void launchIntersect(pt_ctx* c, int q, uint32_t pass, bool coherent = false, const FrameParams* fused = nullptr, bool noOrigins = false, bool skyBundles = false)
 {
     Control* ctl = c->control.p;
     TraceArgs a = traceArgsBase(c);
@@ -452,6 +457,12 @@
     if (coherent && c->dyn[c->active].packetOk && (c->packetUse & 1u)) {
         if (fused && primaryBundles(c)) {
             a.noOrigins = noOrigins ? 1u : 0u;
+            a.skyFlags = nullptr;
+            if (skyBundles) {
+                a.accum = accumView(c);
+                a.skyFlags = c->skyFlags.p;
+                a.skyBundles = c->skyBundles ? 1u : 0u;
+            }
             c->packetLaunches++;
             c->bundleLaunches++;
             if (c->camera.thinLens) {
@@ -491,7 +502,8 @@
         launchTrace(c, true, a, side);
 }
 
-void launchShade(pt_ctx* c, const FrameParams& fp, int in, int out, uint32_t pass, uint32_t launchEntries, const ShadowQueueBuf* ownShadow = nullptr, bool derivedPrimaries = false)
+void launchShade(pt_ctx* c, const FrameParams& fp, int in, int out, uint32_t pass, uint32_t launchEntries, const ShadowQueueBuf* ownShadow = nullptr, bool derivedPrimaries = false,
+    bool skyBundles = false)
 {
     Control* ctl = c->control.p;
     ShadeArgs a {};
@@ -507,6 +519,7 @@
     a.deposits = parityMode(c) ? &ctl->depositsShade : &ctl->depositSlots[0][0];
     a.streams = c->streams.p;
     a.derivedPrimaries = derivedPrimaries ? 1u : 0u;
+    a.skyFlags = skyBundles && pass == 0u ? c->skyFlags.p : nullptr;
     a.outCap = out == 1 ? c->capExt : (c->q0Small ? c->capExt : c->capacity);
     a.shadowCap = ownShadow ? c->capacity : c->capShadow;
     const uint32_t blocks = (std::max(launchEntries, 1u) + kShadeBlock - 1u) / kShadeBlock;
@@ -587,6 +600,7 @@
     const bool packetsFirst = coherentFirst && c->dyn[c->active].packetOk && (c->packetUse & 1u);
     const bool fused = packetsFirst && PT_FUSED_PRIMARY && !(c->cfg.flags & PT_FLAG_QUEUE_PRIMARY_RAYS);
     const bool derived = fused && primaryBundles(c) && !c->camera.thinLens && PT_DERIVED_PRIMARIES;
+    const bool skyPass = fused && primaryBundles(c) && skyBundlePass(c);
     if (c->q0Small && !derived && entries > c->capExt)
         return fail(c, PT_ERR_STATE, "the first queue was sized for camera rays queued as directions only, and this batch queues their origins");
     prof.begin(0);
@@ -608,12 +622,12 @@
         const bool coherent = b == 0 && coherentFirst;
         if (c->profile && coherent && c->dyn[c->active].packetOk && (c->packetUse & 1u))
             prof.marks.back().first = 4;
-        launchIntersect(c, in, b, coherent, fused && b == 0 ? &fp : nullptr, derived && b == 0);
+        launchIntersect(c, in, b, coherent, fused && b == 0 ? &fp : nullptr, derived && b == 0, skyPass && b == 0);
         prof.end();
         if (overlap && !split && b > 0)
             HIPCHK(c, hipStreamWaitEvent(c->stream, c->evShadowed[b - 1], 0));
         prof.begin(2);
-        launchShade(c, fp, in, out, b, entries, split ? &c->shadowQ[b] : nullptr, derived && b == 0);
+        launchShade(c, fp, in, out, b, entries, split ? &c->shadowQ[b] : nullptr, derived && b == 0, skyPass && b == 0);
         if (b == 0 ? smallQueues(c) : c->capShadow < c->capExt) {
             const uint32_t outCap = out == 1 ? c->capExt : (c->q0Small ? c->capExt : c->capacity);
             hipLaunchKernelGGL(k_clamp_counts, dim3(1), dim3(64), 0, c->stream, c->control.p, b, outCap, c->capShadow, c->overflowPinned.p);
diff --git a/opencl-path-tracer_amd/csrc/pt_shade.h b/opencl-path-tracer_amd/csrc/pt_shade.h
--- a/opencl-path-tracer_amd/csrc/pt_shade.h
+++ b/opencl-path-tracer_amd/csrc/pt_shade.h
@@ -654,6 +654,7 @@
     uint32_t firstTile;
     uint32_t derivedPrimaries;
     uint32_t outCap, shadowCap;
+    const uint32_t* skyFlags;
 };
 
 #ifndef PT_SHADE_BLOCK
@@ -689,6 +690,16 @@
 #endif
 }
 
+__device__ inline void depositSky(const SceneDev& sc, float4* ap, const V3 throughput, const V3 d)
+{
+    float4 px = *ap;
+    asm volatile("" : "+v"(px.x), "+v"(px.y), "+v"(px.z), "+v"(px.w));
+    const float len2 = __builtin_fmaf(d.z, d.z, __builtin_fmaf(d.x, d.x, d.y * d.y));
+    const V3 c = throughput * readSkydome(sc, fastNormalize(d, len2));
+    px.x += c.x, px.y += c.y, px.z += c.z;
+    *ap = px;
+}
+
 template <bool PARITY, bool GENERAL = false, bool LOOP = false, bool BINNED = false>
 __global__ void __launch_bounds__(kShadeBlock, (PARITY || GENERAL || LOOP) ? 4 : PT_SHADE_MIN_WAVES) k_shade(ShadeArgs a)
 {
@@ -698,6 +709,19 @@
     uint32_t tile = a.firstTile + blockIdx.x;
     if (tile * kShadeBlock >= count)
         return;
+    constexpr bool SKY = !PARITY && !GENERAL && !LOOP && !BINNED;
+    static_assert(kBundleEntries % 64u == 0u && (kShadeBlock % kBundleEntries == 0u || kBundleEntries % kShadeBlock == 0u), "a wave in one bundle, tiles and bundles nested");
+    bool skyWave = false;
+    if constexpr (SKY) if (a.skyFlags) {
+        bool all = true;
+#pragma unroll
+        for (uint32_t e = 0; e < (uint32_t)kShadeBlock; e += kBundleEntries)
+            all = all && (tile * kShadeBlock + e >= count || a.skyFlags[(tile * kShadeBlock + e) / kBundleEntries] != 0u);
+        if (all)
+            return;
+        const uint32_t first = tile * kShadeBlock + (threadIdx.x & ~63u);
+        skyWave = first < count && __builtin_amdgcn_readfirstlane(a.skyFlags[first / kBundleEntries]) != 0u;
+    }
     __shared__ uint32_t sCount[kShadeBlock / 64][4];
     __shared__ uint32_t sBase[4];
   do {
@@ -746,7 +770,7 @@
     bool emitRay = false, emitShadow = false, shaded = false, deposited = false;
     ShadeResult r;
     uint32_t pixel = 0, bounce = 0, plane = 0;
-    if (i < count) {
+    if (i < count && !skyWave) {
         const float4 rd = ldQ(&a.in.d[i]);
         float4 ro;
         uint32_t fb;
@@ -808,12 +832,7 @@
                 emitRay = PARITY ? true : !(r.flags & FLAG_FINISHED);
                 emitShadow = PARITY ? true : !(r.shadowFlags & FLAG_FINISHED);
             } else {
-                float4* ap = a.accum.at(plane, pixel);
-                float4 px = *ap;
-                asm volatile("" : "+v"(px.x), "+v"(px.y), "+v"(px.z), "+v"(px.w));
-                const V3 c = throughput * readSkydome(a.sc, fastNormalize(d));
-                px.x += c.x, px.y += c.y, px.z += c.z;
-                *ap = px;
+                depositSky(a.sc, a.accum.at(plane, pixel), throughput, d);
                 deposited = true;
             }
         }
@@ -1075,7 +1094,7 @@
     if (blockIdx.x != 0 || threadIdx.x >= 64u)
         return;
     const uint32_t lane = threadIdx.x;
-    unsigned long long ext = 0, sh = 0, hits = 0, slots = 0;
+    unsigned long long ext = 0, sh = 0, hits = 0, slots = 0, bundles = 0, skyBundles = 0;
     if (countsOut && lane <= (uint32_t)kMaxPasses) {
         countsOut[lane] = lane <= passes ? ctl->extCount[lane] : 0u;
         countsOut[kMaxPasses + 1 + lane] = lane <= passes ? ctl->shadowCount[lane] : 0u;
@@ -1089,6 +1108,8 @@
     if (lane < kDepositSlots) {
         slots = ctl->depositSlots[lane][0];
         ctl->depositSlots[lane][0] = 0;
+        bundles = ctl->bundleSlots[lane][0], skyBundles = ctl->bundleSlots[lane][1];
+        ctl->bundleSlots[lane][0] = ctl->bundleSlots[lane][1] = 0;
     }
 #pragma unroll
     for (int m = 32; m >= 1; m >>= 1) {
@@ -1096,8 +1117,12 @@
         sh += __shfl_xor(sh, m);
         hits += __shfl_xor(hits, m);
         slots += __shfl_xor(slots, m);
+        bundles += __shfl_xor(bundles, m);
+        skyBundles += __shfl_xor(skyBundles, m);
     }
     if (lane == 0) {
+        tot->bundles += bundles;
+        tot->skyBundles += skyBundles;
         tot->raysExtension += ext;
         tot->raysShadow += sh;
         tot->shadeHits += hits;
diff --git a/opencl-path-tracer_amd/csrc/pt_walk.h b/opencl-path-tracer_amd/csrc/pt_walk.h
--- a/opencl-path-tracer_amd/csrc/pt_walk.h
+++ b/opencl-path-tracer_amd/csrc/pt_walk.h
@@ -16,7 +16,10 @@
     float4* hit;
     int32_t* inst;
     AccumView accum;
-    uint32_t* occluded;
+    union {
+        uint32_t* occluded;
+        uint32_t* skyFlags;
+    };
     Control* ctl;
     uint32_t pass;
     uint32_t fused;
@@ -25,7 +28,10 @@
     FrameParams fp;
     uint32_t* spill;
     uint32_t totalThreads;
-    uint32_t parityShadow;
+    union {
+        uint32_t parityShadow;
+        uint32_t skyBundles;
+    };
     const float4* instFold;
     uint32_t instFoldCount;
 };
diff --git a/opencl-path-tracer_amd/csrc/ptamd.hip b/opencl-path-tracer_amd/csrc/ptamd.hip
--- a/opencl-path-tracer_amd/csrc/ptamd.hip
+++ b/opencl-path-tracer_amd/csrc/ptamd.hip
@@ -405,8 +405,10 @@
     if (const char* pk = getenv("PTAMD_PACKET"))
         if (!(cfg->flags & PT_FLAG_NO_PACKETS))
             c->packetUse = (uint32_t)atoi(pk) | (c->packetUse & 4u);
+    if (const char* sb = getenv("PTAMD_SKY_BUNDLES"))
+        c->skyBundles = atoi(sb) != 0;
     c->device = cfg->device;
-    auto bail = [&](hipError_t err, const char* what) {
+    auto bail =[&](hipError_t err, const char* what) {
         int rc = fail(nullptr, PT_ERR_HIP, "pt_create: %s: %s", what, hipGetErrorString(err));
         delete c;
         return rc;
@@ -1903,6 +1905,19 @@
     return PT_OK;
 }
 
+int pt_debug_sky_bundles(pt_ctx* c, uint64_t* flagged, uint64_t* total)
+{
+    if (!c || !flagged || !total)
+        return PT_ERR_INVALID;
+    HIPCHK(c, hipSetDevice(c->device));
+    HIPCHK(c, hipStreamSynchronize(c->stream));
+    Totals t {};
+    HIPCHK(c, hipMemcpy(&t, c->totals.p, sizeof(Totals), hipMemcpyDeviceToHost));
+    *flagged = t.skyBundles;
+    *total = t.bundles;
+    return PT_OK;
+}
+
 int pt_profile_kernels(pt_ctx* c, int enable)
 {
     if (!c)
diff --git a/opencl-path-tracer_amd/ptamd/device.py b/opencl-path-tracer_amd/ptamd/device.py
--- a/opencl-path-tracer_amd/ptamd/device.py
+++ b/opencl-path-tracer_amd/ptamd/device.py
@@ -99,7 +99,7 @@
            "pt_read_temporal_variance", "pt_write_temporal_variance", "pt_temporal_variance_device_ptr",
            "pt_set_temporal_response", "pt_temporal_response", "pt_read_temporal_fast", "pt_write_temporal_fast", "pt_read_temporal_response",
            "pt_temporal_fast_device_ptr", "pt_stats_get", "pt_stats_reset", "pt_profile_kernels", "pt_reduce_accum",
-           "pt_intersect", "pt_gen_rays", "pt_primary_pass", "pt_shade_batch", "pt_debug_quantise_node", "pt_debug_convert", "pt_debug_copy_bandwidth", "pt_debug_math_probe", "pt_debug_rng_probe", "pt_debug_live_resources",
+           "pt_intersect", "pt_gen_rays", "pt_primary_pass", "pt_shade_batch", "pt_debug_quantise_node", "pt_debug_convert", "pt_debug_copy_bandwidth", "pt_debug_math_probe", "pt_debug_rng_probe", "pt_debug_sky_bundles", "pt_debug_live_resources",
            "pt_version"]
 
 _lib = None
@@ -583,6 +583,12 @@
         self._chk(lib().pt_debug_rng_probe(self._h, _p(entries), len(entries), _p(out)), "pt_debug_rng_probe")
         return out
 
+    def debug_sky_bundles(self):
+        flagged, total = C.c_uint64(0), C.c_uint64(0)
+        lib().pt_debug_sky_bundles.argtypes = [C.c_void_p, C.POINTER(C.c_uint64), C.POINTER(C.c_uint64)]
+        self._chk(lib().pt_debug_sky_bundles(self._h, C.byref(flagged), C.byref(total)), "pt_debug_sky_bundles")
+        return int(flagged.value), int(total.value)
+
     def reset_stats(self):
         self._chk(lib().pt_stats_reset(self._h), "pt_stats_reset")
 
```
